# MahdiGhafoorian/NLML_HPE

Measured on AMD Instinct MI355X. Metric: faces_per_sec, higher is better.
Workload: dtype f16x2s

## Files before the change

include/nlml_hpe.h:

```cpp
#ifndef NLML_HPE_H
#define NLML_HPE_H

#include <stddef.h>
#include <stdint.h>

#ifdef __cplusplus
extern "C" {
#endif

#define NLML_ABI_VERSION 2

#define NLML_E_BADARG   (-1)
#define NLML_E_BADBLOB  (-2)
#define NLML_E_SHAPE    (-3)

#define NLML_NUM_LANDMARKS 468
#define NLML_F_REFERENCE   1404
#define NLML_LATENT        9
#define NLML_TUCKER_Q      135

int         nlml_abi_version(void);
const char* nlml_last_error(void);

int nlml_normalize_ipd(const float* raw, int64_t B, int normalize,
                       float* out, uint8_t* valid, void* stream);

int nlml_normalize_centroid(const float* raw, int64_t B, float* out, uint8_t* valid, double* stats, void* stream);
int nlml_normalize_centroid_host(const float* h_raw, int64_t B, float* h_out, uint8_t* h_valid, double* h_stats);

#define NLML_ROT_INTRINSIC 0
#define NLML_ROT_EXTRINSIC 1
int nlml_compose_rotation_tensor(const float* base, int64_t I, const double* rot_yaw, int ny, const double* rot_pitch, int np,
                                 const double* rot_roll, int nr, int order, int zero_yaw, int zero_pitch, int zero_roll,
                                 float* out, double* out64, void* stream);
int nlml_rotate_landmarks(const float* lm, const double* rot, float* out, double* out64, int64_t B, void* stream);
int nlml_compose_rotation_tensor_host(const float* h_base, int64_t I, const double* h_rot_yaw, int ny, const double* h_rot_pitch, int np,
                                      const double* h_rot_roll, int nr, int order, int zero_yaw, int zero_pitch, int zero_roll,
                                      float* h_out, double* h_out64);
int nlml_rotate_landmarks_host(const float* h_lm, const double* h_rot, float* h_out, double* h_out64, int64_t B);

#define NLML_MODE_F32   0
#define NLML_MODE_BF16  1
#define NLML_MODE_F16X2 2
#define NLML_MODE_F16X2S 3

size_t nlml_encoder_heads_packed_bytes(int F, int mode);
int    nlml_encoder_heads_pack(int F, int mode,
                               const float* const h_enc_w[6], const float* const h_enc_b[6],
                               const float* const h_head_w[3][5], const float* const h_head_b[3][5],
                               void* h_blob, size_t blob_bytes);

int nlml_encoder_heads_fwd(const float* x, int64_t ldx, int64_t B, int F,
                           const void* blob, size_t blob_bytes,
                           float* out, float* latent, uint8_t* valid, void* stream);

int nlml_encoder_heads_fwd_debug(const float* x, int64_t ldx, int64_t B, int F,
                                 const void* blob, size_t blob_bytes,
                                 float* out, float* latent, float* pre_tanh,
                                 unsigned long long* stamps, void* stream);

int nlml_landmarks_to_pose(const float* raw, int64_t B, int normalize,
                           const void* blob, size_t blob_bytes,
                           float* out, float* latent, uint8_t* valid, void* stream);

size_t nlml_encoder_heads_small_workspace_bytes(int64_t B, int F);
int nlml_encoder_heads_fwd_small(const float* x, int64_t ldx, int64_t B, int F,
                                 const void* blob, size_t blob_bytes, float* out, float* latent, uint8_t* valid,
                                 void* workspace, size_t ws_bytes, void* stream);
int nlml_landmarks_to_pose_small(const float* raw, int64_t B, int normalize,
                                 const void* blob, size_t blob_bytes, float* out, float* latent, uint8_t* valid,
                                 void* workspace, size_t ws_bytes, void* stream);

int nlml_encoder_heads_fwd_streamed(const float* x, int64_t ldx, int64_t B, int F,
                                    const void* blob, size_t blob_bytes, float* out, float* latent, uint8_t* valid,
                                    void* workspace, size_t ws_bytes, void* stream);
int nlml_landmarks_to_pose_streamed(const float* raw, int64_t B, int normalize,
                                    const void* blob, size_t blob_bytes, float* out, float* latent, uint8_t* valid,
                                    void* workspace, size_t ws_bytes, void* stream);

size_t nlml_encoder_heads_workspace_bytes(int64_t B, int F);
int nlml_encoder_heads_fwd_ws(const float* x, int64_t ldx, int64_t B, int F,
                              const void* blob, size_t blob_bytes, float* out, float* latent, uint8_t* valid,
                              void* workspace, size_t ws_bytes, void* stream);
int nlml_landmarks_to_pose_ws(const float* raw, int64_t B, int normalize,
                              const void* blob, size_t blob_bytes, float* out, float* latent, uint8_t* valid,
                              void* workspace, size_t ws_bytes, void* stream);

#define NLML_TD_ORDER_FAST      0
#define NLML_TD_ORDER_REFERENCE 1
int nlml_tucker_objective(const float* Wm, const float* x, int64_t ldx, const int32_t* x_index,
                          const double* params, const double* cos_params, int64_t N,
                          double* err, double* x_hat, void* stream);
int nlml_tucker_objective_ex(const float* Wm, const float* x, int64_t ldx, const int32_t* x_index,
                             const double* params, const double* cos_params, int64_t N,
                             double* err, double* x_hat, int order, void* stream);

int nlml_tucker_powell(const float* Wm, const float* x, int64_t ldx, const double* cos_params, int64_t N,
                       const double* x0, double* result, double* fval, int32_t* nfev, int32_t* nit,
                       int32_t* status, void* stream);
int nlml_tucker_powell_ex(const float* Wm, const float* x, int64_t ldx, const double* cos_params, int64_t N,
                          const double* x0, double* result, double* fval, int32_t* nfev, int32_t* nit,
                          int32_t* status, int order, void* stream);

#define NLML_TUCKER_RANK_MIN 1
#define NLML_TUCKER_RANK_MAX 16
int nlml_tucker_objective_r(const float* Wm, const float* x, int64_t ldx, const int32_t* x_index,
                            const double* params, const double* cos_params, int64_t N,
                            double* err, double* x_hat, int r_id, int order, void* stream);
int nlml_tucker_powell_r(const float* Wm, const float* x, int64_t ldx, const double* cos_params, int64_t N,
                         const double* x0, double* result, double* fval, int32_t* nfev, int32_t* nit,
                         int32_t* status, int r_id, int order, void* stream);

size_t nlml_tucker_gradient_workspace_bytes(int64_t N, int r_id);
int nlml_tucker_gradient_r(const float* Wm, const float* x, int64_t ldx, const int32_t* x_index,
                           const double* params, const double* cos_params, int64_t N,
                           double* err, double* grad, int r_id, void* workspace, size_t workspace_bytes, void* stream);
int nlml_tucker_gradient_host(const float* h_Wm, const float* h_x, int64_t ldx, const int32_t* h_x_index,
                              const double* h_params, const double* h_cos_params, int64_t N,
                              double* h_err, double* h_grad, int r_id, float* h_v);

int nlml_video_post(const float* pose_rad, const float* raw, const uint8_t* valid, int64_t S,
                    double frame_w, double frame_h, double alpha, double max_jump, double size,
                    double* state, double* smoothed, double* centre, double* endpoints, void* stream);
int nlml_video_post_ex(const float* pose_rad, const float* raw, const uint8_t* valid, int64_t S,
                       double frame_w, double frame_h, double alpha, double max_jump, double size,
                       double* state, double* smoothed, double* centre, double* endpoints, uint8_t* updated, void* stream);

#define NLML_POSE_EVAL_MAX_INTERVALS    64
#define NLML_POSE_EVAL_FACES_PER_RECORD 2048
size_t nlml_pose_eval_record_len(int n_intervals);
size_t nlml_pose_eval_result_len(int n_intervals);
size_t nlml_pose_eval_workspace_bytes(int64_t B, int n_intervals);
int nlml_pose_eval(const float* pose_rad, const double* pred_deg, const uint8_t* valid, const double* gt_deg, int64_t B,
                   const double* h_lo, const double* h_hi, int decimals, const double* h_intervals, const int32_t* h_axes,
                   int n_intervals, void* workspace, size_t workspace_bytes, double* record_out, double* result_out,
                   double* pred_out, uint8_t* keep_out, void* stream);
int nlml_pose_eval_merge(const double* records, int64_t n, int n_intervals, double* record_out, double* result_out,
                         void* stream);

int nlml_cosine_table(const float* angles_rad, int64_t n, const double* cos_params, int R, double* out, void* stream);
int nlml_mode5_product(const float* core, const float* U_feat, int Q, int R5, int M, float* W, void* stream);

size_t nlml_powell_state_bytes(void);
int    nlml_powell_init(void* h_state, const double* h_x0, double xtol, double ftol);
int    nlml_powell_step(void* h_state, double fin, double* h_xeval);
int    nlml_powell_result(const void* h_state, double* h_x, double* h_fval, int* h_nfev, int* h_nit, int* h_status);
size_t nlml_powell_state_bytes_n(int n);
int    nlml_powell_init_n(void* h_state, int n, const double* h_x0, double xtol, double ftol);
int    nlml_powell_step_n(void* h_state, double fin, double* h_xeval);
int    nlml_powell_result_n(const void* h_state, double* h_x, double* h_fval, int* h_nfev, int* h_nit, int* h_status);

#ifdef __cplusplus
}
#endif
#endif
```

nlml_hpe_amd/_lib.py:

```python
from __future__ import annotations

import ctypes as C
import os

_HERE = os.path.dirname(os.path.abspath(__file__))
LIB_PATH = os.environ.get("NLML_HPE_LIB") or os.path.join(_HERE, "libnlml_hpe_hip.so")

_c_f32p = C.c_void_p
_FWD_X = [C.c_void_p, C.c_int64, C.c_int64, C.c_int]
_FWD_RAW = [C.c_void_p, C.c_int64, C.c_int]
_FWD_OUT = [C.c_void_p, C.c_size_t, C.c_void_p, C.c_void_p, C.c_void_p]
_FWD_WS = [C.c_void_p, C.c_size_t]


def _k2_forwards():
    for form, ws in (("", []), ("_small", _FWD_WS), ("_streamed", _FWD_WS), ("_ws", _FWD_WS)):
        yield "nlml_encoder_heads_fwd" + form, (C.c_int, _FWD_X + _FWD_OUT + ws + [C.c_void_p])
        yield "nlml_landmarks_to_pose" + form, (C.c_int, _FWD_RAW + _FWD_OUT + ws + [C.c_void_p])


_TD_EVAL = [C.c_void_p, C.c_void_p, C.c_int64, C.c_void_p, C.c_void_p, C.c_void_p, C.c_int64, C.c_void_p, C.c_void_p]
_TD_POWELL = [C.c_void_p, C.c_void_p, C.c_int64, C.c_void_p, C.c_int64] + [C.c_void_p] * 6


def _td_entries():
    for op, head in (("objective", _TD_EVAL), ("powell", _TD_POWELL)):
        for form, tail in (("", []), ("_ex", [C.c_int]), ("_r", [C.c_int, C.c_int])):
            yield f"nlml_tucker_{op}{form}", (C.c_int, head + tail + [C.c_void_p])
    yield "nlml_tucker_gradient_r", (C.c_int, _TD_EVAL + [C.c_int, C.c_void_p, C.c_size_t, C.c_void_p])
    yield "nlml_tucker_gradient_host", (C.c_int, _TD_EVAL + [C.c_int, C.c_void_p])


_ROT_GRID = ([C.c_void_p, C.c_int64] + [C.c_void_p, C.c_int] * 3 + [C.c_int] * 4 + [C.c_void_p, C.c_void_p])

SYMBOLS = {
    **dict(_k2_forwards()),
    **dict(_td_entries()),
    "nlml_abi_version": (C.c_int, []),
    "nlml_last_error": (C.c_char_p, []),
    "nlml_normalize_ipd": (C.c_int, [C.c_void_p, C.c_int64, C.c_int, C.c_void_p, C.c_void_p, C.c_void_p]),
    "nlml_normalize_centroid": (C.c_int, [C.c_void_p, C.c_int64, C.c_void_p, C.c_void_p, C.c_void_p, C.c_void_p]),
    "nlml_normalize_centroid_host": (C.c_int, [C.c_void_p, C.c_int64, C.c_void_p, C.c_void_p, C.c_void_p]),
    "nlml_compose_rotation_tensor": (C.c_int, _ROT_GRID + [C.c_void_p]),
    "nlml_compose_rotation_tensor_host": (C.c_int, _ROT_GRID),
    "nlml_rotate_landmarks": (C.c_int, [C.c_void_p, C.c_void_p, C.c_void_p, C.c_void_p, C.c_int64, C.c_void_p]),
    "nlml_rotate_landmarks_host": (C.c_int, [C.c_void_p, C.c_void_p, C.c_void_p, C.c_void_p, C.c_int64]),
    "nlml_encoder_heads_packed_bytes": (C.c_size_t, [C.c_int, C.c_int]),
    "nlml_encoder_heads_pack": (C.c_int, [C.c_int, C.c_int, C.c_void_p, C.c_void_p, C.c_void_p, C.c_void_p,
                                          C.c_void_p, C.c_size_t]),
    "nlml_encoder_heads_fwd_debug": (C.c_int, [C.c_void_p, C.c_int64, C.c_int64, C.c_int, C.c_void_p, C.c_size_t,
                                               C.c_void_p, C.c_void_p, C.c_void_p, C.c_void_p, C.c_void_p]),
    "nlml_encoder_heads_small_workspace_bytes": (C.c_size_t, [C.c_int64, C.c_int]),
    "nlml_encoder_heads_workspace_bytes": (C.c_size_t, [C.c_int64, C.c_int]),
    "nlml_tucker_gradient_workspace_bytes": (C.c_size_t, [C.c_int64, C.c_int]),
    "nlml_video_post": (C.c_int, [C.c_void_p, C.c_void_p, C.c_void_p, C.c_int64, C.c_double, C.c_double, C.c_double,
                                  C.c_double, C.c_double, C.c_void_p, C.c_void_p, C.c_void_p, C.c_void_p, C.c_void_p]),
    "nlml_video_post_ex": (C.c_int, [C.c_void_p, C.c_void_p, C.c_void_p, C.c_int64, C.c_double, C.c_double, C.c_double,
                                     C.c_double, C.c_double, C.c_void_p, C.c_void_p, C.c_void_p, C.c_void_p, C.c_void_p, C.c_void_p]),
    "nlml_pose_eval_record_len": (C.c_size_t, [C.c_int]),
    "nlml_pose_eval_result_len": (C.c_size_t, [C.c_int]),
    "nlml_pose_eval_workspace_bytes": (C.c_size_t, [C.c_int64, C.c_int]),
    "nlml_pose_eval": (C.c_int, [C.c_void_p, C.c_void_p, C.c_void_p, C.c_void_p, C.c_int64, C.c_void_p, C.c_void_p, C.c_int,
                                 C.c_void_p, C.c_void_p, C.c_int, C.c_void_p, C.c_size_t, C.c_void_p, C.c_void_p, C.c_void_p,
                                 C.c_void_p, C.c_void_p]),
    "nlml_pose_eval_merge": (C.c_int, [C.c_void_p, C.c_int64, C.c_int, C.c_void_p, C.c_void_p, C.c_void_p]),
    "nlml_cosine_table": (C.c_int, [C.c_void_p, C.c_int64, C.c_void_p, C.c_int, C.c_void_p, C.c_void_p]),
    "nlml_mode5_product": (C.c_int, [C.c_void_p, C.c_void_p, C.c_int, C.c_int, C.c_int, C.c_void_p, C.c_void_p]),
    "nlml_powell_state_bytes": (C.c_size_t, []),
    "nlml_powell_init": (C.c_int, [C.c_void_p, C.c_void_p, C.c_double, C.c_double]),
    "nlml_powell_step": (C.c_int, [C.c_void_p, C.c_double, C.c_void_p]),
    "nlml_powell_result": (C.c_int, [C.c_void_p, C.c_void_p, C.c_void_p, C.c_void_p, C.c_void_p, C.c_void_p]),
    "nlml_powell_state_bytes_n": (C.c_size_t, [C.c_int]),
    "nlml_powell_init_n": (C.c_int, [C.c_void_p, C.c_int, C.c_void_p, C.c_double, C.c_double]),
    "nlml_powell_step_n": (C.c_int, [C.c_void_p, C.c_double, C.c_void_p]),
    "nlml_powell_result_n": (C.c_int, [C.c_void_p, C.c_void_p, C.c_void_p, C.c_void_p, C.c_void_p, C.c_void_p]),
}

MODE_F32 = 0
MODE_BF16 = 1
MODE_F16X2 = 2
MODE_F16X2S = 3
MODE_NAMES = {"f32": MODE_F32, "bf16": MODE_BF16, "f16x2": MODE_F16X2, "f16x2s": MODE_F16X2S}
DEFAULT_MODE = MODE_F16X2S
DEFAULT_MODE_NAME = "f16x2s"
TD_ORDER_FAST = 0
TD_ORDER_REFERENCE = 1
TD_ORDER_NAMES = {"fast": TD_ORDER_FAST, "reference": TD_ORDER_REFERENCE}
ROT_INTRINSIC = 0
ROT_EXTRINSIC = 1
ROT_ORDER_NAMES = {"intrinsic": ROT_INTRINSIC, "extrinsic": ROT_EXTRINSIC}
TUCKER_RANK_MIN, TUCKER_RANK_MAX = 1, 16
POSE_EVAL_MAX_INTERVALS = 64
POSE_EVAL_FACES_PER_RECORD = 2048


def td_order_from_name(order) -> int:
    if isinstance(order, str):
        if order not in TD_ORDER_NAMES:
            raise ValueError(f"unknown TD order {order!r}; expected one of {sorted(TD_ORDER_NAMES)}")
        return TD_ORDER_NAMES[order]
    if int(order) not in TD_ORDER_NAMES.values():
        raise ValueError(f"unknown TD order {order!r}")
    return int(order)


def rot_order_from_name(order) -> int:
    if isinstance(order, str):
        if order not in ROT_ORDER_NAMES:
            raise ValueError("Rotation type must be 'intrinsic' or 'extrinsic'.")
        return ROT_ORDER_NAMES[order]
    if int(order) not in ROT_ORDER_NAMES.values():
        raise ValueError(f"unknown rotation order {order!r}")
    return int(order)


def tucker_rank_of_rows(rows: int, what: str = "Wm") -> int:
    r, rem = divmod(int(rows), 27)
    if rem or not TUCKER_RANK_MIN <= r <= TUCKER_RANK_MAX:
        raise ValueError(f"{what}: expected 27*R rows (R*3*3*3) for an identity rank R in [{TUCKER_RANK_MIN}, {TUCKER_RANK_MAX}], "
                         f"got {rows}")
    return r


def mode_from_name(mode) -> int:
    if isinstance(mode, str):
        if mode not in MODE_NAMES:
            raise ValueError(f"unknown mode {mode!r}; expected one of {sorted(MODE_NAMES)}")
        return MODE_NAMES[mode]
    if int(mode) not in MODE_NAMES.values():
        raise ValueError(f"unknown mode {mode!r}")
    return int(mode)

_lib = None


class NlmlError(RuntimeError):
    pass


def lib() -> C.CDLL:
    global _lib
    if _lib is None:
        if not os.path.exists(LIB_PATH):
            raise NlmlError(
                f"{LIB_PATH} is missing: build it with `python -c 'import __graft_entry__ as g; g.build()'` "
                "(make -C nlml_hpe_amd/csrc).  There is no CPU fallback.")
        handle = C.CDLL(LIB_PATH)
        for name, (res, args) in SYMBOLS.items():
            fn = getattr(handle, name)
            fn.restype = res
            fn.argtypes = args
        if handle.nlml_abi_version() != 2:
            raise NlmlError("libnlml_hpe_hip.so ABI version mismatch")
        _lib = handle
    return _lib


def check(rc: int, what: str) -> None:
    if rc != 0:
        msg = lib().nlml_last_error()
        raise NlmlError(f"{what} failed (code {rc}): {msg.decode() if msg else ''}")
```

nlml_hpe_amd/csrc/abi.cpp:

```cpp
#include <hip/hip_runtime_api.h>

#include <cstdio>
#include <cstdlib>
#include <cstring>

#include "../../include/nlml_hpe.h"
#include "abi_internal.h"
#include "centroid_ref.h"
#include "layout.h"
#include "powell.h"
#include "rotate_ref.h"
#include "tucker_grad_ref.h"

namespace nlml {
static thread_local char g_err[256] = "";
int fail(int code, const char* msg) {
  std::snprintf(g_err, sizeof g_err, "%s", msg ? msg : "unknown error");
  return code ? code : NLML_E_BADARG;
}
int hip_launch_status() {
  const hipError_t e = hipGetLastError();
  return e == hipSuccess ? 0 : fail((int)e, hipGetErrorString(e));
}
}

using namespace nlml;

static bool known_mode(int mode) { return mode == NLML_MODE_F32 || mode == NLML_MODE_BF16 || mode == NLML_MODE_F16X2 || mode == NLML_MODE_F16X2S; }
static bool split_f16(int mode) { return mode == NLML_MODE_F16X2 || mode == NLML_MODE_F16X2S; }

extern "C" {

int nlml_abi_version(void) { return NLML_ABI_VERSION; }
const char* nlml_last_error(void) { return g_err; }

int nlml_normalize_ipd(const float* raw, int64_t B, int normalize, float* out, uint8_t* valid, void* stream) {
  if (B < 0 || (B > 0 && (!raw || !out))) return fail(NLML_E_BADARG, "normalize_ipd: null buffer or negative B");
  if ((reinterpret_cast<uintptr_t>(raw) | reinterpret_cast<uintptr_t>(out)) & 15)
    return fail(NLML_E_BADARG, "normalize_ipd: raw/out must be 16-byte aligned");
  return launch_normalize_ipd(raw, B, normalize, out, valid, stream);
}

int nlml_normalize_centroid(const float* raw, int64_t B, float* out, uint8_t* valid, double* stats, void* stream) {
  if (B < 0 || (B > 0 && (!raw || !out))) return fail(NLML_E_BADARG, "normalize_centroid: null buffer or negative B");
  if ((reinterpret_cast<uintptr_t>(raw) | reinterpret_cast<uintptr_t>(out)) & 15)
    return fail(NLML_E_BADARG, "normalize_centroid: raw/out must be 16-byte aligned");
  if (reinterpret_cast<uintptr_t>(stats) & 7) return fail(NLML_E_BADARG, "normalize_centroid: stats must be 8-byte aligned");
  return launch_normalize_centroid(raw, B, out, valid, stats, stream);
}

int nlml_normalize_centroid_host(const float* h_raw, int64_t B, float* h_out, uint8_t* h_valid, double* h_stats) {
  if (B < 0 || (B > 0 && (!h_raw || !h_out))) return fail(NLML_E_BADARG, "normalize_centroid_host: null buffer or negative B");
  for (int64_t b = 0; b < B; ++b) {
    const int v = cn_face_host(h_raw + b * NLML_F_REFERENCE, h_out + b * NLML_F_REFERENCE, h_stats ? h_stats + 4 * b : nullptr);
    if (h_valid) h_valid[b] = (uint8_t)v;
  }
  return 0;
}

static int check_rotation_grid(const char* who, bool have_buffers, int64_t I, int ny, int np, int nr, int order, int zy, int zp, int zr,
                               int64_t* rows) {
  char msg[128];
  const bool empty = I == 0 || ny == 0 || np == 0 || nr == 0;
  auto refuse = [&](const char* what) {
    std::snprintf(msg, sizeof msg, "%s: %s", who, what);
    return fail(NLML_E_BADARG, msg);
  };
  if (!empty && !have_buffers) return refuse("null buffer");
  if (I < 0 || ny < 0 || np < 0 || nr < 0) return refuse("negative extent");
  if (order != NLML_ROT_INTRINSIC && order != NLML_ROT_EXTRINSIC) return refuse("unknown order");
  if (zy < -1 || zy >= ny || zp < -1 || zp >= np || zr < -1 || zr >= nr) return refuse("zero index outside -1..n-1");
  *rows = 0;
  if (empty) return 0;
  int64_t n = 0;
  if (__builtin_mul_overflow(I, (int64_t)ny, &n) || __builtin_mul_overflow(n, (int64_t)np, &n) || __builtin_mul_overflow(n, (int64_t)nr, &n) ||
      n > INT64_MAX / (NLML_F_REFERENCE * 8))
    return refuse("tensor too large for 64-bit byte offsets");
  *rows = n;
  return 0;
}

int nlml_compose_rotation_tensor(const float* base, int64_t I, const double* rot_yaw, int ny, const double* rot_pitch, int np,
                                 const double* rot_roll, int nr, int order, int zero_yaw, int zero_pitch, int zero_roll, float* out,
                                 double* out64, void* stream) {
  int64_t rows;
  if (const int rc = check_rotation_grid("compose_rotation_tensor", base && rot_yaw && rot_pitch && rot_roll && out, I, ny, np, nr, order,
                                         zero_yaw, zero_pitch, zero_roll, &rows))
    return rc;
  if (rows == 0) return 0;
  if ((reinterpret_cast<uintptr_t>(base) | reinterpret_cast<uintptr_t>(out)) & 15)
    return fail(NLML_E_BADARG, "compose_rotation_tensor: base/out must be 16-byte aligned");
  if ((reinterpret_cast<uintptr_t>(rot_yaw) | reinterpret_cast<uintptr_t>(rot_pitch) | reinterpret_cast<uintptr_t>(rot_roll) |
       reinterpret_cast<uintptr_t>(out64)) & 7)
    return fail(NLML_E_BADARG, "compose_rotation_tensor: the matrices and out64 must be 8-byte aligned");
  return launch_compose_rotation_tensor(base, rows, rot_yaw, ny, rot_pitch, np, rot_roll, nr, order, zero_yaw, zero_pitch, zero_roll, out,
                                        out64, stream);
}

int nlml_compose_rotation_tensor_host(const float* h_base, int64_t I, const double* h_rot_yaw, int ny, const double* h_rot_pitch, int np,
                                      const double* h_rot_roll, int nr, int order, int zero_yaw, int zero_pitch, int zero_roll,
                                      float* h_out, double* h_out64) {
  int64_t rows;
  if (const int rc = check_rotation_grid("compose_rotation_tensor_host", h_base && h_rot_yaw && h_rot_pitch && h_rot_roll && (h_out || h_out64),
                                         I, ny, np, nr, order, zero_yaw, zero_pitch, zero_roll, &rows))
    return rc;
  if (rows) rt_grid_host(h_base, I, h_rot_yaw, ny, h_rot_pitch, np, h_rot_roll, nr, order, zero_yaw, zero_pitch, zero_roll, h_out, h_out64);
  return 0;
}

int nlml_rotate_landmarks(const float* lm, const double* rot, float* out, double* out64, int64_t B, void* stream) {
  if (B != 0 && (!lm || !rot || (!out && !out64))) return fail(NLML_E_BADARG, "rotate_landmarks: null buffer (lm, rot, and out or out64)");
  if (B < 0) return fail(NLML_E_BADARG, "rotate_landmarks: negative extent");
  if (B == 0) return 0;
  if (B > INT64_MAX / (NLML_F_REFERENCE * 8)) return fail(NLML_E_BADARG, "rotate_landmarks: too many faces for 64-bit byte offsets");
  if ((reinterpret_cast<uintptr_t>(lm) | reinterpret_cast<uintptr_t>(out)) & 15)
    return fail(NLML_E_BADARG, "rotate_landmarks: lm/out must be 16-byte aligned");
  if ((reinterpret_cast<uintptr_t>(rot) | reinterpret_cast<uintptr_t>(out64)) & 7)
    return fail(NLML_E_BADARG, "rotate_landmarks: rot/out64 must be 8-byte aligned");
  return launch_rotate_landmarks(lm, rot, out, out64, B, stream);
}

int nlml_rotate_landmarks_host(const float* h_lm, const double* h_rot, float* h_out, double* h_out64, int64_t B) {
  if (B != 0 && (!h_lm || !h_rot || (!h_out && !h_out64))) return fail(NLML_E_BADARG, "rotate_landmarks_host: null buffer (lm, rot, and out or out64)");
  if (B < 0) return fail(NLML_E_BADARG, "rotate_landmarks_host: negative extent");
  for (int64_t b = 0; b < B; ++b)
    rt_face_host(h_lm + b * NLML_F_REFERENCE, h_rot + b * 27, h_rot + b * 27 + 9, h_rot + b * 27 + 18,
                 h_out ? h_out + b * NLML_F_REFERENCE : nullptr, h_out64 ? h_out64 + b * NLML_F_REFERENCE : nullptr);
  return 0;
}

size_t nlml_encoder_heads_packed_bytes(int F, int mode) {
  if (F <= 0 || !known_mode(mode)) return 0;
  return blob_bytes_for(F, mode);
}

int nlml_encoder_heads_pack(int F, int mode, const float* const h_enc_w[6], const float* const h_enc_b[6],
                            const float* const h_head_w[3][5], const float* const h_head_b[3][5], void* h_blob,
                            size_t blob_bytes) {
  if (!known_mode(mode)) return fail(NLML_E_BADARG, "pack: unsupported mode");
  if (!h_enc_w || !h_enc_b || !h_head_w || !h_head_b) return fail(NLML_E_BADARG, "pack: null table");
  return pack_blob(F, mode, h_enc_w, h_enc_b, h_head_w, h_head_b, h_blob, blob_bytes);
}

static int check_blob_args(int64_t B, int F, const void* blob, size_t blob_bytes, const float* out, int* mode) {
  if (B < 0 || F <= 0) return fail(NLML_E_BADARG, "encoder_heads: negative B or bad F");
  if (B > 0 && (!blob || !out)) return fail(NLML_E_BADARG, "encoder_heads: null buffer");
  if (reinterpret_cast<uintptr_t>(blob) & 15) return fail(NLML_E_BADARG, "encoder_heads: blob must be 16-byte aligned");
  if (blob_bytes == blob_bytes_for(F, NLML_MODE_F32)) *mode = NLML_MODE_F32;
  else if (blob_bytes == blob_bytes_for(F, NLML_MODE_BF16)) *mode = NLML_MODE_BF16;
  else if (blob_bytes == blob_bytes_for(F, NLML_MODE_F16X2)) *mode = NLML_MODE_F16X2;
  else if (blob_bytes == blob_bytes_for(F, NLML_MODE_F16X2S)) *mode = NLML_MODE_F16X2S;
  else return fail(NLML_E_BADBLOB, "encoder_heads: blob size does not match F in any mode");
  return 0;
}

static const int64_t kSmallMax = 4096;
static int64_t streamed_min() {
  static const int64_t v = [] { const char* e = getenv("NLML_K2_STREAMED_MIN"); return e && e[0] ? (int64_t)atoll(e) : (int64_t)-1; }();
  return v;
}

enum K2Form { K2_FUSED, K2_SMALL, K2_STREAMED, K2_AUTO };

static int k2_forward(K2Form form, bool landmarks, const float* x, int64_t ldx, const float* raw, int normalize, int64_t B, int F,
                      const void* blob, size_t blob_bytes, float* out, float* latent, uint8_t* valid, void* workspace, size_t ws_bytes,
                      void* stream) {
  const char* no_input = nullptr;
  if (B > 0 && landmarks && !raw) no_input = "landmarks_to_pose: null raw";
  if (B > 0 && !landmarks && (!x || ldx < F)) no_input = "encoder_heads: null x or ldx < F";
  if (no_input && form == K2_AUTO && landmarks) return fail(NLML_E_BADARG, no_input);
  int mode = 0;
  if (int rc = check_blob_args(B, F, blob, blob_bytes, out, &mode)) return rc;
  if (form == K2_SMALL && !split_f16(mode)) return fail(NLML_E_BADARG, "small-batch path: NLML_MODE_F16X2 / NLML_MODE_F16X2S blob only");
  if (form == K2_STREAMED && mode != NLML_MODE_F16X2S) return fail(NLML_E_BADARG, "streamed-tail path: NLML_MODE_F16X2S blob only");
  if (no_input) return fail(NLML_E_BADARG, no_input);
  const int split = mode == NLML_MODE_F16X2S;
  if (form == K2_AUTO) {
    if (split_f16(mode) && B <= kSmallMax) form = K2_SMALL;
    else if (split && streamed_min() >= 0 && B >= streamed_min() && k2_input(x, ldx, raw, normalize, F).vec4) form = K2_STREAMED;
    else form = K2_FUSED;
  }
  if (form == K2_SMALL)
    return launch_encoder_heads_f16x2_small(x, ldx, raw, normalize, B, F, blob, out, latent, valid, workspace, ws_bytes, split, stream);
  if (form == K2_STREAMED)
    return launch_encoder_heads_f16x2_tailws(x, ldx, raw, normalize, B, F, blob, out, latent, valid, workspace, ws_bytes, stream);
  if (mode == NLML_MODE_BF16) return launch_encoder_heads_bf16(x, ldx, raw, normalize, B, F, blob, out, latent, valid, stream);
  if (split_f16(mode)) return launch_encoder_heads_f16x2(x, ldx, raw, normalize, B, F, blob, out, latent, valid, split, stream);
  return launch_encoder_heads_f32(x, ldx, raw, normalize, B, F, blob, out, latent, valid, nullptr, nullptr, stream);
}

int nlml_encoder_heads_fwd(const float* x, int64_t ldx, int64_t B, int F, const void* blob, size_t blob_bytes,
                           float* out, float* latent, uint8_t* valid, void* stream) {
  return k2_forward(K2_FUSED, false, x, ldx, nullptr, 0, B, F, blob, blob_bytes, out, latent, valid, nullptr, 0, stream);
}

int nlml_encoder_heads_fwd_debug(const float* x, int64_t ldx, int64_t B, int F, const void* blob, size_t blob_bytes,
                                 float* out, float* latent, float* pre_tanh, unsigned long long* stamps, void* stream) {
  int mode = 0;
  if (int rc = check_blob_args(B, F, blob, blob_bytes, out, &mode)) return rc;
  if (mode != NLML_MODE_F32) return fail(NLML_E_BADARG, "debug build: f32 blob only");
  if (B > 0 && (!x || ldx < F)) return fail(NLML_E_BADARG, "encoder_heads: null x or ldx < F");
  return launch_encoder_heads_f32(x, ldx, nullptr, 0, B, F, blob, out, latent, nullptr, pre_tanh, stamps, stream);
}

int nlml_landmarks_to_pose(const float* raw, int64_t B, int normalize, const void* blob, size_t blob_bytes,
                           float* out, float* latent, uint8_t* valid, void* stream) {
  return k2_forward(K2_FUSED, true, nullptr, 0, raw, normalize, B, NLML_F_REFERENCE, blob, blob_bytes, out, latent, valid, nullptr, 0, stream);
}

size_t nlml_encoder_heads_small_workspace_bytes(int64_t B, int F) { return small_workspace_bytes(B, F); }

int nlml_encoder_heads_fwd_small(const float* x, int64_t ldx, int64_t B, int F, const void* blob, size_t blob_bytes,
                                 float* out, float* latent, uint8_t* valid, void* workspace, size_t ws_bytes, void* stream) {
  return k2_forward(K2_SMALL, false, x, ldx, nullptr, 0, B, F, blob, blob_bytes, out, latent, valid, workspace, ws_bytes, stream);
}

int nlml_landmarks_to_pose_small(const float* raw, int64_t B, int normalize, const void* blob, size_t blob_bytes,
                                 float* out, float* latent, uint8_t* valid, void* workspace, size_t ws_bytes, void* stream) {
  return k2_forward(K2_SMALL, true, nullptr, 0, raw, normalize, B, NLML_F_REFERENCE, blob, blob_bytes, out, latent, valid, workspace, ws_bytes, stream);
}

int nlml_encoder_heads_fwd_streamed(const float* x, int64_t ldx, int64_t B, int F, const void* blob, size_t blob_bytes,
                                    float* out, float* latent, uint8_t* valid, void* workspace, size_t ws_bytes, void* stream) {
  return k2_forward(K2_STREAMED, false, x, ldx, nullptr, 0, B, F, blob, blob_bytes, out, latent, valid, workspace, ws_bytes, stream);
}

int nlml_landmarks_to_pose_streamed(const float* raw, int64_t B, int normalize, const void* blob, size_t blob_bytes,
                                    float* out, float* latent, uint8_t* valid, void* workspace, size_t ws_bytes, void* stream) {
  return k2_forward(K2_STREAMED, true, nullptr, 0, raw, normalize, B, NLML_F_REFERENCE, blob, blob_bytes, out, latent, valid, workspace, ws_bytes, stream);
}

size_t nlml_encoder_heads_workspace_bytes(int64_t B, int F) {
  const size_t a = small_workspace_bytes(B, F), b = tailws_workspace_bytes(B, F);
  return a > b ? a : b;
}

int nlml_encoder_heads_fwd_ws(const float* x, int64_t ldx, int64_t B, int F, const void* blob, size_t blob_bytes,
                              float* out, float* latent, uint8_t* valid, void* workspace, size_t ws_bytes, void* stream) {
  return k2_forward(K2_AUTO, false, x, ldx, nullptr, 0, B, F, blob, blob_bytes, out, latent, valid, workspace, ws_bytes, stream);
}

int nlml_landmarks_to_pose_ws(const float* raw, int64_t B, int normalize, const void* blob, size_t blob_bytes,
                              float* out, float* latent, uint8_t* valid, void* workspace, size_t ws_bytes, void* stream) {
  return k2_forward(K2_AUTO, true, nullptr, 0, raw, normalize, B, NLML_F_REFERENCE, blob, blob_bytes, out, latent, valid, workspace, ws_bytes, stream);
}

int nlml_video_post_ex(const float* pose_rad, const float* raw, const uint8_t* valid, int64_t S, double frame_w,
                       double frame_h, double alpha, double max_jump, double size, double* state, double* smoothed,
                       double* centre, double* endpoints, uint8_t* updated, void* stream) {
  if (S < 0) return fail(NLML_E_BADARG, "video_post: negative S");
  if (S > 0 && (!pose_rad || !raw || !state || !smoothed || !centre || !endpoints))
    return fail(NLML_E_BADARG, "video_post: null buffer");
  return launch_video_post(pose_rad, raw, valid, S, frame_w, frame_h, alpha, max_jump, size, state, smoothed, centre,
                           endpoints, updated, stream);
}

int nlml_video_post(const float* pose_rad, const float* raw, const uint8_t* valid, int64_t S, double frame_w,
                    double frame_h, double alpha, double max_jump, double size, double* state, double* smoothed,
                    double* centre, double* endpoints, void* stream) {
  return nlml_video_post_ex(pose_rad, raw, valid, S, frame_w, frame_h, alpha, max_jump, size, state, smoothed, centre, endpoints,
                            nullptr, stream);
}

int nlml_cosine_table(const float* angles_rad, int64_t n, const double* cos_params, int R, double* out, void* stream) {
  if (n < 0 || R < 0) return fail(NLML_E_BADARG, "cosine_table: negative size");
  if (n > 0 && R > 0 && (!angles_rad || !cos_params || !out)) return fail(NLML_E_BADARG, "cosine_table: null buffer");
  return launch_cosine_table(angles_rad, n, cos_params, R, out, stream);
}

int nlml_mode5_product(const float* core, const float* U_feat, int Q, int R5, int M, float* W, void* stream) {
  if (Q < 0 || R5 < 0 || M < 0) return fail(NLML_E_BADARG, "mode5_product: negative size");
  if (Q > 0 && M > 0 && (!W || (R5 > 0 && (!core || !U_feat)))) return fail(NLML_E_BADARG, "mode5_product: null buffer");
  return launch_mode5_product(core, U_feat, Q, R5, M, W, stream);
}

static bool eval_k_ok(int K) { return K >= 0 && K <= NLML_POSE_EVAL_MAX_INTERVALS; }
static int64_t eval_records(int64_t B) { return (B + NLML_POSE_EVAL_FACES_PER_RECORD - 1) / NLML_POSE_EVAL_FACES_PER_RECORD; }

size_t nlml_pose_eval_record_len(int n_intervals) { return eval_k_ok(n_intervals) ? (size_t)(12 + 2 * n_intervals) : 0; }
size_t nlml_pose_eval_result_len(int n_intervals) { return eval_k_ok(n_intervals) ? (size_t)(14 + 2 * n_intervals) : 0; }
size_t nlml_pose_eval_workspace_bytes(int64_t B, int n_intervals) {
  if (B < 0 || !eval_k_ok(n_intervals)) return 0;
  return (size_t)eval_records(B) * nlml_pose_eval_record_len(n_intervals) * sizeof(double);
}

static bool misaligned8(const void* p) { return (reinterpret_cast<uintptr_t>(p) & 7) != 0; }

int nlml_pose_eval(const float* pose_rad, const double* pred_deg, const uint8_t* valid, const double* gt_deg, int64_t B,
                   const double* h_lo, const double* h_hi, int decimals, const double* h_intervals, const int32_t* h_axes,
                   int n_intervals, void* workspace, size_t workspace_bytes, double* record_out, double* result_out,
                   double* pred_out, uint8_t* keep_out, void* stream) {
  if (B < 0) return fail(NLML_E_BADARG, "pose_eval: negative B");
  if ((pose_rad && pred_deg) || (B > 0 && !pose_rad && !pred_deg))
    return fail(NLML_E_BADARG, "pose_eval: give exactly one of pose_rad and pred_deg");
  if (B > 0 && !gt_deg) return fail(NLML_E_BADARG, "pose_eval: null gt_deg");
  if (!h_lo || !h_hi || !result_out) return fail(NLML_E_BADARG, "pose_eval: null lo / hi / result_out");
  if (!eval_k_ok(n_intervals)) return fail(NLML_E_BADARG, "pose_eval: number of intervals outside [0, NLML_POSE_EVAL_MAX_INTERVALS]");
  if (n_intervals > 0 && (!h_intervals || !h_axes)) return fail(NLML_E_BADARG, "pose_eval: null intervals / axes");
  if (decimals > 15) return fail(NLML_E_BADARG, "pose_eval: decimals > 15");
  const size_t need = nlml_pose_eval_workspace_bytes(B, n_intervals);
  if (workspace_bytes < need || (need > 0 && !workspace)) return fail(NLML_E_BADARG, "pose_eval: workspace too small");
  if (misaligned8(pred_deg) || misaligned8(gt_deg) || misaligned8(workspace) || misaligned8(record_out) || misaligned8(result_out) ||
      misaligned8(pred_out) || (reinterpret_cast<uintptr_t>(pose_rad) & 3))
    return fail(NLML_E_BADARG, "pose_eval: f64 buffers must be 8-byte aligned, pose_rad 4-byte aligned");
  PoseEvalArgs a{};
  for (int i = 0; i < 3; ++i) { a.lo[i] = h_lo[i]; a.hi[i] = h_hi[i]; }
  for (int k = 0; k < n_intervals; ++k) {
    if (h_axes[k] < 0 || h_axes[k] > 2) return fail(NLML_E_BADARG, "pose_eval: interval axis outside {0, 1, 2}");
    a.axes[k] = h_axes[k];
    a.ivl[k][0] = h_intervals[2 * k];
    a.ivl[k][1] = h_intervals[2 * k + 1];
  }
  a.scale = 1.0;
  for (int i = 0; i < decimals; ++i) a.scale *= 10.0;
  a.K = n_intervals;
  a.decimals = decimals;
  return launch_pose_eval(pose_rad, pred_deg, valid, gt_deg, B, a, static_cast<double*>(workspace), record_out, result_out, pred_out,
                          keep_out, stream);
}

int nlml_pose_eval_merge(const double* records, int64_t n, int n_intervals, double* record_out, double* result_out, void* stream) {
  if (n < 0) return fail(NLML_E_BADARG, "pose_eval_merge: negative record count");
  if (!eval_k_ok(n_intervals)) return fail(NLML_E_BADARG, "pose_eval_merge: number of intervals outside [0, NLML_POSE_EVAL_MAX_INTERVALS]");
  if ((n > 0 && !records) || !result_out) return fail(NLML_E_BADARG, "pose_eval_merge: null records / result_out");
  if (misaligned8(records) || misaligned8(record_out) || misaligned8(result_out))
    return fail(NLML_E_BADARG, "pose_eval_merge: buffers must be 8-byte aligned");
  return launch_pose_eval_merge(records, n, n_intervals, record_out, result_out, stream);
}

static_assert(PW_NMAX == 3 + NLML_TUCKER_RANK_MAX && PW_N == 3 + 5, "powell.h's state sizes follow the ranks");
static bool rank_ok(int r_id) { return r_id >= NLML_TUCKER_RANK_MIN && r_id <= NLML_TUCKER_RANK_MAX; }
static int bad_rank(const char* who, int r_id) {
  char msg[160];
  snprintf(msg, sizeof msg, "%s: identity rank %d outside [%d, %d]", who, r_id, NLML_TUCKER_RANK_MIN, NLML_TUCKER_RANK_MAX);
  return fail(NLML_E_SHAPE, msg);
}

static int check_td_args(const char* who, int r_id, int order, int64_t N, int64_t ldx, bool null_buffer, const float* Wm, const float* x) {
  if (!rank_ok(r_id)) return bad_rank(who, r_id);
  const char* what = nullptr;
  if (order != NLML_TD_ORDER_FAST && order != NLML_TD_ORDER_REFERENCE) what = "unknown order";
  else if (N < 0) what = "negative N";
  else if (N == 0) return 0;
  else if (null_buffer) what = "null buffer";
  else if (ldx < NLML_F_REFERENCE) what = "ldx < 1404";
  else if (order == NLML_TD_ORDER_FAST && (((reinterpret_cast<uintptr_t>(Wm) | reinterpret_cast<uintptr_t>(x)) & 15) || (ldx & 3)))
    what = "NLML_TD_ORDER_FAST needs Wm and x 16-byte aligned and ldx % 4 == 0";
  if (!what) return 0;
  char msg[160];
  snprintf(msg, sizeof msg, "%s: %s", who, what);
  return fail(NLML_E_BADARG, msg);
}

static int td_objective(const char* who, const float* Wm, const float* x, int64_t ldx, const int32_t* x_index, const double* params,
                        const double* cos_params, int64_t N, double* err, double* x_hat, int r_id, int order, void* stream) {
  if (int rc = check_td_args(who, r_id, order, N, ldx, !Wm || !x || !params || !cos_params || !err, Wm, x)) return rc;
  return launch_tucker_objective(Wm, x, ldx, x_index, params, cos_params, N, err, x_hat, r_id, order, stream);
}

int nlml_tucker_objective(const float* Wm, const float* x, int64_t ldx, const int32_t* x_index, const double* params,
                          const double* cos_params, int64_t N, double* err, double* x_hat, void* stream) {
  return td_objective("tucker_objective", Wm, x, ldx, x_index, params, cos_params, N, err, x_hat, 5, NLML_TD_ORDER_REFERENCE, stream);
}

int nlml_tucker_objective_ex(const float* Wm, const float* x, int64_t ldx, const int32_t* x_index, const double* params,
                             const double* cos_params, int64_t N, double* err, double* x_hat, int order, void* stream) {
  return td_objective("tucker_objective", Wm, x, ldx, x_index, params, cos_params, N, err, x_hat, 5, order, stream);
}

int nlml_tucker_objective_r(const float* Wm, const float* x, int64_t ldx, const int32_t* x_index, const double* params,
                            const double* cos_params, int64_t N, double* err, double* x_hat, int r_id, int order, void* stream) {
  return td_objective("tucker_objective_r", Wm, x, ldx, x_index, params, cos_params, N, err, x_hat, r_id, order, stream);
}

static int td_powell(const char* who, const float* Wm, const float* x, int64_t ldx, const double* cos_params, int64_t N, const double* x0,
                     double* result, double* fval, int32_t* nfev, int32_t* nit, int32_t* status, int r_id, int order, void* stream) {
  if (int rc = check_td_args(who, r_id, order, N, ldx, !Wm || !x || !cos_params || !result, Wm, x)) return rc;
  return launch_tucker_powell(Wm, x, ldx, cos_params, N, x0, result, fval, nfev, nit, status, r_id, order, stream);
}

int nlml_tucker_powell(const float* Wm, const float* x, int64_t ldx, const double* cos_params, int64_t N, const double* x0,
                       double* result, double* fval, int32_t* nfev, int32_t* nit, int32_t* status, void* stream) {
  return td_powell("tucker_powell", Wm, x, ldx, cos_params, N, x0, result, fval, nfev, nit, status, 5, NLML_TD_ORDER_REFERENCE, stream);
}

int nlml_tucker_powell_ex(const float* Wm, const float* x, int64_t ldx, const double* cos_params, int64_t N, const double* x0,
                          double* result, double* fval, int32_t* nfev, int32_t* nit, int32_t* status, int order, void* stream) {
  return td_powell("tucker_powell", Wm, x, ldx, cos_params, N, x0, result, fval, nfev, nit, status, 5, order, stream);
}

int nlml_tucker_powell_r(const float* Wm, const float* x, int64_t ldx, const double* cos_params, int64_t N, const double* x0,
                         double* result, double* fval, int32_t* nfev, int32_t* nit, int32_t* status, int r_id, int order,
                         void* stream) {
  return td_powell("tucker_powell_r", Wm, x, ldx, cos_params, N, x0, result, fval, nfev, nit, status, r_id, order, stream);
}

size_t nlml_tucker_gradient_workspace_bytes(int64_t N, int r_id) { return rank_ok(r_id) ? tucker_gradient_workspace_bytes(N) : 0; }

int nlml_tucker_gradient_r(const float* Wm, const float* x, int64_t ldx, const int32_t* x_index, const double* params,
                           const double* cos_params, int64_t N, double* err, double* grad, int r_id, void* workspace,
                           size_t workspace_bytes, void* stream) {
  if (int rc = check_td_args("tucker_gradient_r", r_id, NLML_TD_ORDER_REFERENCE, N, ldx, !Wm || !x || !params || !cos_params || !grad, Wm, x))
    return rc;
  const size_t need = tucker_gradient_workspace_bytes(N);
  if (workspace_bytes < need || (need > 0 && !workspace)) return fail(NLML_E_BADARG, "tucker_gradient_r: workspace too small");
  if (misaligned8(workspace) || misaligned8(err) || misaligned8(grad) || misaligned8(params))
    return fail(NLML_E_BADARG, "tucker_gradient_r: f64 buffers and the workspace must be 8-byte aligned");
  return launch_tucker_gradient(Wm, x, ldx, x_index, params, cos_params, N, err, grad, r_id, workspace, stream);
}

int nlml_tucker_gradient_host(const float* h_Wm, const float* h_x, int64_t ldx, const int32_t* h_x_index, const double* h_params,
                              const double* h_cos_params, int64_t N, double* h_err, double* h_grad, int r_id, float* h_v) {
  if (int rc = check_td_args("tucker_gradient_host", r_id, NLML_TD_ORDER_REFERENCE, N, ldx,
                             !h_Wm || !h_x || !h_params || !h_cos_params || !h_grad, h_Wm, h_x))
    return rc;
  for (int64_t n = 0; n < N; ++n)
    tg_gradient_host(h_Wm, h_x + (h_x_index ? (int64_t)h_x_index[n] : n) * ldx, h_params + n * (3 + r_id), h_cos_params, r_id,
                     h_err ? h_err + n : nullptr, h_grad + n * (3 + r_id), h_v ? h_v + n * NLML_F_REFERENCE : nullptr);
  return 0;
}

static bool dim_ok(int n) { return n >= 3 + NLML_TUCKER_RANK_MIN && n <= 3 + NLML_TUCKER_RANK_MAX; }
static int null_pointer(const char* who) {
  char msg[64];
  snprintf(msg, sizeof msg, "%s: null pointer", who);
  return fail(NLML_E_BADARG, msg);
}

extern "C++" {
template <class S> static int powell_host_init(const char* who, void* h_state, int n, const double* h_x0, double xtol, double ftol) {
  if (!dim_ok(n)) return bad_rank(who, n - 3);
  if (!h_state || !h_x0) return null_pointer(who);
  S& s = *static_cast<S*>(h_state);
  if (S::kDyn) std::memset(h_state, 0, sizeof(S));
  s.set_dim(n);
  powell_init(s, h_x0, xtol, ftol);
  return 0;
}

template <class S> static int powell_host_step(const char* who, void* h_state, double fin, double* h_xeval) {
  if (!h_state || !h_xeval) return null_pointer(who);
  S& s = *static_cast<S*>(h_state);
  if (!dim_ok(s.dim())) return bad_rank(who, s.dim() - 3);
  const bool need = powell_step(s, fin);
  if (need) std::memcpy(h_xeval, s.xeval, sizeof(double) * s.dim());
  return need ? 1 : 0;
}

template <class S>
static int powell_host_result(const char* who, const void* h_state, double* h_x, double* h_fval, int* h_nfev, int* h_nit, int* h_status) {
  if (!h_state || !h_x) return null_pointer(who);
  const S& s = *static_cast<const S*>(h_state);
  if (!dim_ok(s.dim())) return bad_rank(who, s.dim() - 3);
  std::memcpy(h_x, s.x, sizeof(double) * s.dim());
  if (h_fval) *h_fval = s.fval;
  if (h_nfev) *h_nfev = s.nfev;
  if (h_nit) *h_nit = s.iter;
  if (h_status) *h_status = s.status;
  return 0;
}
}

size_t nlml_powell_state_bytes(void) { return sizeof(PowellState); }
int nlml_powell_init(void* h_state, const double* h_x0, double xtol, double ftol) {
  return powell_host_init<PowellState>("powell_init", h_state, PW_N, h_x0, xtol, ftol);
}
int nlml_powell_step(void* h_state, double fin, double* h_xeval) { return powell_host_step<PowellState>("powell_step", h_state, fin, h_xeval); }
int nlml_powell_result(const void* h_state, double* h_x, double* h_fval, int* h_nfev, int* h_nit, int* h_status) {
  return powell_host_result<PowellState>("powell_result", h_state, h_x, h_fval, h_nfev, h_nit, h_status);
}

size_t nlml_powell_state_bytes_n(int n) { return dim_ok(n) ? sizeof(PowellStateN) : 0; }
int nlml_powell_init_n(void* h_state, int n, const double* h_x0, double xtol, double ftol) {
  return powell_host_init<PowellStateN>("powell_init_n", h_state, n, h_x0, xtol, ftol);
}
int nlml_powell_step_n(void* h_state, double fin, double* h_xeval) { return powell_host_step<PowellStateN>("powell_step_n", h_state, fin, h_xeval); }
int nlml_powell_result_n(const void* h_state, double* h_x, double* h_fval, int* h_nfev, int* h_nit, int* h_status) {
  return powell_host_result<PowellStateN>("powell_result_n", h_state, h_x, h_fval, h_nfev, h_nit, h_status);
}

}
```

nlml_hpe_amd/csrc/abi_internal.h:

```cpp
#pragma once
#include <stddef.h>
#include <stdint.h>

#include <type_traits>

#include "../../include/nlml_hpe.h"

namespace nlml {

int fail(int code, const char* msg);
int hip_launch_status();

struct K2Input { const float* src; int64_t ld; int norm; bool vec4; };
inline K2Input k2_input(const float* x, int64_t ldx, const float* raw, int normalize, int F) {
  K2Input a;
  if (raw) {
    a.src = raw; a.ld = NLML_F_REFERENCE; a.norm = normalize ? 1 : 0;
  } else {
    a.src = x; a.ld = ldx; a.norm = 0;
  }
  a.vec4 = (F % 4 == 0) && (a.ld % 4 == 0) && ((reinterpret_cast<uintptr_t>(a.src) & 15) == 0);
  return a;
}
template <class Args>
Args k2_args(const K2Input& in, int64_t B, int F, const void* blob, float* out, float* latent, uint8_t* valid) {
  Args a{};
  a.B = B; a.F = F; a.blob = blob; a.out = out; a.latent = latent; a.valid = valid;
  a.x = in.src; a.ldx = in.ld; a.norm = in.norm;
  return a;
}
template <class Fn> void k2_with_variant(const K2Input& in, Fn&& fn) {
  if (in.norm) {
    if (in.vec4) fn(std::true_type{}, std::true_type{}); else fn(std::false_type{}, std::true_type{});
  } else {
    if (in.vec4) fn(std::true_type{}, std::false_type{}); else fn(std::false_type{}, std::false_type{});
  }
}

size_t blob_bytes_for(int F, int mode);
int pack_blob(int F, int mode, const float* const enc_w[6], const float* const enc_b[6],
              const float* const head_w[3][5], const float* const head_b[3][5],
              void* blob, size_t blob_bytes);

int launch_encoder_heads_f32(const float* x, int64_t ldx, const float* raw, int normalize,
                             int64_t B, int F, const void* blob, float* out, float* latent,
                             uint8_t* valid, float* pre_tanh, unsigned long long* stamps, void* stream,
                             int reeval_over = -1);
size_t strict_f32_image_offset(int F);
int launch_strict_reeval(const float* x, int64_t ldx, const float* raw, int normalize, int64_t B, int F, const void* blob,
                         float* out, float* latent, void* stream);
constexpr int STRICT_INKERNEL_RESCUE_MAX = 0;
int launch_encoder_heads_bf16(const float* x, int64_t ldx, const float* raw, int normalize,
                              int64_t B, int F, const void* blob, float* out, float* latent,
                              uint8_t* valid, void* stream);
int launch_encoder_heads_f16x2(const float* x, int64_t ldx, const float* raw, int normalize,
                               int64_t B, int F, const void* blob, float* out, float* latent,
                               uint8_t* valid, int split, void* stream);
int launch_encoder_heads_f16x2_w8(const float* x, int64_t ldx, const float* raw, int normalize, int64_t B, int F,
                                  const void* blob, float* out, float* latent, uint8_t* valid, void* stream);
size_t tailws_workspace_bytes(int64_t B, int F);
int launch_encoder_heads_f16x2_tailws(const float* x, int64_t ldx, const float* raw, int normalize, int64_t B, int F,
                                      const void* blob, float* out, float* latent, uint8_t* valid, void* workspace,
                                      size_t ws_bytes, void* stream);
int launch_tail_ws(const void* blob, const void* h3, int64_t nfb, int64_t B, float* out, float* latent, void* stream);
size_t small_workspace_bytes(int64_t B, int F);
int launch_encoder_heads_f16x2_small(const float* x, int64_t ldx, const float* raw, int normalize, int64_t B, int F,
                                     const void* blob, float* out, float* latent, uint8_t* valid, void* workspace,
                                     size_t ws_bytes, int split, void* stream);
int launch_cosine_table(const float* angles, int64_t n, const double* cos_params, int R, double* out, void* stream);
int launch_mode5_product(const float* core, const float* U, int Q, int R5, int M, float* W, void* stream);
int launch_normalize_ipd(const float* raw, int64_t B, int normalize, float* out, uint8_t* valid,
                         void* stream);
int launch_normalize_centroid(const float* raw, int64_t B, float* out, uint8_t* valid, double* stats, void* stream);
int launch_compose_rotation_tensor(const float* base, int64_t rows, const double* rot_yaw, int ny, const double* rot_pitch, int np,
                                   const double* rot_roll, int nr, int order, int zero_yaw, int zero_pitch, int zero_roll, float* out,
                                   double* out64, void* stream);
int launch_rotate_landmarks(const float* lm, const double* rot, float* out, double* out64, int64_t B, void* stream);
int launch_tucker_objective(const float* Wm, const float* x, int64_t ldx, const int32_t* x_index, const double* params,
                            const double* cos_params, int64_t N, double* err, double* x_hat, int r_id, int order, void* stream);
int launch_tucker_powell(const float* Wm, const float* x, int64_t ldx, const double* cos_params, int64_t N, const double* x0,
                         double* result, double* fval, int32_t* nfev, int32_t* nit, int32_t* status, int r_id, int order,
                         void* stream);

size_t tucker_gradient_workspace_bytes(int64_t N);
int launch_tucker_gradient(const float* Wm, const float* x, int64_t ldx, const int32_t* x_index, const double* params,
                           const double* cos_params, int64_t N, double* err, double* grad, int r_id, void* workspace, void* stream);

int launch_video_post(const float* pose_rad, const float* raw, const uint8_t* valid, int64_t S, double frame_w,
                      double frame_h, double alpha, double max_jump, double size, double* state, double* smoothed,
                      double* centre, double* endpoints, uint8_t* updated, void* stream);

struct PoseEvalArgs {
  double lo[3], hi[3];
  double scale;
  double ivl[NLML_POSE_EVAL_MAX_INTERVALS][2];
  int32_t axes[NLML_POSE_EVAL_MAX_INTERVALS];
  int K, decimals;
};
int launch_pose_eval(const float* pose_rad, const double* pred_deg, const uint8_t* valid, const double* gt_deg, int64_t B,
                     const PoseEvalArgs& args, double* workspace, double* record_out, double* result_out, double* pred_out,
                     uint8_t* keep_out, void* stream);
int launch_pose_eval_merge(const double* records, int64_t n, int K, double* record_out, double* result_out, void* stream);

}
```

nlml_hpe_amd/csrc/encoder_heads_f16x2_tailws.hip:

```cpp
#include <hip/hip_runtime.h>

#include "../../include/nlml_hpe.h"
#include "abi_internal.h"
#include "encoder_heads_f16x2_dev.h"
#include "layout.h"

#if defined(__HIP_DEVICE_COMPILE__) && !defined(__gfx950__)
#error "global_load_lds_dwordx4: gfx950"
#endif

namespace nlml {
namespace hx {

typedef unsigned u4 __attribute__((ext_vector_type(4)));
#define TW_PRIO(p) __builtin_amdgcn_s_setprio(p)
typedef __attribute__((address_space(3))) const char LdsC;
typedef __attribute__((address_space(3))) char LdsW;

struct TwArgs {
  const void* blob;
  const u4* h3;
  float* out;
  float* latent;
  int64_t B, nfb;
};

constexpr int TW_SLOT = 65536;
constexpr int tw_bias_n16(int s) { return kStages[s].jobs * kStages[s].nb * 8; }
constexpr int tw_bias_off(int s) {
  int o = 0;
  for (int t = ST_E3; t < s; ++t) o += tw_bias_n16(t) * 16;
  return o;
}
constexpr uint32_t tw_b_off(int s, uint32_t k16_e0) {
  int c = (int)(sizeof(Header) / 16), m = 0;
  for (int t = 0; t < s; ++t) {
    c += kStages[t].jobs * ((t == ST_E0 ? 0 : kStages[t].k8 * kStages[t].nb * 64 * PIECES) + kStages[t].nb * 8);
    m += kStages[t].jobs * (t == ST_E0 ? kStages[t].nb * 64 * PIECES : 0);
  }
  return c + m * k16_e0 + kStages[s].jobs * ((s == ST_E0 ? 0 : kStages[s].k8 * kStages[s].nb * 64 * PIECES) + (s == ST_E0 ? kStages[s].nb * 64 * PIECES : 0) * k16_e0);
}
constexpr bool tw_b_off_is_layouts() {
  for (int s = 0; s < NUM_STAGES; ++s)
    if (tw_b_off(s, 0u) != layout_b_off(kLayoutHX, s, 0u) || tw_b_off(s, 88u) != layout_b_off(kLayoutHX, s, 88u)) return false;
  return true;
}
static_assert(tw_b_off_is_layouts(), "the written-out bias offsets are layout.h's");
constexpr int TW_O_BIAS = 2 * TW_SLOT;
constexpr int TW_O_LAT = TW_O_BIAS + ((tw_bias_off(NUM_STAGES) + 511) / 512) * 512;
constexpr int TW_LAT_WAVE = 3 * 2 * 256;
constexpr int TW_LDS = TW_O_LAT + 8 * TW_LAT_WAVE;
static_assert(TW_LDS <= 163840, "LDS map");

constexpr int TW_HEAD_UNITS = 9, TW_UNITS = 4 + 3 * TW_HEAD_UNITS;
constexpr uint32_t tw_job_w16(int s) { return layout_job_w16(kLayoutHX, s, 0u); }
__device__ __forceinline__ void tw_unit(const HdrRegs& H, int idx, uint32_t& off, uint32_t& n16) {
  constexpr uint32_t J3 = tw_job_w16(ST_E3), J4 = tw_job_w16(ST_E4), J5 = tw_job_w16(ST_E5);
  constexpr uint32_t K0 = tw_job_w16(ST_H0), K1 = tw_job_w16(ST_H1), K2 = tw_job_w16(ST_H2), K3 = tw_job_w16(ST_H3), K4 = tw_job_w16(ST_H4);
  static_assert(2 * J3 * 16 == TW_SLOT && 2 * J4 * 16 <= TW_SLOT && J5 * 16 <= TW_SLOT && 4 * K0 * 16 <= TW_SLOT && K1 * 16 <= TW_SLOT &&
                    2 * K2 * 16 == TW_SLOT && 2 * K3 * 16 <= TW_SLOT && K4 * 16 <= TW_SLOT,
                "a unit fits a buffer");
  if (idx < 2) { n16 = 2 * J3; off = H.w_off(ST_E3) + idx * 2 * J3; }
  else if (idx == 2) { n16 = 2 * J4; off = H.w_off(ST_E4); }
  else if (idx == 3) { n16 = J5; off = H.w_off(ST_E5); }
  else {
    const int k = idx - 4, g = k / TW_HEAD_UNITS, r = k - TW_HEAD_UNITS * g;
    if (r == 0) { n16 = 4 * K0; off = H.w_off(ST_H0) + 4 * g * K0; }
    else if (r <= 4) { n16 = K1; off = H.w_off(ST_H1) + (4 * g + (r - 1)) * K1; }
    else if (r <= 6) { n16 = 2 * K2; off = H.w_off(ST_H2) + (4 * g + 2 * (r - 5)) * K2; }
    else if (r == 7) { n16 = 2 * K3; off = H.w_off(ST_H3) + 2 * g * K3; }
    else { n16 = K4; off = H.w_off(ST_H4) + g * K4; }
  }
}

template <int K16, int NCH = 2>
__device__ __forceinline__ void tw_job2(f32x16 (&acc)[2], LdsC* w0, LdsC* w1, int wstep, LdsC* b0, LdsC* b1, const h8 (&in)[K16][2]) {
  typedef const __attribute__((address_space(3))) h8 LdsH8;
#pragma unroll
  for (int c = 0; c < NCH; ++c)
#pragma unroll
    for (int q = 0; q < 4; ++q) {
      const f32x4 v = *reinterpret_cast<const __attribute__((address_space(3))) f32x4*>((c ? b1 : b0) + q * 16);
      acc[c][4 * q + 0] = v[0];
      acc[c][4 * q + 1] = v[1];
      acc[c][4 * q + 2] = v[2];
      acc[c][4 * q + 3] = v[3];
    }
  TW_PRIO(2);
#pragma unroll
  for (int ks = 0; ks < K16; ++ks) {
    h8 wf[NCH][2];
#pragma unroll
    for (int c = 0; c < NCH; ++c)
#pragma unroll
      for (int p = 0; p < 2; ++p) wf[c][p] = *reinterpret_cast<LdsH8*>((c ? w1 : w0) + ks * wstep + p * 1024);
#pragma unroll
    for (int t = 0; t < 3; ++t)
#pragma unroll
      for (int c = 0; c < NCH; ++c)
        acc[c] = __builtin_amdgcn_mfma_f32_32x32x16_f16(wf[c][t == 0 ? 1 : 0], in[ks][t == 1 ? 1 : 0], acc[c], 0, 0, 0);
  }
  TW_PRIO(0);
}

template <int K16>
__device__ __forceinline__ void tw_job2p(f32x16 (&acc)[2], LdsC* w0, LdsC* w1, int wstep, LdsC* b0, LdsC* b1, const h8 (&in)[K16][2]) {
  typedef const __attribute__((address_space(3))) h8 LdsH8;
#pragma unroll
  for (int c = 0; c < 2; ++c)
#pragma unroll
    for (int q = 0; q < 4; ++q) {
      const f32x4 v = *reinterpret_cast<const __attribute__((address_space(3))) f32x4*>((c ? b1 : b0) + q * 16);
      acc[c][4 * q + 0] = v[0];
      acc[c][4 * q + 1] = v[1];
      acc[c][4 * q + 2] = v[2];
      acc[c][4 * q + 3] = v[3];
    }
  h8 wf[2][2][2];
#pragma unroll
  for (int c = 0; c < 2; ++c)
#pragma unroll
    for (int p = 0; p < 2; ++p) wf[0][c][p] = *reinterpret_cast<LdsH8*>((c ? w1 : w0) + p * 1024);
  TW_PRIO(2);
  __builtin_amdgcn_sched_barrier(0);
#pragma unroll
  for (int ks = 0; ks < K16; ++ks) {
#pragma unroll
    for (int m = 0; m < 6; ++m) {
      const int t = m >> 1, c = m & 1;
      acc[c] = __builtin_amdgcn_mfma_f32_32x32x16_f16(wf[ks & 1][c][t == 0 ? 1 : 0], in[ks][t == 1 ? 1 : 0], acc[c], 0, 0, 0);
      __builtin_amdgcn_sched_barrier(0);
      if (m < 4 && ks + 1 < K16)
        wf[(ks + 1) & 1][m & 1][m < 2 ? 1 : 0] = *reinterpret_cast<LdsH8*>(((m & 1) ? w1 : w0) + (ks + 1) * wstep + (m < 2 ? 1024 : 0));
      __builtin_amdgcn_sched_barrier(0);
    }
  }
  TW_PRIO(0);
}

__global__ __launch_bounds__(512) void tail_ws_kernel(TwArgs a) {
  __shared__ __attribute__((aligned(1024))) char lds[TW_LDS];
  const int tid = threadIdx.x, lane = tid & 63, f = lane & 31, h = lane >> 5;
  const int wv = __builtin_amdgcn_readfirstlane(tid >> 6);
  const HdrRegs H = load_hdr(reinterpret_cast<const Header*>(a.blob));
  const h8* const blob8 = reinterpret_cast<const h8*>(a.blob);
  const f32x4* const blob4 = reinterpret_cast<const f32x4*>(a.blob);

  int64_t fbg = (int64_t)blockIdx.x * 8 + wv;
  const bool wave_live = fbg < a.nfb;
  fbg = wave_live ? fbg : a.nfb - 1;
  const int64_t row = fbg * 32 + f;
  const bool row_live = wave_live && row < a.B;

  LdsW* const ring = (LdsW*)(lds);
  auto issue = [&](int idx, int slot_off) {
    if (idx >= TW_UNITS) return;
    uint32_t off, n16;
    tw_unit(H, idx, off, n16);
    const int npieces = (int)(n16 >> 6);
#pragma unroll
    for (int i = 0; i < TW_SLOT / 8192; ++i) {
      const int pc = wv + 8 * i;
      if (pc < npieces)
        __builtin_amdgcn_global_load_lds((const __attribute__((address_space(1))) void*)(blob8 + off + pc * 64 + lane),
                                         (__attribute__((address_space(3))) void*)(ring + slot_off + pc * 1024), 16, 0, 0);
    }
  };
#ifdef TW_STAMPS
  int tw_u = 0;
#define TWS(i)                                                                                                                \
  do {                                                                                                                        \
    if (a.latent && lane == 0)                                                                                                \
      reinterpret_cast<unsigned long long*>(a.latent)[((size_t)blockIdx.x * 8 + wv) * 96 + (i)] = __builtin_amdgcn_s_memtime(); \
  } while (0)
#define TW_STAMP_MID() TWS(2 + 2 * tw_u)
#define TW_STAMP_END() do { TWS(3 + 2 * tw_u); ++tw_u; } while (0)
#else
#define TWS(i) do { } while (0)
#define TW_STAMP_MID() do { } while (0)
#define TW_STAMP_END() do { } while (0)
#endif
  TWS(0);
  issue(0, 0);

  {
    f32x4* const bl = reinterpret_cast<f32x4*>(lds + TW_O_BIAS);
#pragma unroll
    for (int s = ST_E3; s < NUM_STAGES; ++s) {
      const f32x4* src = blob4 + tw_b_off(s, H.k8_e0);
      for (int i = tid; i < tw_bias_n16(s); i += 512) bl[tw_bias_off(s) / 16 + i] = src[i];
    }
  }
  h8 x3[TrunkFrags::STEPS][2];
  {
    const u4* src = a.h3 + TrunkFrags::unit(fbg, 0, 0, 0) + lane;
#pragma unroll
    for (int ks = 0; ks < TrunkFrags::STEPS; ++ks)
#pragma unroll
      for (int p = 0; p < 2; ++p) x3[ks][p] = __builtin_bit_cast(h8, src[TrunkFrags::frag(0, ks, p)]);
  }
  asm volatile("s_waitcnt vmcnt(0)" ::: "memory");
  __syncthreads();
  TWS(1);

  int cur = 0;
  LdsC* const bias0 = (LdsC*)(lds + TW_O_BIAS) + 64 * h;
  LdsC* const wl0 = (LdsC*)(lds) + lane * 16;
  LdsW* const latw = (LdsW*)(lds + TW_O_LAT) + wv * TW_LAT_WAVE + f * 8;
#ifdef TW_NO_SKEW
  const bool late = false;
#else
  const bool late = wv >= 4;
#endif
#define TW_BEGIN(idx) issue((idx) + 1, cur ^ TW_SLOT); LdsC* const wl = wl0 + cur
#define TW_MID()                                      \
  TW_STAMP_MID();                                     \
  asm volatile("s_waitcnt vmcnt(0)" ::: "memory");    \
  if (late) __syncthreads()
#define TW_END()                                      \
  asm volatile("s_waitcnt vmcnt(0)" ::: "memory");    \
  if (!late) __syncthreads();                         \
  TW_STAMP_END();                                     \
  cur ^= TW_SLOT

  f32x16 acc[2];
  auto emit = [&](auto act, const f32x16& ac, float inv, h8 (&d0)[2], h8 (&d1)[2]) {
    h8 fr[2][2];
    frags_from_acc<decltype(act)::value>(ac, inv, fr);
    d0[0] = fr[0][0]; d0[1] = fr[0][1]; d1[0] = fr[1][0]; d1[1] = fr[1][1];
  };
  constexpr std::integral_constant<int, ACT_RELU> RELU{};
  constexpr std::integral_constant<int, ACT_TANH> TANH{};
  const float inv3 = H.inv_scale[ST_E3], inv4 = H.inv_scale[ST_E4], inv5 = H.inv_scale[ST_E5];
  constexpr int JB3 = (int)(tw_job_w16(ST_E3) * 16), JB4 = (int)(tw_job_w16(ST_E4) * 16);

  h8 x4[8][2];
#pragma unroll
  for (int u = 0; u < 2; ++u) {
    TW_BEGIN(u);
    LdsC* const b = bias0 + tw_bias_off(ST_E3) + (2 * u) * 128;
    tw_job2p<16>(acc, wl, wl + JB3, 2048, b, b + 128, x3);
    TW_MID();
    emit(RELU, acc[0], inv3, x4[4 * u], x4[4 * u + 1]);
    emit(RELU, acc[1], inv3, x4[4 * u + 2], x4[4 * u + 3]);
    TW_END();
  }
  h8 x5[4][2];
  {
    TW_BEGIN(2);
    LdsC* const b = bias0 + tw_bias_off(ST_E4);
    tw_job2<8>(acc, wl, wl + JB4, 2048, b, b + 128, x4);
    TW_MID();
    emit(TANH, acc[0], inv4, x5[0], x5[1]);
    emit(TANH, acc[1], inv4, x5[2], x5[3]);
    TW_END();
  }
  {
    TW_BEGIN(3);
    LdsC* const b = bias0 + tw_bias_off(ST_E5);
    tw_job2<4>(acc, wl, wl + 2048, 4096, b, b + 128, x5);
    TW_MID();
#ifndef TW_STAMPS
    if (a.latent && row_live) {
#pragma unroll
      for (int nb = 0; nb < 2; ++nb)
#pragma unroll
        for (int q = 0; q < 16; ++q) {
          const int rowi = 32 * nb + (q & 3) + 8 * (q >> 2) + 4 * h, g = rowi >> 4, cc = rowi & 15;
          if (g < 3 && cc < 3) a.latent[row * NLML_LATENT + 3 * g + cc] = acc[nb][q] * inv5;
        }
    }
#endif
#pragma unroll
    for (int nb = 0; nb < 2; ++nb) {
      h8 fr[2][2];
      frags_from_acc<ACT_NONE>(acc[nb], inv5, fr);
#pragma unroll
      for (int p = 0; p < 2; ++p)
#pragma unroll
        for (int pc = 0; pc < 2; ++pc)
          if (2 * nb + p < 3 && h == 0) {
            const u4 t = __builtin_bit_cast(u4, fr[p][pc]);
            typedef unsigned u2 __attribute__((ext_vector_type(2)));
            *reinterpret_cast<__attribute__((address_space(3))) u2*>(latw + ((2 * nb + p) * 2 + pc) * 256) = u2{t[0], t[1]};
          }
    }
    TW_END();
  }
#pragma unroll 1
  for (int g = 0; g < 3; ++g) {
    const int u0 = 4 + TW_HEAD_UNITS * g;
    const float i0 = H.inv_scale[ST_H0], i1 = H.inv_scale[ST_H1], i2 = H.inv_scale[ST_H2], i3 = H.inv_scale[ST_H3];
    h8 xa[8][2];
    {
      TW_BEGIN(u0);
      h8 xin[1][2];
#pragma unroll
      for (int pc = 0; pc < 2; ++pc) {
        typedef unsigned u2 __attribute__((ext_vector_type(2)));
        const u2 t = *reinterpret_cast<const __attribute__((address_space(3))) u2*>((LdsC*)latw + (g * 2 + pc) * 256);
        xin[0][pc] = __builtin_bit_cast(h8, u4{h == 0 ? t[0] : 0u, h == 0 ? t[1] : 0u, 0u, 0u});
      }
      LdsC* const b = bias0 + tw_bias_off(ST_H0) + (4 * g) * 128;
      constexpr int JB = (int)(tw_job_w16(ST_H0) * 16);
#pragma unroll
      for (int jj = 0; jj < 2; ++jj) {
        tw_job2<1>(acc, wl + (2 * jj) * JB, wl + (2 * jj + 1) * JB, 2048, b + (2 * jj) * 128, b + (2 * jj + 1) * 128, xin);
        if (jj == 1) { TW_MID(); }
        emit(RELU, acc[0], i0, xa[4 * jj], xa[4 * jj + 1]);
        emit(RELU, acc[1], i0, xa[4 * jj + 2], xa[4 * jj + 3]);
      }
      TW_END();
    }
    h8 xb[16][2];
#pragma unroll
    for (int j = 0; j < 4; ++j) {
      TW_BEGIN(u0 + 1 + j);
      LdsC* const b = bias0 + tw_bias_off(ST_H1) + (4 * g + j) * 256;
      tw_job2p<8>(acc, wl, wl + 2048, 4096, b, b + 128, xa);
      TW_MID();
      emit(RELU, acc[0], i1, xb[4 * j], xb[4 * j + 1]);
      emit(RELU, acc[1], i1, xb[4 * j + 2], xb[4 * j + 3]);
      TW_END();
    }
    h8 xc[8][2];
#pragma unroll
    for (int u = 0; u < 2; ++u) {
      TW_BEGIN(u0 + 5 + u);
      constexpr int JB = (int)(tw_job_w16(ST_H2) * 16);
      LdsC* const b = bias0 + tw_bias_off(ST_H2) + (4 * g + 2 * u) * 128;
      tw_job2p<16>(acc, wl, wl + JB, 2048, b, b + 128, xb);
      TW_MID();
      emit(RELU, acc[0], i2, xc[4 * u], xc[4 * u + 1]);
      emit(RELU, acc[1], i2, xc[4 * u + 2], xc[4 * u + 3]);
      TW_END();
    }
    h8 xd[4][2];
    {
      TW_BEGIN(u0 + 7);
      LdsC* const b = bias0 + tw_bias_off(ST_H3) + (2 * g) * 128;
      tw_job2p<8>(acc, wl, wl + (int)(tw_job_w16(ST_H3) * 16), 2048, b, b + 128, xc);
      TW_MID();
      emit(RELU, acc[0], i3, xd[0], xd[1]);
      emit(RELU, acc[1], i3, xd[2], xd[3]);
      TW_END();
    }
    {
      TW_BEGIN(u0 + 8);
      LdsC* const b = bias0 + tw_bias_off(ST_H4) + g * 128;
      tw_job2<4, 1>(acc, wl, wl, 2048, b, b, xd);
      TW_MID();
      if (h == 0 && row_live) a.out[row * 3 + g] = acc[0][0] * H.inv_scale[ST_H4];
      TW_END();
    }
  }
#undef TW_BEGIN
#undef TW_MID
#undef TW_END
}

}

int launch_tail_ws(const void* blob, const void* h3, int64_t nfb, int64_t B, float* out, float* latent, void* stream) {
  if (B == 0) return 0;
  hx::TwArgs a;
  a.blob = blob; a.h3 = reinterpret_cast<const hx::u4*>(h3); a.out = out; a.latent = latent; a.B = B; a.nfb = nfb;
  hipLaunchKernelGGL(hx::tail_ws_kernel, dim3((unsigned)((nfb + 7) / 8)), dim3(512), 0, reinterpret_cast<hipStream_t>(stream), a);
  return hip_launch_status();
}

}
```

nlml_hpe_amd/csrc/encoder_heads_f16x2_w8.hip:

```cpp
#include <hip/hip_runtime.h>

#include "../../include/nlml_hpe.h"
#include "abi_internal.h"
#include "ipd_norm.h"
#include "encoder_heads_f16x2_dev.h"
#include "layout.h"

#ifndef W8_D0_HI
#define W8_D0_HI 2
#endif
#ifndef W8_D0_LO
#define W8_D0_LO 2
#endif

namespace nlml {
namespace hx {

template <typename XHi, typename XLo, typename Extra>
__device__ __forceinline__ void step_w8(f32x16 (&acc)[2][2], f32x16 (&accS)[2][2], const h8 (&wcur)[2][2], const h8 (&xh)[2], h8 (&xl)[2],
                                        h8 (&wnext_hi)[2][2], const h8* __restrict__ wp_hi, h8 (&wnext_lo)[2][2], const h8* __restrict__ wp_lo,
                                        XHi xload_hi, XLo xload_lo, Extra extra) {
#pragma unroll
  for (int m = 0; m < 12; ++m) {
    const int t = m / 4, nb = (m % 4) / 2, fb = m % 2;
    if (t == 0) accS[nb][fb] = __builtin_amdgcn_mfma_f32_32x32x16_f16(wcur[nb][1], xh[fb], accS[nb][fb], 0, 0, 0);
    else if (t == 1) accS[nb][fb] = __builtin_amdgcn_mfma_f32_32x32x16_f16(wcur[nb][0], xl[fb], accS[nb][fb], 0, 0, 0);
    else acc[nb][fb] = __builtin_amdgcn_mfma_f32_32x32x16_f16(wcur[nb][0], xh[fb], acc[nb][fb], 0, 0, 0);
    __builtin_amdgcn_sched_barrier(0);
    if (m == 0) xload_hi(0);
    if (m == 1) xload_hi(1);
    if (m == 2) wnext_hi[0][0] = wp_hi[0];
    if (m == 4) wnext_lo[0][1] = wp_lo[64];
    if (m == 6) wnext_hi[1][0] = wp_hi[128];
    if (m == 8) xload_lo(0);
    if (m == 9) xload_lo(1);
    if (m == 10) wnext_lo[1][1] = wp_lo[192];
    extra(m);
    __builtin_amdgcn_sched_barrier(0);
  }
}

template <bool VEC4, bool NORM>
__device__ __forceinline__ void stage_e0_pass_w8(const Ctx& c, const Args& a, int64_t row0, int tid, int pass, int jw, int nbh,
                                                 f32x16 (&acc)[2][2], f32x16 (&accS)[2][2]) {
  constexpr int NB = 2, NFB = 2;
  constexpr int WSTEP = 4 * 2 * 64;
  const int F = a.F;
  const int nslab = (int)c.hdr.k8_e0 / XS_STEPS;

  const int srow = tid >> 3, scol = (tid & 7) * 4;
  int64_t r = row0 + srow;
  const bool live = r < a.B;
  r = live ? r : a.B - 1;
  const float* p = a.x + r * a.ldx;
  double ipd = 1.0, rcp = 1.0, ra = 0.0, rb = 0.0, rc = 0.0;
  if (NORM) {
    double x0, y0, z0;
    ipd_setup(p, ipd, rcp, x0, y0, z0);
    ipd_phase(scol % 3, x0, y0, z0, ra, rb, rc);
  }
  unsigned nzbits = 0u;

  struct Set { float v[4]; };
  auto gload = [&](int s, Set& st) {
    s = s < nslab ? s : nslab - 1;
    const int k = s * XS_COLS + scol;
    if (VEC4) {
      const int kc = k < F ? k : (NORM ? k - 12 * ((k - F + 15) / 12) : F - 4);
      const f32x4 t = *reinterpret_cast<const f32x4*>(p + kc);
#pragma unroll
      for (int e = 0; e < 4; ++e) st.v[e] = t[e];
    } else {
#pragma unroll
      for (int e = 0; e < 4; ++e) st.v[e] = p[k + e < F ? k + e : F - 1];
    }
  };
  auto lw_begin = [&](Set& st) {
#pragma unroll
    for (int e = 0; e < 4; ++e) asm volatile("" : "+v"(st.v[e]));
  };
  auto lw_norm = [&](Set& st, int q) {
    const int t = q % 3;
    const double rr = t == 0 ? ra : (t == 1 ? rb : rc);
    st.v[q] = (float)div_ipd((double)st.v[q] - rr, ipd, rcp);
  };
  auto lw_rotate = [&]() {
    const double t0 = rc; rc = rb; rb = ra; ra = t0;
  };
  typedef unsigned u2 __attribute__((ext_vector_type(2)));
  unsigned pend_hi[2], pend_lo[2];
  auto lw_split = [&](Set& st, int j, bool real_slab) {
    const unsigned m = real_slab ? 0x7fffffffu : 0u;
    nzbits |= (__float_as_uint(st.v[2 * j]) | __float_as_uint(st.v[2 * j + 1])) & m;
    split2(st.v[2 * j], st.v[2 * j + 1], pend_hi[j], pend_lo[j]);
  };
  constexpr int XW_PLANE = 64 * 64, XW_SLAB = 2 * XW_PLANE, XW_BUF = 2 * XW_SLAB, O_XW = LDS_BYTES - 2 * XW_BUF;
  static_assert(O_XW >= 16 * 512 * 16, "slabs behind the parked accumulators");
  const int wr_off = srow * 64 + ((((tid & 7) >> 1) ^ ((srow >> 2) & 3)) << 4) + 8 * (tid & 1);
  auto lw_store = [&](int slab_off, int piece) {
    char* d = c.lds + O_XW + slab_off + wr_off;
    if (piece == 0) *reinterpret_cast<u2*>(d) = u2{pend_hi[0], pend_hi[1]};
    else *reinterpret_cast<u2*>(d + XW_PLANE) = u2{pend_lo[0], pend_lo[1]};
  };
  auto lwrite = [&](int slab_off, Set& st, bool real_slab) {
    lw_begin(st);
    if (NORM) {
#pragma unroll
      for (int q = 0; q < 4; ++q) lw_norm(st, q);
      lw_rotate();
    }
#pragma unroll
    for (int j = 0; j < 2; ++j) lw_split(st, j, real_slab);
    lw_store(slab_off, 0);
    lw_store(slab_off, 1);
  };

  const int job = 4 * pass + jw;
  load_bias<NB, NFB>(acc, c.blob4 + c.hdr.b_off(ST_E0) + job * (4 * 8) + (2 * nbh) * 8, c.h);
  zero_acc<NB, NFB>(accS);
  const h8* w = c.blob8 + c.hdr.w_off(ST_E0) + (size_t)job * c.hdr.job_w16(ST_E0) + (2 * nbh * 2) * 64 + c.lane;
  auto wfrag = [&](int ks) { return w + (size_t)ks * WSTEP; };

  Set set[2];
  constexpr int R0 = 4, DH = W8_D0_HI, DL = W8_D0_LO;
  h8 wr[R0][NB][2];
  gload(0, set[0]);
  gload(1, set[1]);
  lwrite(0, set[0], true);
  lwrite(XW_SLAB, set[1], true);
  gload(2, set[0]);
  gload(3, set[1]);
#pragma unroll
  for (int d = 0; d < (DH > DL ? DH : DL); ++d)
#pragma unroll
    for (int nb = 0; nb < NB; ++nb)
#pragma unroll
      for (int pp = 0; pp < 2; ++pp)
        if (d < (pp ? DL : DH)) wr[d][nb][pp] = wfrag(d)[(nb * 2 + pp) * 64];
  __syncthreads();

  const int rd0 = c.f * 64 + ((c.h ^ ((c.f >> 2) & 3)) << 4);
  typedef __attribute__((address_space(3))) const char LdsC;
  LdsC* const xb0 = (LdsC*)(c.lds + O_XW + rd0);
  LdsC* const xb1 = (LdsC*)(c.lds + O_XW + (rd0 ^ 32));
  h8 xh[2][NFB], xl[NFB];
  auto xread = [&](LdsC* base, int t, int fb, int pp) {
    return *reinterpret_cast<const __attribute__((address_space(3))) h8*>(base + (t >> 1) * XW_SLAB + pp * XW_PLANE + fb * (32 * 64));
  };
  const int niter = nslab / 2;
#pragma unroll
  for (int fb = 0; fb < NFB; ++fb) {
    xh[0][fb] = xread(xb0, 0, fb, 0);
    xl[fb] = xread(xb0, 0, fb, 1);
  }
  int cur = 0, nxt = XW_BUF;
  for (int it = 0; it < niter; ++it) {
    const int s = 2 * it;
    LdsC* xc[2] = {xb0 + cur, xb1 + cur};
    LdsC* xn = xb0 + nxt;
    asm volatile("" : "+v"(xc[0]), "+v"(xc[1]), "+v"(xn));
#pragma unroll
    for (int t = 0; t < 4; ++t) {
      const int ks = 4 * it + t;
      if (t == 3) __syncthreads();
      step_w8(acc, accS, wr[t], xh[t & 1], xl, wr[(t + DH) % R0], wfrag(ks + DH), wr[(t + DL) % R0], wfrag(ks + DL),
              [&](int fb) { xh[(t + 1) & 1][fb] = t < 3 ? xread(xc[(t + 1) & 1], t + 1, fb, 0) : xread(xn, 0, fb, 0); },
              [&](int fb) { xl[fb] = t < 3 ? xread(xc[(t + 1) & 1], t + 1, fb, 1) : xread(xn, 0, fb, 1); },
              [&](int m) {
                if (t >= 2) return;
                Set& st = set[t & 1];
                const int j = m;
                const bool real = s + t + 2 < nslab;
                if (j == 0) lw_begin(st);
                if (NORM && j >= 1 && j < 5) lw_norm(st, j - 1);
                if (NORM && j == 5) lw_rotate();
                if (j == 6 || j == 7) lw_split(st, j - 6, real);
                if (j == 8) lw_store(nxt + t * XW_SLAB, 0);
                if (j == 9) lw_store(nxt + t * XW_SLAB, 1);
                if (j == 11) gload(s + t + 4, st);
              });
    }
    const int t0 = cur; cur = nxt; nxt = t0;
  }
  if (pass == 0 && a.valid) write_valid<8>(a.valid, nzbits, tid & 7, c.lane, live, row0 + srow);
}

#ifdef HX_STAMPS
#define W8S(i)                                                                                                          \
  do {                                                                                                                  \
    if (a.latent && c.lane == 0)                                                                                        \
      reinterpret_cast<unsigned long long*>(a.latent)[((size_t)blockIdx.x * 8 + c.wv) * 16 + (i)] = __builtin_amdgcn_s_memtime(); \
  } while (0)
#define W8S_WALL(i)                                                                                                     \
  do {                                                                                                                  \
    if (a.latent && c.lane == 0)                                                                                        \
      reinterpret_cast<unsigned long long*>(a.latent)[((size_t)blockIdx.x * 8 + c.wv) * 16 + (i)] = wall_clock64();     \
  } while (0)
#else
#define W8S(i) do { } while (0)
#define W8S_WALL(i) do { } while (0)
#endif

template <bool VEC4, bool NORM, bool TRUNK = false>
__global__ __launch_bounds__(512) void encoder_heads_f16x2_w8_kernel(Args a) {
  __shared__ __attribute__((aligned(16))) char lds[LDS_BYTES];

  const int tid = threadIdx.x;
  Ctx c;
  c.blob8 = reinterpret_cast<const h8*>(a.blob);
  c.blob4 = reinterpret_cast<const f32x4*>(a.blob);
  c.hdr = load_hdr(reinterpret_cast<const Header*>(a.blob));
  c.lds = lds;
  c.lane = tid & 63;
  c.f = c.lane & 31;
  c.h = c.lane >> 5;
  c.wv = __builtin_amdgcn_readfirstlane(tid >> 6);
  const int jw = c.wv >> 1, nbh = c.wv & 1;
  const int64_t row0 = (int64_t)blockIdx.x * TILE_FACES;

  {
    constexpr int WSTEP1 = 4 * 2 * 64;
    const h8* w1 = c.blob8 + c.hdr.w_off(ST_E1) + (size_t)jw * c.hdr.job_w16(ST_E1) + (2 * nbh * 2) * 64 + c.lane;
    const float inv0 = c.hdr.inv_scale[ST_E0];
    f32x16 acc1[2][2];
    f32x4* const park = reinterpret_cast<f32x4*>(c.lds + O_H1H) + tid;
    static_assert(16 * 512 * 16 <= 2 * P_H1H, "the parked layer-1 accumulators fit the h1 half image");
    load_bias<2, 2>(acc1, c.blob4 + c.hdr.b_off(ST_E1) + jw * (4 * 8) + (2 * nbh) * 8, c.h);
    auto park_acc1 = [&]() {
#pragma unroll
      for (int nb = 0; nb < 2; ++nb)
#pragma unroll
        for (int fb = 0; fb < 2; ++fb)
#pragma unroll
          for (int q = 0; q < 4; ++q)
            park[512 * ((nb * 2 + fb) * 4 + q)] = f32x4{acc1[nb][fb][4 * q], acc1[nb][fb][4 * q + 1], acc1[nb][fb][4 * q + 2], acc1[nb][fb][4 * q + 3]};
    };
    park_acc1();
    W8S(0);
    W8S_WALL(14);
#pragma unroll 1
    for (int pass = 0; pass < 2; ++pass) {
      {
        f32x16 acc0[2][2], acc0s[2][2];
        stage_e0_pass_w8<VEC4, NORM>(c, a, row0, tid, pass, jw, nbh, acc0, acc0s);
        add_acc<2, 2>(acc0, acc0s);
        W8S(1 + 4 * pass);
#pragma unroll
        for (int nb = 0; nb < 2; ++nb)
#pragma unroll
          for (int fb = 0; fb < 2; ++fb)
#pragma unroll
            for (int q = 0; q < 4; ++q) {
              const f32x4 t = park[512 * ((nb * 2 + fb) * 4 + q)];
              acc1[nb][fb][4 * q] = t[0]; acc1[nb][fb][4 * q + 1] = t[1]; acc1[nb][fb][4 * q + 2] = t[2]; acc1[nb][fb][4 * q + 3] = t[3];
            }
        __syncthreads();
        job_store<2, 2, ACT_RELU>(c, acc0, O_H1H, P_H1H, S_H1H, 128 * jw + 64 * nbh, 0, inv0);
      }
      __syncthreads();
      W8S(2 + 4 * pass);
      {
        f32x16 acc1s[2][2];
        zero_acc<2, 2>(acc1s);
        kloop<2, 2, 32, WSTEP1>(acc1, acc1s, w1 + (size_t)pass * 32 * WSTEP1, c.lds + O_H1H + (c.f * S_H1H + 8 * c.h) * 2, P_H1H,
                                32 * S_H1H * 2);
        add_acc<2, 2>(acc1, acc1s);
      }
      W8S(3 + 4 * pass);
      __syncthreads();
      if (pass == 0) park_acc1();
      W8S(4 + 4 * pass);
    }
    job_store<2, 2, ACT_RELU>(c, acc1, O_H2, P_H2, S_H2, 128 * jw + 64 * nbh, 0, c.hdr.inv_scale[ST_E1]);
  }
  __syncthreads();
  W8S(9);
  Ctx ct = c;
  ct.wv = c.wv & 3;
  f32x16 acc3[1][2];
  h8 wr3[ring_slots(1, 2)][1][2];
  {
    constexpr int WSTEP2 = 2 * 2 * 64;
    f32x16 acc2[1][2], acc2s[1][2];
    load_bias<1, 2>(acc2, c.blob4 + c.hdr.b_off(ST_E2) + jw * (2 * 8) + nbh * 8, c.h);
    zero_acc<1, 2>(acc2s);
    const h8* w2 = c.blob8 + c.hdr.w_off(ST_E2) + (size_t)jw * c.hdr.job_w16(ST_E2) + (nbh * 2) * 64 + c.lane;
    kloop<1, 2, 32, WSTEP2>(acc2, acc2s, w2, c.lds + O_H2 + (c.f * S_H2 + 8 * c.h) * 2, P_H2, 32 * S_H2 * 2);
    add_acc<1, 2>(acc2, acc2s);
    W8S(10);
    if constexpr (TRUNK) {
      typedef unsigned u4_ __attribute__((ext_vector_type(4)));
      u4_* const dst = reinterpret_cast<u4_*>(a.h3ws) + (size_t)blockIdx.x * TrunkFrags::TILE_UNITS + c.lane;
#pragma unroll
      for (int fb = 0; fb < 2; ++fb) {
        h8 fr[2][2];
        frags_from_acc<ACT_RELU>(acc2[0][fb], c.hdr.inv_scale[ST_E2], fr);
#pragma unroll
        for (int p = 0; p < 2; ++p)
#pragma unroll
          for (int pc = 0; pc < 2; ++pc)
            dst[((fb * TrunkFrags::STEPS + 4 * jw + 2 * nbh + p) * PIECES + pc) * 64] = __builtin_bit_cast(u4_, fr[p][pc]);
      }
      return;
    }
    tail_pre_e3<false>(ct, acc3, wr3);
    __syncthreads();
    job_store<1, 2, ACT_RELU>(c, acc2, O_H3, P_H3, S_H3, 64 * jw + 32 * nbh, 0, c.hdr.inv_scale[ST_E2]);
  }
  __syncthreads();
  W8S(11);
  W8S_WALL(15);
  ct.helper = c.wv >= 4 ? 1 : 0;
  constexpr bool H1W8 = true;
#ifdef HX_STAMPS
  Args at = a;
  if (a.latent) at.latent = a.latent + (size_t)gridDim.x * 8 * 16 * 2;
  tail_stages<false, STRICT_INKERNEL_RESCUE_MAX, H1W8>(ct, at, row0, acc3, wr3);
#else
  tail_stages<false, STRICT_INKERNEL_RESCUE_MAX, H1W8>(ct, a, row0, acc3, wr3);
#endif
}

}

size_t tailws_workspace_bytes(int64_t B, int F) {
  if (B <= 0 || F <= 0) return 0;
  return hx::TrunkFrags::bytes(B);
}

int launch_encoder_heads_f16x2_tailws(const float* x, int64_t ldx, const float* raw, int normalize, int64_t B, int F,
                                      const void* blob, float* out, float* latent, uint8_t* valid, void* workspace,
                                      size_t ws_bytes, void* stream) {
  if (B == 0) return 0;
  if (!workspace || ws_bytes < tailws_workspace_bytes(B, F)) return fail(NLML_E_BADARG, "streamed-tail path: workspace too small");
  if (reinterpret_cast<uintptr_t>(workspace) & 15) return fail(NLML_E_BADARG, "streamed-tail path: workspace must be 16-byte aligned");
  const K2Input in = k2_input(x, ldx, raw, normalize, F);
  hx::Args a = k2_args<hx::Args>(in, B, F, blob, out, latent, valid);
  a.h3ws = workspace;
  if (!in.vec4) return fail(NLML_E_BADARG, "streamed-tail path: x must be 16-byte aligned with F and ldx multiples of 4");
  const int64_t ntiles = (B + TILE_FACES - 1) / TILE_FACES;
  const dim3 grid((unsigned)ntiles), block(512);
  hipStream_t st = reinterpret_cast<hipStream_t>(stream);
  if (a.norm) hipLaunchKernelGGL((hx::encoder_heads_f16x2_w8_kernel<true, true, true>), grid, block, 0, st, a);
  else hipLaunchKernelGGL((hx::encoder_heads_f16x2_w8_kernel<true, false, true>), grid, block, 0, st, a);
  if (int rc = hip_launch_status()) return rc;
  if (int rc = launch_tail_ws(blob, workspace, 2 * ntiles, B, out, latent, stream)) return rc;
  return launch_strict_reeval(x, ldx, raw, normalize, B, F, blob, out, latent, stream);
}

int launch_encoder_heads_f16x2_w8(const float* x, int64_t ldx, const float* raw, int normalize, int64_t B, int F,
                                  const void* blob, float* out, float* latent, uint8_t* valid, void* stream) {
  if (B == 0) return 0;
  const K2Input in = k2_input(x, ldx, raw, normalize, F);
  const hx::Args a = k2_args<hx::Args>(in, B, F, blob, out, latent, valid);
  const dim3 grid((unsigned)((B + TILE_FACES - 1) / TILE_FACES)), block(512);
  hipStream_t st = reinterpret_cast<hipStream_t>(stream);
  k2_with_variant(in, [&](auto V, auto N) {
    hipLaunchKernelGGL((hx::encoder_heads_f16x2_w8_kernel<decltype(V)::value, decltype(N)::value>), grid, block, 0, st, a);
  });
  if (int rc = hip_launch_status()) return rc;
  return launch_strict_reeval(x, ldx, raw, normalize, B, F, blob, out, latent, stream);
}

}
```

nlml_hpe_amd/csrc/torch_ops.cpp:

```cpp
#include <ATen/ATen.h>
#include <ATen/hip/impl/HIPGuardImplMasqueradingAsCUDA.h>
#include <ATen/hip/impl/HIPStreamMasqueradingAsCUDA.h>
#include <torch/library.h>

#include <string>
#include <tuple>
#include <vector>

#include "../../include/nlml_hpe.h"

namespace {

constexpr int64_t F_REF = NLML_F_REFERENCE;

void need(const at::Tensor& t, const char* name, at::ScalarType dt) {
  TORCH_CHECK(t.is_cuda(), name, ": expected a GPU tensor (there is no CPU fallback), got ", t.device());
  TORCH_CHECK(t.scalar_type() == dt, name, ": expected ", dt, ", got ", t.scalar_type());
}

void need_dense(const at::Tensor& t, const char* name) {
  TORCH_CHECK(t.is_contiguous(), name, ": expected a contiguous tensor (its data_ptr() and numel() go to the kernel as pointer and size)");
}

void same_device(const at::Tensor& a, const at::Tensor& b, const char* nb) {
  TORCH_CHECK(a.device() == b.device(), nb, " is on ", b.device(), " but the first operand is on ", a.device(),
              ": all operands must share one GPU");
}

void check(int rc, const char* what) {
  if (rc != 0) {
    const char* msg = nlml_last_error();
    TORCH_CHECK(false, what, " failed (code ", rc, "): ", msg ? msg : "");
  }
}

struct OnDevice {
  c10::hip::HIPGuardMasqueradingAsCUDA guard;
  void* stream;
  explicit OnDevice(const at::Tensor& t)
      : guard(t.device()), stream(c10::hip::getCurrentHIPStreamMasqueradingAsCUDA(t.device().index()).stream()) {}
};

int td_order(const std::string& order) {
  if (order == "reference") return NLML_TD_ORDER_REFERENCE;
  if (order == "fast") return NLML_TD_ORDER_FAST;
  TORCH_CHECK(false, "unknown TD order '", order, "'; expected 'fast' or 'reference'");
}

at::Tensor normalize_ipd(const at::Tensor& raw_, bool normalize) {
  need(raw_, "raw", at::kFloat);
  TORCH_CHECK(raw_.dim() == 3 && raw_.size(1) == 468 && raw_.size(2) == 3, "raw: expected [B,468,3], got ", raw_.sizes());
  const at::Tensor raw = raw_.contiguous();
  const int64_t B = raw.size(0);
  at::Tensor out = at::empty({B, F_REF}, raw.options());
  OnDevice dev(raw);
  check(nlml_normalize_ipd(raw.data_ptr<float>(), B, normalize ? 1 : 0, out.data_ptr<float>(), nullptr, dev.stream), "nlml_normalize_ipd");
  return out;
}

at::Tensor normalize_centroid(const at::Tensor& raw_) {
  need(raw_, "raw", at::kFloat);
  TORCH_CHECK(raw_.dim() == 3 && raw_.size(1) == 468 && raw_.size(2) == 3, "raw: expected [B,468,3], got ", raw_.sizes());
  const at::Tensor raw = raw_.contiguous();
  const int64_t B = raw.size(0);
  at::Tensor out = at::empty({B, F_REF}, raw.options());
  OnDevice dev(raw);
  check(nlml_normalize_centroid(raw.data_ptr<float>(), B, out.data_ptr<float>(), nullptr, nullptr, dev.stream), "nlml_normalize_centroid");
  return out;
}

std::tuple<at::Tensor, at::Tensor> compose_rotation_tensor(const at::Tensor& base_, const at::Tensor& ry_, const at::Tensor& rp_,
                                                           const at::Tensor& rr_, int64_t order, at::IntArrayRef zero_index, bool return_f64) {
  need(base_, "base", at::kFloat);
  TORCH_CHECK(base_.dim() == 3 && base_.size(1) == 468 && base_.size(2) == 3, "base: expected [I,468,3], got ", base_.sizes());
  const at::Tensor* const tabs[] = {&ry_, &rp_, &rr_};
  const char* const names[] = {"rot_yaw", "rot_pitch", "rot_roll"};
  for (int k = 0; k < 3; ++k) {
    need(*tabs[k], names[k], at::kDouble);
    same_device(base_, *tabs[k], names[k]);
    TORCH_CHECK(tabs[k]->dim() == 3 && tabs[k]->size(1) == 3 && tabs[k]->size(2) == 3, names[k], ": expected [n,3,3], got ", tabs[k]->sizes());
  }
  TORCH_CHECK(zero_index.size() == 3, "zero_index: expected 3 values (yaw, pitch, roll)");
  const at::Tensor base = base_.contiguous(), ry = ry_.contiguous(), rp = rp_.contiguous(), rr = rr_.contiguous();
  const int64_t I = base.size(0), ny = ry.size(0), np = rp.size(0), nr = rr.size(0);
  TORCH_CHECK(ny <= INT32_MAX && np <= INT32_MAX && nr <= INT32_MAX, "more than 2^31 - 1 bins on an axis");
  for (int k = 0; k < 3; ++k)
    TORCH_CHECK(zero_index[k] >= -1 && zero_index[k] < tabs[k]->size(0), "zero_index[", k, "] = ", zero_index[k], " is outside -1..n-1");
  at::Tensor out = at::empty({I, ny, np, nr, F_REF}, base.options());
  at::Tensor out64 = return_f64 ? at::empty({I, ny, np, nr, F_REF}, ry.options()) : at::empty({0}, ry.options());
  OnDevice dev(base);
  check(nlml_compose_rotation_tensor(base.data_ptr<float>(), I, ry.data_ptr<double>(), (int)ny, rp.data_ptr<double>(), (int)np,
                                     rr.data_ptr<double>(), (int)nr, (int)order, (int)zero_index[0], (int)zero_index[1], (int)zero_index[2],
                                     out.data_ptr<float>(), return_f64 ? out64.data_ptr<double>() : nullptr, dev.stream),
        "nlml_compose_rotation_tensor");
  return {out, out64};
}

std::tuple<at::Tensor, at::Tensor> rotate_landmarks(const at::Tensor& lm_, const at::Tensor& rot_, bool return_f32, bool return_f64) {
  need(lm_, "lm", at::kFloat);
  need(rot_, "rot", at::kDouble);
  same_device(lm_, rot_, "rot");
  TORCH_CHECK(lm_.dim() == 3 && lm_.size(1) == 468 && lm_.size(2) == 3, "lm: expected [B,468,3], got ", lm_.sizes());
  const int64_t B = lm_.size(0);
  TORCH_CHECK(rot_.dim() == 4 && rot_.size(0) == B && rot_.size(1) == 3 && rot_.size(2) == 3 && rot_.size(3) == 3, "rot: expected [", B,
              ",3,3,3], got ", rot_.sizes());
  TORCH_CHECK(return_f32 || return_f64, "rotate_landmarks: at least one of return_f32, return_f64");
  const at::Tensor lm = lm_.contiguous(), rot = rot_.contiguous();
  at::Tensor out = return_f32 ? at::empty({B, 468, 3}, lm.options()) : at::empty({0}, lm.options());
  at::Tensor out64 = return_f64 ? at::empty({B, 468, 3}, rot.options()) : at::empty({0}, rot.options());
  OnDevice dev(lm);
  check(nlml_rotate_landmarks(lm.data_ptr<float>(), rot.data_ptr<double>(), return_f32 ? out.data_ptr<float>() : nullptr,
                              return_f64 ? out64.data_ptr<double>() : nullptr, B, dev.stream), "nlml_rotate_landmarks");
  return {out, out64};
}

struct K2Out { at::Tensor pose, valid; };
K2Out k2_forward(const at::Tensor& in_, bool landmarks, const at::Tensor& blob, int64_t F, bool normalize, const at::Tensor* ws,
                 bool want_valid) {
  need(in_, landmarks ? "raw" : "x", at::kFloat);
  need(blob, "packed_w", at::kByte);
  need_dense(blob, "packed_w");
  if (ws) {
    need(*ws, "workspace", at::kByte);
    need_dense(*ws, "workspace");
  }
  same_device(in_, blob, "packed_w");
  if (ws) same_device(in_, *ws, "workspace");
  if (landmarks) {
    TORCH_CHECK(in_.dim() == 3 && in_.size(1) == 468 && in_.size(2) == 3, "raw: expected [B,468,3], got ", in_.sizes());
  } else {
    TORCH_CHECK(in_.dim() == 2 && in_.size(1) == F, "x: expected [B,", F, "], got ", in_.sizes());
  }
  const at::Tensor in = !landmarks && in_.stride(1) == 1 ? in_ : in_.contiguous();
  const int64_t B = in.size(0);
  K2Out r{at::empty({B, 3}, in.options()), want_valid ? at::empty({B}, in.options().dtype(at::kByte)) : at::Tensor()};
  uint8_t* const valid = want_valid ? r.valid.data_ptr<uint8_t>() : nullptr;
  float* const out = r.pose.data_ptr<float>();
  const size_t blob_bytes = (size_t)blob.numel();
  OnDevice dev(in);
  if (landmarks) {
    const int norm = normalize ? 1 : 0;
    if (ws)
      check(nlml_landmarks_to_pose_small(in.data_ptr<float>(), B, norm, blob.data_ptr(), blob_bytes, out, nullptr, valid, ws->data_ptr(),
                                         (size_t)ws->numel(), dev.stream), "nlml_landmarks_to_pose_small");
    else
      check(nlml_landmarks_to_pose(in.data_ptr<float>(), B, norm, blob.data_ptr(), blob_bytes, out, nullptr, valid, dev.stream),
            "nlml_landmarks_to_pose");
  } else {
    const int64_t ldx = B > 1 ? in.stride(0) : F;
    if (ws)
      check(nlml_encoder_heads_fwd_small(in.data_ptr<float>(), ldx, B, (int)F, blob.data_ptr(), blob_bytes, out, nullptr, valid,
                                         ws->data_ptr(), (size_t)ws->numel(), dev.stream), "nlml_encoder_heads_fwd_small");
    else
      check(nlml_encoder_heads_fwd(in.data_ptr<float>(), ldx, B, (int)F, blob.data_ptr(), blob_bytes, out, nullptr, valid, dev.stream),
            "nlml_encoder_heads_fwd");
  }
  return r;
}

at::Tensor encoder_heads_fwd(const at::Tensor& x, const at::Tensor& blob, int64_t F) {
  return k2_forward(x, false, blob, F, false, nullptr, false).pose;
}
at::Tensor landmarks_to_pose(const at::Tensor& raw, const at::Tensor& blob, bool normalize) {
  return k2_forward(raw, true, blob, F_REF, normalize, nullptr, false).pose;
}
at::Tensor encoder_heads_fwd_small(const at::Tensor& x, const at::Tensor& blob, int64_t F, const at::Tensor& ws) {
  return k2_forward(x, false, blob, F, false, &ws, false).pose;
}
at::Tensor landmarks_to_pose_small(const at::Tensor& raw, const at::Tensor& blob, bool normalize, const at::Tensor& ws) {
  return k2_forward(raw, true, blob, F_REF, normalize, &ws, false).pose;
}
std::tuple<at::Tensor, at::Tensor> landmarks_to_pose_valid(const at::Tensor& raw, const at::Tensor& blob, bool normalize,
                                                           const std::optional<at::Tensor>& ws) {
  K2Out r = k2_forward(raw, true, blob, F_REF, normalize, ws.has_value() ? &*ws : nullptr, true);
  return {r.pose, r.valid};
}

int check_td(const at::Tensor& Wm, const at::Tensor& x, const at::Tensor& cosp, const at::Tensor* params = nullptr) {
  need(Wm, "Wm", at::kFloat);
  need(x, "x", at::kFloat);
  need(cosp, "cos_params", at::kDouble);
  same_device(x, Wm, "Wm");
  same_device(x, cosp, "cos_params");
  TORCH_CHECK(Wm.dim() == 2 && Wm.size(1) == F_REF && Wm.size(0) % 27 == 0 && Wm.size(0) >= 27 * NLML_TUCKER_RANK_MIN &&
                  Wm.size(0) <= 27 * NLML_TUCKER_RANK_MAX,
              "Wm: expected [27*R,1404] for an identity rank R in [", NLML_TUCKER_RANK_MIN, ", ", NLML_TUCKER_RANK_MAX, "], got ", Wm.sizes());
  TORCH_CHECK(x.dim() == 2 && x.size(1) == F_REF, "x: expected [N,1404], got ", x.sizes());
  TORCH_CHECK(cosp.dim() == 3 && cosp.size(0) == 3 && cosp.size(1) == 3 && cosp.size(2) == 4, "cos_params: expected [3,3,4], got ", cosp.sizes());
  const int r_id = (int)(Wm.size(0) / 27);
  if (params) {
    need(*params, "params", at::kDouble);
    same_device(x, *params, "params");
    TORCH_CHECK(params->dim() == 2 && params->size(1) == 3 + r_id, "params: expected [N,", 3 + r_id, "], got ", params->sizes());
    TORCH_CHECK(x.size(0) == params->size(0), "x has ", x.size(0), " rows but params has ", params->size(0));
  }
  return r_id;
}

at::Tensor tucker_objective(const at::Tensor& Wm_, const at::Tensor& x_, const at::Tensor& params_, const at::Tensor& cosp_,
                            std::string order) {
  const int r_id = check_td(Wm_, x_, cosp_, &params_);
  const at::Tensor Wm = Wm_.contiguous(), x = x_.contiguous(), params = params_.contiguous(), cosp = cosp_.contiguous();
  const int64_t N = params.size(0);
  at::Tensor err = at::empty({N}, params.options());
  OnDevice dev(x);
  check(nlml_tucker_objective_r(Wm.data_ptr<float>(), x.data_ptr<float>(), F_REF, nullptr, params.data_ptr<double>(),
                                cosp.data_ptr<double>(), N, err.data_ptr<double>(), nullptr, r_id, td_order(order), dev.stream),
        "nlml_tucker_objective_r");
  return err;
}

std::tuple<at::Tensor, at::Tensor> tucker_gradient(const at::Tensor& Wm_, const at::Tensor& x_, const at::Tensor& params_,
                                                   const at::Tensor& cosp_) {
  const int r_id = check_td(Wm_, x_, cosp_, &params_);
  const at::Tensor Wm = Wm_.contiguous(), x = x_.contiguous(), params = params_.contiguous(), cosp = cosp_.contiguous();
  const int64_t N = params.size(0);
  at::Tensor err = at::empty({N}, params.options()), grad = at::empty({N, 3 + r_id}, params.options());
  const size_t ws_bytes = nlml_tucker_gradient_workspace_bytes(N, r_id);
  at::Tensor ws = at::empty({(int64_t)(ws_bytes / sizeof(double))}, params.options());
  OnDevice dev(x);
  check(nlml_tucker_gradient_r(Wm.data_ptr<float>(), x.data_ptr<float>(), F_REF, nullptr, params.data_ptr<double>(),
                               cosp.data_ptr<double>(), N, err.data_ptr<double>(), grad.data_ptr<double>(), r_id, ws.data_ptr(), ws_bytes,
                               dev.stream),
        "nlml_tucker_gradient_r");
  return {err, grad};
}

std::tuple<at::Tensor, at::Tensor, at::Tensor, at::Tensor, at::Tensor> tucker_powell(const at::Tensor& Wm_, const at::Tensor& x_,
                                                                                      const at::Tensor& cosp_, std::string order) {
  const int r_id = check_td(Wm_, x_, cosp_);
  const at::Tensor Wm = Wm_.contiguous(), x = x_.contiguous(), cosp = cosp_.contiguous();
  const int64_t N = x.size(0);
  const auto f64 = x.options().dtype(at::kDouble), i32 = x.options().dtype(at::kInt);
  at::Tensor res = at::empty({N, 3 + r_id}, f64), fun = at::empty({N}, f64), nfev = at::empty({N}, i32), nit = at::empty({N}, i32),
             status = at::empty({N}, i32);
  OnDevice dev(x);
  check(nlml_tucker_powell_r(Wm.data_ptr<float>(), x.data_ptr<float>(), F_REF, cosp.data_ptr<double>(), N, nullptr,
                             res.data_ptr<double>(), fun.data_ptr<double>(), nfev.data_ptr<int32_t>(), nit.data_ptr<int32_t>(),
                             status.data_ptr<int32_t>(), r_id, td_order(order), dev.stream), "nlml_tucker_powell_r");
  return {res, fun, nfev, nit, status};
}

void video_post(const at::Tensor& pose_, const at::Tensor& raw_, const std::optional<at::Tensor>& valid_, double frame_w, double frame_h,
                double alpha, double max_jump, double size, at::Tensor state, at::Tensor sm, at::Tensor centre, at::Tensor ep,
                at::Tensor upd) {
  need(pose_, "pose_rad", at::kFloat);
  need(raw_, "raw", at::kFloat);
  need(state, "state", at::kDouble);
  need(sm, "smoothed", at::kDouble);
  need(centre, "centre", at::kDouble);
  need(ep, "endpoints", at::kDouble);
  need(upd, "updated", at::kByte);
  const at::Tensor* const others[] = {&raw_, &state, &sm, &centre, &ep, &upd};
  for (const at::Tensor* t : others) same_device(pose_, *t, "video_post operand");
  const int64_t S = pose_.size(0);
  TORCH_CHECK(pose_.dim() == 2 && pose_.size(1) == 3, "pose_rad: expected [S,3], got ", pose_.sizes());
  TORCH_CHECK(raw_.dim() == 3 && raw_.size(0) == S && raw_.size(1) == 468 && raw_.size(2) == 3, "raw: expected [S,468,3], got ", raw_.sizes());
  TORCH_CHECK(state.is_contiguous() && state.numel() == S * 6 && sm.is_contiguous() && sm.numel() == S * 3 && centre.is_contiguous() &&
                  centre.numel() == S * 2 && ep.is_contiguous() && ep.numel() == S * 6 && upd.is_contiguous() && upd.numel() == S,
              "video_post: state [S,6], smoothed [S,3], centre [S,2], endpoints [S,3,2], updated [S], all contiguous");
  const at::Tensor pose = pose_.contiguous(), raw = raw_.contiguous();
  at::Tensor valid;
  if (valid_.has_value()) {
    need(*valid_, "valid", at::kByte);
    same_device(pose_, *valid_, "valid");
    TORCH_CHECK(valid_->dim() == 1 && valid_->size(0) == S, "valid: expected [S]");
    valid = valid_->contiguous();
  }
  OnDevice dev(pose);
  check(nlml_video_post_ex(pose.data_ptr<float>(), raw.data_ptr<float>(), valid.defined() ? valid.data_ptr<uint8_t>() : nullptr, S,
                           frame_w, frame_h, alpha, max_jump, size, state.data_ptr<double>(), sm.data_ptr<double>(),
                           centre.data_ptr<double>(), ep.data_ptr<double>(), upd.data_ptr<uint8_t>(), dev.stream), "nlml_video_post_ex");
}

at::Tensor cosine_table(const at::Tensor& angles_, const at::Tensor& cosp_) {
  need(angles_, "angles_rad", at::kFloat);
  need(cosp_, "cos_params", at::kDouble);
  same_device(angles_, cosp_, "cos_params");
  TORCH_CHECK(angles_.dim() == 1 && cosp_.dim() == 2 && cosp_.size(1) == 4, "expected angles [n] and cos_params [R,4]");
  const at::Tensor angles = angles_.contiguous(), cosp = cosp_.contiguous();
  at::Tensor out = at::empty({angles.size(0), cosp.size(0)}, cosp.options());
  OnDevice dev(angles);
  check(nlml_cosine_table(angles.data_ptr<float>(), angles.size(0), cosp.data_ptr<double>(), (int)cosp.size(0), out.data_ptr<double>(),
                          dev.stream), "nlml_cosine_table");
  return out;
}

std::tuple<at::Tensor, at::Tensor> pose_eval(const at::Tensor& pose_, const std::optional<at::Tensor>& valid_, const at::Tensor& gt_,
                                             at::ArrayRef<double> lo, at::ArrayRef<double> hi, int64_t decimals,
                                             at::ArrayRef<double> intervals, at::ArrayRef<int64_t> axes) {
  TORCH_CHECK(pose_.is_cuda(), "pose: expected a GPU tensor (there is no CPU fallback), got ", pose_.device());
  TORCH_CHECK(pose_.scalar_type() == at::kFloat || pose_.scalar_type() == at::kDouble, "pose: expected float32 radians or float64 degrees");
  need(gt_, "gt", at::kDouble);
  same_device(pose_, gt_, "gt");
  const int64_t B = pose_.size(0);
  TORCH_CHECK(pose_.dim() == 2 && pose_.size(1) == 3 && gt_.dim() == 2 && gt_.size(0) == B && gt_.size(1) == 3,
              "pose and gt: expected [B,3] each, got ", pose_.sizes(), " and ", gt_.sizes());
  TORCH_CHECK(lo.size() == 3 && hi.size() == 3, "lo / hi: expected 3 values each");
  const int64_t K = (int64_t)axes.size();
  TORCH_CHECK((int64_t)intervals.size() == 2 * K, "intervals: expected 2 values per axis entry");
  TORCH_CHECK(K <= NLML_POSE_EVAL_MAX_INTERVALS, "at most ", NLML_POSE_EVAL_MAX_INTERVALS, " intervals");
  std::vector<int32_t> ax(axes.begin(), axes.end());
  const at::Tensor pose = pose_.contiguous(), gt = gt_.contiguous();
  at::Tensor valid;
  if (valid_.has_value()) {
    TORCH_CHECK(valid_->scalar_type() == at::kBool || valid_->scalar_type() == at::kByte, "valid: expected bool or uint8");
    same_device(pose_, *valid_, "valid");
    TORCH_CHECK(valid_->dim() == 1 && valid_->size(0) == B, "valid: expected [B]");
    valid = valid_->contiguous();
  }
  const auto f64 = gt.options();
  at::Tensor ws = at::empty({std::max<int64_t>(1, (int64_t)nlml_pose_eval_workspace_bytes(B, (int)K) / 8)}, f64);
  at::Tensor record = at::empty({12 + 2 * K}, f64), result = at::empty({14 + 2 * K}, f64);
  const bool f32 = pose.scalar_type() == at::kFloat;
  OnDevice dev(pose);
  check(nlml_pose_eval(f32 ? pose.data_ptr<float>() : nullptr, f32 ? nullptr : pose.data_ptr<double>(),
                       valid.defined() ? static_cast<const uint8_t*>(valid.data_ptr()) : nullptr, gt.data_ptr<double>(), B, lo.data(),
                       hi.data(), (int)decimals, intervals.data(), ax.data(), (int)K, ws.data_ptr(), (size_t)ws.numel() * 8,
                       record.data_ptr<double>(), result.data_ptr<double>(), nullptr, nullptr, dev.stream), "nlml_pose_eval");
  return {record, result};
}

std::tuple<at::Tensor, at::Tensor> pose_eval_merge(const at::Tensor& records_, int64_t K) {
  need(records_, "records", at::kDouble);
  TORCH_CHECK(K >= 0 && K <= NLML_POSE_EVAL_MAX_INTERVALS, "K: at most ", NLML_POSE_EVAL_MAX_INTERVALS, " intervals");
  TORCH_CHECK(records_.dim() == 2 && records_.size(1) == 12 + 2 * K, "records: expected [n,", 12 + 2 * K, "], got ", records_.sizes());
  const at::Tensor records = records_.contiguous();
  at::Tensor record = at::empty({12 + 2 * K}, records.options()), result = at::empty({14 + 2 * K}, records.options());
  OnDevice dev(records);
  check(nlml_pose_eval_merge(records.data_ptr<double>(), records.size(0), (int)K, record.data_ptr<double>(), result.data_ptr<double>(),
                             dev.stream), "nlml_pose_eval_merge");
  return {record, result};
}

at::Tensor normalize_ipd_meta(const at::Tensor& raw, bool) { return at::empty({raw.size(0), F_REF}, raw.options()); }
at::Tensor normalize_centroid_meta(const at::Tensor& raw) { return at::empty({raw.size(0), F_REF}, raw.options()); }
std::tuple<at::Tensor, at::Tensor> compose_rotation_tensor_meta(const at::Tensor& base, const at::Tensor& ry, const at::Tensor& rp,
                                                                const at::Tensor& rr, int64_t, at::IntArrayRef, bool return_f64) {
  const std::vector<int64_t> shape = {base.size(0), ry.size(0), rp.size(0), rr.size(0), F_REF};
  return {at::empty(shape, base.options()), return_f64 ? at::empty(shape, ry.options()) : at::empty({0}, ry.options())};
}
std::tuple<at::Tensor, at::Tensor> rotate_landmarks_meta(const at::Tensor& lm, const at::Tensor& rot, bool return_f32, bool return_f64) {
  return {return_f32 ? at::empty({lm.size(0), 468, 3}, lm.options()) : at::empty({0}, lm.options()),
          return_f64 ? at::empty({lm.size(0), 468, 3}, rot.options()) : at::empty({0}, rot.options())};
}
template <class... Rest> at::Tensor pose_meta(const at::Tensor& x, const at::Tensor&, Rest...) { return at::empty({x.size(0), 3}, x.options()); }
at::Tensor tucker_objective_meta(const at::Tensor&, const at::Tensor&, const at::Tensor& params, const at::Tensor&, std::string) {
  return at::empty({params.size(0)}, params.options());
}
std::tuple<at::Tensor, at::Tensor> tucker_gradient_meta(const at::Tensor&, const at::Tensor&, const at::Tensor& params, const at::Tensor&) {
  return {at::empty({params.size(0)}, params.options()), at::empty({params.size(0), params.size(1)}, params.options())};
}
std::tuple<at::Tensor, at::Tensor> pose_valid_meta(const at::Tensor& raw, const at::Tensor&, bool, const std::optional<at::Tensor>&) {
  return {at::empty({raw.size(0), 3}, raw.options()), at::empty({raw.size(0)}, raw.options().dtype(at::kByte))};
}
std::tuple<at::Tensor, at::Tensor, at::Tensor, at::Tensor, at::Tensor> tucker_powell_meta(const at::Tensor& Wm, const at::Tensor& x, const at::Tensor&,
                                                                                           std::string) {
  const int64_t N = x.size(0), n_par = 3 + Wm.size(0) / 27;
  const auto f64 = x.options().dtype(at::kDouble), i32 = x.options().dtype(at::kInt);
  return {at::empty({N, n_par}, f64), at::empty({N}, f64), at::empty({N}, i32), at::empty({N}, i32), at::empty({N}, i32)};
}
void video_post_meta(const at::Tensor&, const at::Tensor&, const std::optional<at::Tensor>&, double, double, double, double, double, at::Tensor,
                     at::Tensor, at::Tensor, at::Tensor, at::Tensor) {}
at::Tensor cosine_table_meta(const at::Tensor& angles, const at::Tensor& cosp) { return at::empty({angles.size(0), cosp.size(0)}, cosp.options()); }

std::tuple<at::Tensor, at::Tensor> pose_eval_meta(const at::Tensor& pose, const std::optional<at::Tensor>&, const at::Tensor& gt,
                                                  at::ArrayRef<double>, at::ArrayRef<double>, int64_t, at::ArrayRef<double>,
                                                  at::ArrayRef<int64_t> axes) {
  const int64_t K = (int64_t)axes.size();
  return {at::empty({12 + 2 * K}, gt.options()), at::empty({14 + 2 * K}, gt.options())};
}
std::tuple<at::Tensor, at::Tensor> pose_eval_merge_meta(const at::Tensor& records, int64_t K) {
  return {at::empty({12 + 2 * K}, records.options()), at::empty({14 + 2 * K}, records.options())};
}

}

TORCH_LIBRARY(nlml_hpe, m) {
  m.def("normalize_ipd(Tensor raw, bool normalize) -> Tensor");
  m.def("normalize_centroid(Tensor raw) -> Tensor");
  m.def("compose_rotation_tensor(Tensor base, Tensor rot_yaw, Tensor rot_pitch, Tensor rot_roll, int order, int[] zero_index, "
        "bool return_f64=False) -> (Tensor, Tensor)");
  m.def("rotate_landmarks(Tensor lm, Tensor rot, bool return_f32=True, bool return_f64=False) -> (Tensor, Tensor)");
  m.def("encoder_heads_fwd(Tensor x, Tensor packed_w, int F) -> Tensor");
  m.def("landmarks_to_pose(Tensor raw, Tensor packed_w, bool normalize) -> Tensor");
  m.def("encoder_heads_fwd_small(Tensor x, Tensor packed_w, int F, Tensor workspace) -> Tensor");
  m.def("landmarks_to_pose_small(Tensor raw, Tensor packed_w, bool normalize, Tensor workspace) -> Tensor");
  m.def("landmarks_to_pose_valid(Tensor raw, Tensor packed_w, bool normalize, Tensor? workspace) -> (Tensor, Tensor)");
  m.def("tucker_objective(Tensor Wm, Tensor x, Tensor params, Tensor cos_params, str order=\"reference\") -> Tensor");
  m.def("tucker_gradient(Tensor Wm, Tensor x, Tensor params, Tensor cos_params) -> (Tensor, Tensor)");
  m.def("tucker_powell(Tensor Wm, Tensor x, Tensor cos_params, str order=\"reference\") -> (Tensor, Tensor, Tensor, Tensor, Tensor)");
  m.def("video_post(Tensor pose_rad, Tensor raw, Tensor? valid, float frame_w, float frame_h, float alpha, float max_jump, float size, "
        "Tensor(a!) state, Tensor(b!) smoothed, Tensor(c!) centre, Tensor(d!) endpoints, Tensor(e!) updated) -> ()");
  m.def("cosine_table(Tensor angles_rad, Tensor cos_params) -> Tensor");
  m.def("pose_eval(Tensor pose, Tensor? valid, Tensor gt, float[] lo, float[] hi, int decimals, float[] intervals, int[] axes) "
        "-> (Tensor, Tensor)");
  m.def("pose_eval_merge(Tensor records, int K) -> (Tensor, Tensor)");
}

TORCH_LIBRARY_IMPL(nlml_hpe, CUDA, m) {
  m.impl("normalize_ipd", &normalize_ipd);
  m.impl("normalize_centroid", &normalize_centroid);
  m.impl("compose_rotation_tensor", &compose_rotation_tensor);
  m.impl("rotate_landmarks", &rotate_landmarks);
  m.impl("encoder_heads_fwd", &encoder_heads_fwd);
  m.impl("landmarks_to_pose", &landmarks_to_pose);
  m.impl("encoder_heads_fwd_small", &encoder_heads_fwd_small);
  m.impl("landmarks_to_pose_small", &landmarks_to_pose_small);
  m.impl("landmarks_to_pose_valid", &landmarks_to_pose_valid);
  m.impl("tucker_objective", &tucker_objective);
  m.impl("tucker_gradient", &tucker_gradient);
  m.impl("tucker_powell", &tucker_powell);
  m.impl("video_post", &video_post);
  m.impl("cosine_table", &cosine_table);
  m.impl("pose_eval", &pose_eval);
  m.impl("pose_eval_merge", &pose_eval_merge);
}

TORCH_LIBRARY_IMPL(nlml_hpe, Meta, m) {
  m.impl("normalize_ipd", &normalize_ipd_meta);
  m.impl("normalize_centroid", &normalize_centroid_meta);
  m.impl("compose_rotation_tensor", &compose_rotation_tensor_meta);
  m.impl("rotate_landmarks", &rotate_landmarks_meta);
  m.impl("encoder_heads_fwd", &pose_meta<int64_t>);
  m.impl("landmarks_to_pose", &pose_meta<bool>);
  m.impl("encoder_heads_fwd_small", &pose_meta<int64_t, const at::Tensor&>);
  m.impl("landmarks_to_pose_small", &pose_meta<bool, const at::Tensor&>);
  m.impl("tucker_objective", &tucker_objective_meta);
  m.impl("landmarks_to_pose_valid", &pose_valid_meta);
  m.impl("tucker_gradient", &tucker_gradient_meta);
  m.impl("tucker_powell", &tucker_powell_meta);
  m.impl("video_post", &video_post_meta);
  m.impl("cosine_table", &cosine_table_meta);
  m.impl("pose_eval", &pose_eval_meta);
  m.impl("pose_eval_merge", &pose_eval_merge_meta);
}
```

nlml_hpe_amd/ops.py:

```python
from __future__ import annotations

import torch

from . import _lib

F_REF = 1404
LATENT = 9


def _stream_ptr(device=None) -> int:
    return torch.cuda.current_stream(device).cuda_stream


def _need_cuda(t: torch.Tensor, name: str, dtype) -> None:
    if not t.is_cuda:
        raise _lib.NlmlError(f"{name}: expected a GPU tensor (there is no CPU fallback), got device {t.device}")
    if t.dtype != dtype:
        raise TypeError(f"{name}: expected {dtype}, got {t.dtype}")


class _on_device_of:

    def __init__(self, *named):
        ts = [(n, t) for n, t in named if t is not None]
        self.device = ts[0][1].device
        for n, t in ts[1:]:
            if t.device != self.device:
                raise _lib.NlmlError(f"{n} is on {t.device} but {ts[0][0]} is on {self.device}: all operands must share one GPU")
        self.guard = torch.cuda.device(self.device)

    def __enter__(self) -> int:
        self.guard.__enter__()
        return _stream_ptr(self.device)

    def __exit__(self, *exc):
        return self.guard.__exit__(*exc)


def _raw_rows(raw: torch.Tensor) -> torch.Tensor:
    if raw.dim() != 3 or raw.shape[1:] != (468, 3):
        raise ValueError(f"raw: expected [B,468,3], got {tuple(raw.shape)}")
    return raw.contiguous()


def normalize_ipd(raw: torch.Tensor, normalize: bool = True, return_valid: bool = False):
    _need_cuda(raw, "raw", torch.float32)
    raw = _raw_rows(raw)
    B = raw.shape[0]
    out = torch.empty((B, F_REF), dtype=torch.float32, device=raw.device)
    valid = torch.empty((B,), dtype=torch.uint8, device=raw.device) if return_valid else None
    with _on_device_of(("raw", raw)) as stream:
        _lib.check(_lib.lib().nlml_normalize_ipd(raw.data_ptr(), B, int(bool(normalize)), out.data_ptr(),
                                                 valid.data_ptr() if valid is not None else None, stream),
                   "nlml_normalize_ipd")
    return (out, valid.bool()) if return_valid else out


def normalize_centroid(raw: torch.Tensor, return_valid: bool = False, return_stats: bool = False):
    _need_cuda(raw, "raw", torch.float32)
    raw = _raw_rows(raw)
    B = raw.shape[0]
    out = torch.empty((B, F_REF), dtype=torch.float32, device=raw.device)
    valid = torch.empty((B,), dtype=torch.uint8, device=raw.device) if return_valid else None
    stats = torch.empty((B, 4), dtype=torch.float64, device=raw.device) if return_stats else None
    with _on_device_of(("raw", raw)) as stream:
        _lib.check(_lib.lib().nlml_normalize_centroid(raw.data_ptr(), B, out.data_ptr(),
                                                      valid.data_ptr() if valid is not None else None,
                                                      stats.data_ptr() if stats is not None else None, stream),
                   "nlml_normalize_centroid")
    res = [out]
    if return_valid:
        res.append(valid.bool())
    if return_stats:
        res.append(stats)
    return res[0] if len(res) == 1 else tuple(res)


def _rot_table(t: torch.Tensor, name: str) -> torch.Tensor:
    _need_cuda(t, name, torch.float64)
    if t.dim() != 3 or t.shape[1:] != (3, 3):
        raise ValueError(f"{name}: expected [n,3,3], got {tuple(t.shape)}")
    return t.contiguous()


def compose_rotation_tensor(base: torch.Tensor, rot_yaw: torch.Tensor, rot_pitch: torch.Tensor, rot_roll: torch.Tensor,
                            order="intrinsic", zero_index=None, return_f64: bool = False):
    _need_cuda(base, "base", torch.float32)
    if base.dim() != 3 or base.shape[1:] != (468, 3):
        raise ValueError(f"base: expected [I,468,3], got {tuple(base.shape)}")
    base = base.contiguous()
    rot_yaw, rot_pitch, rot_roll = _rot_table(rot_yaw, "rot_yaw"), _rot_table(rot_pitch, "rot_pitch"), _rot_table(rot_roll, "rot_roll")
    order = _lib.rot_order_from_name(order)
    zero = [-1, -1, -1] if zero_index is None else [int(z) for z in zero_index]
    I, ny, np_, nr = base.shape[0], rot_yaw.shape[0], rot_pitch.shape[0], rot_roll.shape[0]
    if len(zero) != 3 or any(not -1 <= z < n for z, n in zip(zero, (ny, np_, nr))):
        raise ValueError(f"zero_index: expected (yaw, pitch, roll) indices in -1..n-1 for {ny} x {np_} x {nr} bins, got {zero_index!r}")
    out = torch.empty((I, ny, np_, nr, F_REF), dtype=torch.float32, device=base.device)
    out64 = torch.empty((I, ny, np_, nr, F_REF), dtype=torch.float64, device=base.device) if return_f64 else None
    with _on_device_of(("base", base), ("rot_yaw", rot_yaw), ("rot_pitch", rot_pitch), ("rot_roll", rot_roll)) as stream:
        _lib.check(_lib.lib().nlml_compose_rotation_tensor(
            base.data_ptr(), I, rot_yaw.data_ptr(), ny, rot_pitch.data_ptr(), np_, rot_roll.data_ptr(), nr, order, *zero, out.data_ptr(),
            out64.data_ptr() if return_f64 else None, stream), "nlml_compose_rotation_tensor")
    return (out, out64) if return_f64 else out


def rotate_landmarks(lm: torch.Tensor, rot: torch.Tensor, return_f64: bool = False, return_f32: bool = True):
    _need_cuda(lm, "lm", torch.float32)
    _need_cuda(rot, "rot", torch.float64)
    lm = _raw_rows(lm)
    B = lm.shape[0]
    if tuple(rot.shape) != (B, 3, 3, 3):
        raise ValueError(f"rot: expected [{B},3,3,3], got {tuple(rot.shape)}")
    if not (return_f32 or return_f64):
        raise ValueError("rotate_landmarks: at least one of return_f32, return_f64")
    rot = rot.contiguous()
    out = torch.empty((B, 468, 3), dtype=torch.float32, device=lm.device) if return_f32 else None
    out64 = torch.empty((B, 468, 3), dtype=torch.float64, device=lm.device) if return_f64 else None
    with _on_device_of(("lm", lm), ("rot", rot)) as stream:
        _lib.check(_lib.lib().nlml_rotate_landmarks(lm.data_ptr(), rot.data_ptr(), out.data_ptr() if return_f32 else None,
                                                    out64.data_ptr() if return_f64 else None, B, stream), "nlml_rotate_landmarks")
    if return_f32 and return_f64:
        return out, out64
    return out if return_f32 else out64


_k2_ws: dict = {}


def _k2_workspace(form: str, B: int, F: int, device, floor_faces: int = 0) -> torch.Tensor:
    size_of = _lib.lib().nlml_encoder_heads_small_workspace_bytes if form == "small" else _lib.lib().nlml_encoder_heads_workspace_bytes
    need = max(16, size_of(B, F))
    pool = _k2_ws.setdefault((form, str(device), _stream_ptr(device)), [])
    for ws in pool:
        if ws.numel() >= need:
            return ws
    ws = torch.empty((max(need, size_of(floor_faces, F_REF)),), dtype=torch.uint8, device=device)
    pool.append(ws)
    return ws


def _small_workspace(B: int, F: int, device) -> torch.Tensor:
    return _k2_workspace("small", B, F, device, floor_faces=4096)


def _k2_forward(form: str, x, raw, blob: torch.Tensor, F: int, normalize, return_latent: bool, return_valid: bool, workspace=None):
    if raw is None:
        _need_cuda(x, "x", torch.float32)
        _need_cuda(blob, "blob", torch.uint8)
        if x.dim() != 2 or x.shape[1] != F:
            raise ValueError(f"x: expected [B,{F}], got {tuple(x.shape)}")
        if x.stride(1) != 1:
            x = x.contiguous()
        src, name, symbol = x, "x", "nlml_encoder_heads_fwd"
        B = x.shape[0]
        head = (x.data_ptr(), x.stride(0) if B > 1 else F, B, F)
    else:
        _need_cuda(raw, "raw", torch.float32)
        _need_cuda(blob, "blob", torch.uint8)
        src, name, symbol = _raw_rows(raw), "raw", "nlml_landmarks_to_pose"
        B = src.shape[0]
        head = (src.data_ptr(), B, int(bool(normalize)))
    dev = src.device
    tail = ()
    if form:
        symbol += "_" + form
        if workspace is None:
            workspace = _small_workspace(B, F, dev) if form == "small" else _k2_workspace(form, B, F, dev)
        tail = (workspace.data_ptr(), workspace.numel())
    out = torch.empty((B, 3), dtype=torch.float32, device=dev)
    latent = torch.empty((B, LATENT), dtype=torch.float32, device=dev) if return_latent else None
    valid = torch.empty((B,), dtype=torch.uint8, device=dev) if return_valid else None
    with _on_device_of((name, src), ("blob", blob), ("workspace", workspace)) as stream:
        _lib.check(getattr(_lib.lib(), symbol)(
            *head, blob.data_ptr(), blob.numel(), out.data_ptr(),
            latent.data_ptr() if latent is not None else None,
            valid.data_ptr() if valid is not None else None, *tail, stream), symbol)
    res = [out]
    if return_latent:
        res.append(latent)
    if return_valid:
        res.append(valid.bool())
    return res[0] if len(res) == 1 else tuple(res)


def encoder_heads_fwd(x: torch.Tensor, blob: torch.Tensor, F: int, return_latent: bool = False,
                      return_valid: bool = False):
    return _k2_forward("", x, None, blob, F, None, return_latent, return_valid)


def encoder_heads_fwd_debug(x: torch.Tensor, blob: torch.Tensor, F: int, want_stamps: bool = False):
    _need_cuda(x, "x", torch.float32)
    _need_cuda(blob, "blob", torch.uint8)
    if x.dim() != 2 or x.shape[1] != F:
        raise ValueError(f"x: expected [B,{F}], got {tuple(x.shape)}")
    x = x.contiguous()
    B = x.shape[0]
    out = torch.empty((B, 3), dtype=torch.float32, device=x.device)
    latent = torch.empty((B, LATENT), dtype=torch.float32, device=x.device)
    pre = torch.empty((B, 64), dtype=torch.float32, device=x.device)
    stamps = torch.zeros(((B + 63) // 64, 4, 16), dtype=torch.int64, device=x.device) if want_stamps else None
    with _on_device_of(("x", x), ("blob", blob)) as stream:
        _lib.check(_lib.lib().nlml_encoder_heads_fwd_debug(x.data_ptr(), F, B, F, blob.data_ptr(), blob.numel(),
                                                           out.data_ptr(), latent.data_ptr(), pre.data_ptr(),
                                                           stamps.data_ptr() if want_stamps else None, stream),
                   "nlml_encoder_heads_fwd_debug")
    return (out, latent, pre, stamps) if want_stamps else (out, latent, pre)


def landmarks_to_pose(raw: torch.Tensor, blob: torch.Tensor, normalize: bool = True, return_latent: bool = False,
                      return_valid: bool = False):
    return _k2_forward("", None, raw, blob, F_REF, normalize, return_latent, return_valid)


def _td_operands(Wm, x, cos_params, params=None, x_index=None, x0=None):
    _need_cuda(Wm, "Wm", torch.float32)
    _need_cuda(x, "x", torch.float32)
    if params is not None:
        _need_cuda(params, "params", torch.float64)
    _need_cuda(cos_params, "cos_params", torch.float64)
    if Wm.dim() != 2 or Wm.shape[1] != F_REF:
        raise ValueError(f"Wm: expected [27*R,1404], got {tuple(Wm.shape)}")
    r_id = _lib.tucker_rank_of_rows(Wm.shape[0])
    if x.dim() != 2 or x.shape[1] != F_REF:
        raise ValueError(f"x: expected [{'N' if params is None else 'M'},1404], got {tuple(x.shape)}")
    if params is not None and (params.dim() != 2 or params.shape[1] != 3 + r_id):
        raise ValueError(f"params: expected [N,{3 + r_id}] for Wm of identity rank {r_id}, got {tuple(params.shape)}")
    if tuple(cos_params.shape) != (3, 3, 4):
        raise ValueError(f"cos_params: expected [3,3,4], got {tuple(cos_params.shape)}")
    Wm, x, cos_params = Wm.contiguous(), x.contiguous(), cos_params.contiguous()
    if params is None:
        N = x.shape[0]
        if x0 is not None:
            _need_cuda(x0, "x0", torch.float64)
            if tuple(x0.shape) != (N, 3 + r_id):
                raise ValueError(f"x0: expected [{N},{3 + r_id}], got {tuple(x0.shape)}")
            x0 = x0.contiguous()
        return Wm, x, cos_params, None, None, x0, r_id, N
    params = params.contiguous()
    N = params.shape[0]
    if x_index is not None:
        _need_cuda(x_index, "x_index", torch.int32)
        if x_index.shape != (N,):
            raise ValueError("x_index: expected [N]")
        x_index = x_index.contiguous()
        if N and (int(x_index.min()) < 0 or int(x_index.max()) >= x.shape[0]):
            raise IndexError("x_index out of range")
    elif x.shape[0] != N:
        raise ValueError(f"x has {x.shape[0]} rows but params has {N} (pass x_index to share rows)")
    return Wm, x, cos_params, params, x_index, None, r_id, N


def tucker_objective(Wm: torch.Tensor, x: torch.Tensor, params: torch.Tensor, cos_params: torch.Tensor,
                     x_index: torch.Tensor | None = None, return_xhat: bool = False, order="reference"):
    order = _lib.td_order_from_name(order)
    Wm, x, cos_params, params, x_index, _, r_id, N = _td_operands(Wm, x, cos_params, params, x_index)
    err = torch.empty((N,), dtype=torch.float64, device=x.device)
    xh = torch.empty((N, F_REF), dtype=torch.float64, device=x.device) if return_xhat else None
    with _on_device_of(("x", x), ("Wm", Wm), ("params", params), ("cos_params", cos_params), ("x_index", x_index)) as stream:
        _lib.check(_lib.lib().nlml_tucker_objective_r(
            Wm.data_ptr(), x.data_ptr(), F_REF, x_index.data_ptr() if x_index is not None else None,
            params.data_ptr(), cos_params.data_ptr(), N, err.data_ptr(),
            xh.data_ptr() if xh is not None else None, r_id, order, stream), "nlml_tucker_objective_r")
    return (err, xh) if return_xhat else err


def tucker_gradient(Wm: torch.Tensor, x: torch.Tensor, params: torch.Tensor, cos_params: torch.Tensor,
                    x_index: torch.Tensor | None = None, return_err: bool = True):
    Wm, x, cos_params, params, x_index, _, r_id, N = _td_operands(Wm, x, cos_params, params, x_index)
    err = torch.empty((N,), dtype=torch.float64, device=x.device) if return_err else None
    grad = torch.empty((N, 3 + r_id), dtype=torch.float64, device=x.device)
    ws_bytes = _lib.lib().nlml_tucker_gradient_workspace_bytes(N, r_id)
    ws = torch.empty((ws_bytes // 8,), dtype=torch.float64, device=x.device)
    with _on_device_of(("x", x), ("Wm", Wm), ("params", params), ("cos_params", cos_params), ("x_index", x_index)) as stream:
        _lib.check(_lib.lib().nlml_tucker_gradient_r(
            Wm.data_ptr(), x.data_ptr(), F_REF, x_index.data_ptr() if x_index is not None else None,
            params.data_ptr(), cos_params.data_ptr(), N, err.data_ptr() if err is not None else None, grad.data_ptr(), r_id,
            ws.data_ptr(), ws_bytes, stream), "nlml_tucker_gradient_r")
    return (err, grad) if return_err else grad


import os as _os

TORCH_OPS_PATH = _os.path.join(_os.path.dirname(_os.path.abspath(__file__)), "libnlml_torch_ops.so")


def _load_torch_ops():
    if not _os.path.exists(TORCH_OPS_PATH):
        raise _lib.NlmlError(f"{TORCH_OPS_PATH} is missing: build it with `python -c 'import __graft_entry__ as g; g.build()'` "
                             "(make -C nlml_hpe_amd/csrc); torch.ops.nlml_hpe.* are registered from it")
    _lib.lib()
    torch.ops.load_library(TORCH_OPS_PATH)
    for name in ("normalize_ipd", "normalize_centroid", "encoder_heads_fwd", "landmarks_to_pose", "encoder_heads_fwd_small", "landmarks_to_pose_small",
                 "landmarks_to_pose_valid", "tucker_objective", "tucker_gradient", "tucker_powell", "video_post", "cosine_table", "pose_eval",
                 "pose_eval_merge", "compose_rotation_tensor", "rotate_landmarks"):
        getattr(torch.ops.nlml_hpe, name)


_load_torch_ops()


def tucker_powell(Wm: torch.Tensor, x: torch.Tensor, cos_params: torch.Tensor, x0: torch.Tensor | None = None, order="reference"):
    Wm, x, cos_params, _, _, x0, r_id, N = _td_operands(Wm, x, cos_params, x0=x0)
    n_par = 3 + r_id
    order = _lib.td_order_from_name(order)
    dev = x.device
    res = torch.empty((N, n_par), dtype=torch.float64, device=dev)
    fun = torch.empty((N,), dtype=torch.float64, device=dev)
    nfev = torch.empty((N,), dtype=torch.int32, device=dev)
    nit = torch.empty((N,), dtype=torch.int32, device=dev)
    status = torch.empty((N,), dtype=torch.int32, device=dev)
    with _on_device_of(("x", x), ("Wm", Wm), ("cos_params", cos_params), ("x0", x0)) as stream:
        _lib.check(_lib.lib().nlml_tucker_powell_r(Wm.data_ptr(), x.data_ptr(), F_REF, cos_params.data_ptr(), N,
                                                   x0.data_ptr() if x0 is not None else None, res.data_ptr(), fun.data_ptr(),
                                                   nfev.data_ptr(), nit.data_ptr(), status.data_ptr(), r_id, order, stream),
                   "nlml_tucker_powell_r")
    return {"x": res, "fun": fun, "nfev": nfev, "nit": nit, "status": status}


def cosine_table(angles_rad: torch.Tensor, cos_params: torch.Tensor) -> torch.Tensor:
    _need_cuda(angles_rad, "angles_rad", torch.float32)
    _need_cuda(cos_params, "cos_params", torch.float64)
    if angles_rad.dim() != 1 or cos_params.dim() != 2 or cos_params.shape[1] != 4:
        raise ValueError(f"expected angles [n] and cos_params [R,4], got {tuple(angles_rad.shape)}, {tuple(cos_params.shape)}")
    angles_rad, cos_params = angles_rad.contiguous(), cos_params.contiguous()
    n, R = angles_rad.shape[0], cos_params.shape[0]
    out = torch.empty((n, R), dtype=torch.float64, device=angles_rad.device)
    with _on_device_of(("angles_rad", angles_rad), ("cos_params", cos_params)) as stream:
        _lib.check(_lib.lib().nlml_cosine_table(angles_rad.data_ptr(), n, cos_params.data_ptr(), R, out.data_ptr(), stream),
                   "nlml_cosine_table")
    return out


def mode5_product(core: torch.Tensor, U_feat: torch.Tensor) -> torch.Tensor:
    _need_cuda(core, "core", torch.float32)
    _need_cuda(U_feat, "U_feat", torch.float32)
    if U_feat.dim() != 2 or core.dim() < 1 or core.shape[-1] != U_feat.shape[1]:
        raise ValueError(f"core [..., R5] and U_feat [M, R5] disagree: {tuple(core.shape)}, {tuple(U_feat.shape)}")
    lead = tuple(core.shape[:-1])
    c2 = core.contiguous().reshape(-1, core.shape[-1])
    U_feat = U_feat.contiguous()
    Q, R5, M = c2.shape[0], c2.shape[1], U_feat.shape[0]
    W = torch.empty((Q, M), dtype=torch.float32, device=core.device)
    with _on_device_of(("core", core), ("U_feat", U_feat)) as stream:
        _lib.check(_lib.lib().nlml_mode5_product(c2.data_ptr(), U_feat.data_ptr(), Q, R5, M, W.data_ptr(), stream),
                   "nlml_mode5_product")
    return W.reshape(lead + (M,))


def encoder_heads_fwd_small(x: torch.Tensor, blob: torch.Tensor, F: int, return_latent: bool = False,
                            return_valid: bool = False, workspace: torch.Tensor | None = None):
    return _k2_forward("small", x, None, blob, F, None, return_latent, return_valid, workspace)


def landmarks_to_pose_small(raw: torch.Tensor, blob: torch.Tensor, normalize: bool = True, return_latent: bool = False,
                            return_valid: bool = False, workspace: torch.Tensor | None = None):
    return _k2_forward("small", None, raw, blob, F_REF, normalize, return_latent, return_valid, workspace)


def landmarks_to_pose_streamed(raw: torch.Tensor, blob: torch.Tensor, normalize: bool = True, return_latent: bool = False,
                               return_valid: bool = False, workspace: torch.Tensor | None = None):
    return _k2_forward("streamed", None, raw, blob, F_REF, normalize, return_latent, return_valid, workspace)


_eval_ws: dict = {}


def _eval_workspace(B: int, K: int, device) -> torch.Tensor:
    need = max(8, _lib.lib().nlml_pose_eval_workspace_bytes(B, K))
    key = (str(device), _stream_ptr(device))
    ws = _eval_ws.get(key)
    if ws is None or ws.numel() * 8 < need:
        ws = torch.empty(((need + 7) // 8,), dtype=torch.float64, device=device)
        _eval_ws[key] = ws
    return ws


def _eval_intervals(intervals):
    import ctypes as C
    iv = [(int(a), float(lo), float(hi)) for a, lo, hi in intervals]
    K = len(iv)
    h_iv = (C.c_double * max(1, 2 * K))(*[v for _, lo, hi in iv for v in (lo, hi)])
    h_ax = (C.c_int32 * max(1, K))(*[a for a, _, _ in iv])
    return h_iv, h_ax, K


def pose_eval(pose: torch.Tensor, gt: torch.Tensor, valid: torch.Tensor | None = None, lo=None, hi=None, intervals=(), decimals: int = 3,
              return_per_face: bool = False, workspace: torch.Tensor | None = None):
    if not pose.is_cuda:
        raise _lib.NlmlError(f"pose: expected a GPU tensor (there is no CPU fallback), got device {pose.device}")
    if pose.dtype not in (torch.float32, torch.float64):
        raise TypeError(f"pose: expected float32 radians or float64 degrees, got {pose.dtype}")
    _need_cuda(gt, "gt", torch.float64)
    B = pose.shape[0]
    if pose.dim() != 2 or pose.shape[1] != 3 or tuple(gt.shape) != (B, 3):
        raise ValueError(f"pose and gt: expected [B,3] each, got {tuple(pose.shape)}, {tuple(gt.shape)}")
    if valid is not None:
        if not valid.is_cuda or valid.dtype not in (torch.bool, torch.uint8) or tuple(valid.shape) != (B,):
            raise ValueError(f"valid: expected a GPU bool/uint8 tensor [{B}], got {valid.dtype} {tuple(valid.shape)} on {valid.device}")
        valid = valid.contiguous()
        valid = valid.view(torch.uint8) if valid.dtype == torch.bool else valid
    pose, gt = pose.contiguous(), gt.contiguous()
    import ctypes as C
    h_lo = (C.c_double * 3)(*([-float("inf")] * 3 if lo is None else [float(v) for v in lo]))
    h_hi = (C.c_double * 3)(*([float("inf")] * 3 if hi is None else [float(v) for v in hi]))
    h_iv, h_ax, K = _eval_intervals(intervals)
    L = _lib.lib()
    dev = pose.device
    ws = workspace if workspace is not None else _eval_workspace(B, K, dev)
    record = torch.empty((L.nlml_pose_eval_record_len(K) or 1,), dtype=torch.float64, device=dev)
    result = torch.empty((L.nlml_pose_eval_result_len(K) or 1,), dtype=torch.float64, device=dev)
    pred = torch.empty((B, 3), dtype=torch.float64, device=dev) if return_per_face else None
    keep = torch.empty((B,), dtype=torch.uint8, device=dev) if return_per_face else None
    f32 = pose.dtype == torch.float32
    with _on_device_of(("pose", pose), ("gt", gt), ("valid", valid), ("workspace", ws)) as stream:
        _lib.check(L.nlml_pose_eval(pose.data_ptr() if f32 else None, None if f32 else pose.data_ptr(),
                                    valid.data_ptr() if valid is not None else None, gt.data_ptr(), B, h_lo, h_hi, int(decimals),
                                    h_iv, h_ax, K, ws.data_ptr(), ws.numel() * ws.element_size(), record.data_ptr(), result.data_ptr(),
                                    pred.data_ptr() if pred is not None else None, keep.data_ptr() if keep is not None else None, stream),
                   "nlml_pose_eval")
    if return_per_face:
        return record, result, pred, keep.bool()
    return record, result


def pose_eval_merge(records: torch.Tensor, K: int):
    _need_cuda(records, "records", torch.float64)
    Lr = _lib.lib().nlml_pose_eval_record_len(int(K))
    if Lr == 0:
        raise ValueError(f"K = {K}: at most {_lib.POSE_EVAL_MAX_INTERVALS} intervals")
    if records.dim() != 2 or records.shape[1] != Lr:
        raise ValueError(f"records: expected [n,{Lr}], got {tuple(records.shape)}")
    records = records.contiguous()
    dev = records.device
    record = torch.empty((Lr,), dtype=torch.float64, device=dev)
    result = torch.empty((_lib.lib().nlml_pose_eval_result_len(int(K)),), dtype=torch.float64, device=dev)
    with _on_device_of(("records", records)) as stream:
        _lib.check(_lib.lib().nlml_pose_eval_merge(records.data_ptr(), records.shape[0], int(K), record.data_ptr(), result.data_ptr(),
                                                   stream), "nlml_pose_eval_merge")
    return record, result
```

Measured before the change: 75.29 million.

## Add quad-tile fused kernel path splitting batch across CUs with trunk workspace

Adds a new "quad" forward path for F16X2S blobs. Each 512-thread workgroup processes four tiles (256 faces): the trunk writes intermediate fragments to a workspace, and the tail/head stages, now moved into a shared device header, reuse them. The batch is split so the quad part is a whole multiple of workgroups per CU, and the remainder runs through the existing fused w8 kernel. Auto dispatch, the torch ops and the Python wrapper now allocate the workspace and choose this path by default for large aligned batches. The cost is extra workspace memory traffic and a second kernel launch for the remainder.

```diff
diff --git a/include/nlml_hpe.h b/include/nlml_hpe.h
--- a/include/nlml_hpe.h
+++ b/include/nlml_hpe.h
@@ -78,6 +78,15 @@
                                     const void* blob, size_t blob_bytes, float* out, float* latent, uint8_t* valid,
                                     void* workspace, size_t ws_bytes, void* stream);
 
+int nlml_encoder_heads_fwd_quad(const float* x, int64_t ldx, int64_t B, int F,
+                                const void* blob, size_t blob_bytes, float* out, float* latent, uint8_t* valid,
+                                void* workspace, size_t ws_bytes, void* stream);
+int nlml_landmarks_to_pose_quad(const float* raw, int64_t B, int normalize,
+                                const void* blob, size_t blob_bytes, float* out, float* latent, uint8_t* valid,
+                                void* workspace, size_t ws_bytes, void* stream);
+int nlml_k2_quad_split(int64_t B, int cus, int64_t* quad_faces);
+int nlml_k2_quad_faces(int64_t B, int64_t* quad_faces, size_t* ws_bytes);
+
 size_t nlml_encoder_heads_workspace_bytes(int64_t B, int F);
 int nlml_encoder_heads_fwd_ws(const float* x, int64_t ldx, int64_t B, int F,
                               const void* blob, size_t blob_bytes, float* out, float* latent, uint8_t* valid,
diff --git a/nlml_hpe_amd/_lib.py b/nlml_hpe_amd/_lib.py
--- a/nlml_hpe_amd/_lib.py
+++ b/nlml_hpe_amd/_lib.py
@@ -14,7 +14,7 @@
 
 
 def _k2_forwards():
-    for form, ws in (("", []), ("_small", _FWD_WS), ("_streamed", _FWD_WS), ("_ws", _FWD_WS)):
+    for form, ws in (("", []), ("_small", _FWD_WS), ("_streamed", _FWD_WS), ("_quad", _FWD_WS), ("_ws", _FWD_WS)):
         yield "nlml_encoder_heads_fwd" + form, (C.c_int, _FWD_X + _FWD_OUT + ws + [C.c_void_p])
         yield "nlml_landmarks_to_pose" + form, (C.c_int, _FWD_RAW + _FWD_OUT + ws + [C.c_void_p])
 
@@ -52,6 +52,8 @@
                                                C.c_void_p, C.c_void_p, C.c_void_p, C.c_void_p, C.c_void_p]),
     "nlml_encoder_heads_small_workspace_bytes": (C.c_size_t, [C.c_int64, C.c_int]),
     "nlml_encoder_heads_workspace_bytes": (C.c_size_t, [C.c_int64, C.c_int]),
+    "nlml_k2_quad_split": (C.c_int, [C.c_int64, C.c_int, C.POINTER(C.c_int64)]),
+    "nlml_k2_quad_faces": (C.c_int, [C.c_int64, C.POINTER(C.c_int64), C.POINTER(C.c_size_t)]),
     "nlml_tucker_gradient_workspace_bytes": (C.c_size_t, [C.c_int64, C.c_int]),
     "nlml_video_post": (C.c_int, [C.c_void_p, C.c_void_p, C.c_void_p, C.c_int64, C.c_double, C.c_double, C.c_double,
                                   C.c_double, C.c_double, C.c_void_p, C.c_void_p, C.c_void_p, C.c_void_p, C.c_void_p]),
diff --git a/nlml_hpe_amd/csrc/abi.cpp b/nlml_hpe_amd/csrc/abi.cpp
--- a/nlml_hpe_amd/csrc/abi.cpp
+++ b/nlml_hpe_amd/csrc/abi.cpp
@@ -21,6 +21,10 @@
 int hip_launch_status() {
   const hipError_t e = hipGetLastError();
   return e == hipSuccess ? 0 : fail((int)e, hipGetErrorString(e));
+}
+int64_t k2_quad_faces(int64_t B, int cus) {
+  if (B <= 0 || cus <= 0) return 0;
+  return (B / TILE_FACES) / (4 * (int64_t)cus) * cus * (4 * TILE_FACES);
 }
 }
 
@@ -160,7 +164,39 @@
   return v;
 }
 
-enum K2Form { K2_FUSED, K2_SMALL, K2_STREAMED, K2_AUTO };
+static int64_t env_i64(const char* name, int64_t unset) {
+  const char* e = getenv(name);
+  return e && e[0] ? (int64_t)atoll(e) : unset;
+}
+static const int64_t kQuadMinUnset = INT64_MIN;
+static int64_t quad_min() {
+  static const int64_t v = env_i64("NLML_K2_QUAD_MIN", kQuadMinUnset);
+  return v;
+}
+static int device_cus() {
+  static const int64_t forced = env_i64("NLML_K2_QUAD_CUS", 0);
+  if (forced > 0) return (int)forced;
+  constexpr int kMaxDev = 64;
+  static int cus[kMaxDev];
+  int dev = 0;
+  if (hipGetDevice(&dev) != hipSuccess || dev < 0 || dev >= kMaxDev) return 0;
+  if (cus[dev] == 0) {
+    int n = 0;
+    if (hipDeviceGetAttribute(&n, hipDeviceAttributeMultiprocessorCount, dev) != hipSuccess || n <= 0) n = -1;
+    cus[dev] = n;
+  }
+  return cus[dev] > 0 ? cus[dev] : 0;
+}
+
+
+static int64_t auto_quad_faces(int64_t B) {
+  if (B <= 0) return 0;
+  if (B > kSmallMax && streamed_min() >= 0 && B >= streamed_min()) return 0;
+  if (quad_min() != kQuadMinUnset) return quad_min() >= 0 && B >= quad_min() ? B : 0;
+  return B > kSmallMax ? k2_quad_faces(B, device_cus()) : 0;
+}
+
+enum K2Form { K2_FUSED, K2_SMALL, K2_STREAMED, K2_QUAD, K2_AUTO };
 
 static int k2_forward(K2Form form, bool landmarks, const float* x, int64_t ldx, const float* raw, int normalize, int64_t B, int F,
                       const void* blob, size_t blob_bytes, float* out, float* latent, uint8_t* valid, void* workspace, size_t ws_bytes,
@@ -173,17 +209,25 @@
   if (int rc = check_blob_args(B, F, blob, blob_bytes, out, &mode)) return rc;
   if (form == K2_SMALL && !split_f16(mode)) return fail(NLML_E_BADARG, "small-batch path: NLML_MODE_F16X2 / NLML_MODE_F16X2S blob only");
   if (form == K2_STREAMED && mode != NLML_MODE_F16X2S) return fail(NLML_E_BADARG, "streamed-tail path: NLML_MODE_F16X2S blob only");
+  if (form == K2_QUAD && mode != NLML_MODE_F16X2S) return fail(NLML_E_BADARG, "quad path: NLML_MODE_F16X2S blob only");
   if (no_input) return fail(NLML_E_BADARG, no_input);
   const int split = mode == NLML_MODE_F16X2S;
+  int64_t quad_faces = B;
   if (form == K2_AUTO) {
-    if (split_f16(mode) && B <= kSmallMax) form = K2_SMALL;
-    else if (split && streamed_min() >= 0 && B >= streamed_min() && k2_input(x, ldx, raw, normalize, F).vec4) form = K2_STREAMED;
+    const bool wide = split && k2_input(x, ldx, raw, normalize, F).vec4;
+    quad_faces = wide ? auto_quad_faces(B) : 0;
+    const bool fits = workspace && ws_bytes >= quad_workspace_bytes(quad_faces) && !(reinterpret_cast<uintptr_t>(workspace) & 15);
+    if (quad_faces > 0 && (fits || quad_min() != kQuadMinUnset)) form = K2_QUAD;
+    else if (split_f16(mode) && B <= kSmallMax) form = K2_SMALL;
+    else if (wide && streamed_min() >= 0 && B >= streamed_min()) form = K2_STREAMED;
     else form = K2_FUSED;
   }
   if (form == K2_SMALL)
     return launch_encoder_heads_f16x2_small(x, ldx, raw, normalize, B, F, blob, out, latent, valid, workspace, ws_bytes, split, stream);
   if (form == K2_STREAMED)
     return launch_encoder_heads_f16x2_tailws(x, ldx, raw, normalize, B, F, blob, out, latent, valid, workspace, ws_bytes, stream);
+  if (form == K2_QUAD)
+    return launch_encoder_heads_f16x2_w8_mixed(x, ldx, raw, normalize, B, F, blob, out, latent, valid, quad_faces, workspace, ws_bytes, stream);
   if (mode == NLML_MODE_BF16) return launch_encoder_heads_bf16(x, ldx, raw, normalize, B, F, blob, out, latent, valid, stream);
   if (split_f16(mode)) return launch_encoder_heads_f16x2(x, ldx, raw, normalize, B, F, blob, out, latent, valid, split, stream);
   return launch_encoder_heads_f32(x, ldx, raw, normalize, B, F, blob, out, latent, valid, nullptr, nullptr, stream);
@@ -228,6 +272,34 @@
 int nlml_landmarks_to_pose_streamed(const float* raw, int64_t B, int normalize, const void* blob, size_t blob_bytes,
                                     float* out, float* latent, uint8_t* valid, void* workspace, size_t ws_bytes, void* stream) {
   return k2_forward(K2_STREAMED, true, nullptr, 0, raw, normalize, B, NLML_F_REFERENCE, blob, blob_bytes, out, latent, valid, workspace, ws_bytes, stream);
+}
+
+int nlml_encoder_heads_fwd_quad(const float* x, int64_t ldx, int64_t B, int F, const void* blob, size_t blob_bytes,
+                                float* out, float* latent, uint8_t* valid, void* workspace, size_t ws_bytes, void* stream) {
+  return k2_forward(K2_QUAD, false, x, ldx, nullptr, 0, B, F, blob, blob_bytes, out, latent, valid, workspace, ws_bytes, stream);
+}
+
+int nlml_landmarks_to_pose_quad(const float* raw, int64_t B, int normalize, const void* blob, size_t blob_bytes,
+                                float* out, float* latent, uint8_t* valid, void* workspace, size_t ws_bytes, void* stream) {
+  return k2_forward(K2_QUAD, true, nullptr, 0, raw, normalize, B, NLML_F_REFERENCE, blob, blob_bytes, out, latent, valid, workspace, ws_bytes, stream);
+}
+
+int nlml_k2_quad_split(int64_t B, int cus, int64_t* quad_faces) {
+  if (!quad_faces) return fail(NLML_E_BADARG, "k2_quad_split: null quad_faces");
+  *quad_faces = 0;
+  if (B < 0 || cus <= 0) return fail(NLML_E_BADARG, "k2_quad_split: negative B or cus <= 0");
+  *quad_faces = k2_quad_faces(B, cus);
+  return 0;
+}
+
+int nlml_k2_quad_faces(int64_t B, int64_t* quad_faces, size_t* ws_bytes) {
+  if (quad_faces) *quad_faces = 0;
+  if (ws_bytes) *ws_bytes = 0;
+  if (!quad_faces) return fail(NLML_E_BADARG, "k2_quad_faces: null quad_faces");
+  if (B < 0) return fail(NLML_E_BADARG, "k2_quad_faces: negative B");
+  *quad_faces = auto_quad_faces(B);
+  if (ws_bytes) *ws_bytes = quad_workspace_bytes(*quad_faces);
+  return 0;
 }
 
 size_t nlml_encoder_heads_workspace_bytes(int64_t B, int F) {
diff --git a/nlml_hpe_amd/csrc/abi_internal.h b/nlml_hpe_amd/csrc/abi_internal.h
--- a/nlml_hpe_amd/csrc/abi_internal.h
+++ b/nlml_hpe_amd/csrc/abi_internal.h
@@ -62,6 +62,11 @@
 int launch_encoder_heads_f16x2_tailws(const float* x, int64_t ldx, const float* raw, int normalize, int64_t B, int F,
                                       const void* blob, float* out, float* latent, uint8_t* valid, void* workspace,
                                       size_t ws_bytes, void* stream);
+size_t quad_workspace_bytes(int64_t quad_faces);
+int launch_encoder_heads_f16x2_w8_mixed(const float* x, int64_t ldx, const float* raw, int normalize, int64_t B, int F,
+                                        const void* blob, float* out, float* latent, uint8_t* valid, int64_t quad_faces,
+                                        void* workspace, size_t ws_bytes, void* stream);
+int64_t k2_quad_faces(int64_t B, int cus);
 int launch_tail_ws(const void* blob, const void* h3, int64_t nfb, int64_t B, float* out, float* latent, void* stream);
 size_t small_workspace_bytes(int64_t B, int F);
 int launch_encoder_heads_f16x2_small(const float* x, int64_t ldx, const float* raw, int normalize, int64_t B, int F,
diff --git a/nlml_hpe_amd/csrc/encoder_heads_f16x2_tailws.hip b/nlml_hpe_amd/csrc/encoder_heads_f16x2_tailws.hip
--- a/nlml_hpe_amd/csrc/encoder_heads_f16x2_tailws.hip
+++ b/nlml_hpe_amd/csrc/encoder_heads_f16x2_tailws.hip
@@ -2,361 +2,14 @@
 
 #include "../../include/nlml_hpe.h"
 #include "abi_internal.h"
-#include "encoder_heads_f16x2_dev.h"
-#include "layout.h"
-
-#if defined(__HIP_DEVICE_COMPILE__) && !defined(__gfx950__)
-#error "global_load_lds_dwordx4: gfx950"
-#endif
+#include "encoder_heads_f16x2_tailws_dev.h"
 
 namespace nlml {
 namespace hx {
 
-typedef unsigned u4 __attribute__((ext_vector_type(4)));
-#define TW_PRIO(p) __builtin_amdgcn_s_setprio(p)
-typedef __attribute__((address_space(3))) const char LdsC;
-typedef __attribute__((address_space(3))) char LdsW;
-
-struct TwArgs {
-  const void* blob;
-  const u4* h3;
-  float* out;
-  float* latent;
-  int64_t B, nfb;
-};
-
-constexpr int TW_SLOT = 65536;
-constexpr int tw_bias_n16(int s) { return kStages[s].jobs * kStages[s].nb * 8; }
-constexpr int tw_bias_off(int s) {
-  int o = 0;
-  for (int t = ST_E3; t < s; ++t) o += tw_bias_n16(t) * 16;
-  return o;
-}
-constexpr uint32_t tw_b_off(int s, uint32_t k16_e0) {
-  int c = (int)(sizeof(Header) / 16), m = 0;
-  for (int t = 0; t < s; ++t) {
-    c += kStages[t].jobs * ((t == ST_E0 ? 0 : kStages[t].k8 * kStages[t].nb * 64 * PIECES) + kStages[t].nb * 8);
-    m += kStages[t].jobs * (t == ST_E0 ? kStages[t].nb * 64 * PIECES : 0);
-  }
-  return c + m * k16_e0 + kStages[s].jobs * ((s == ST_E0 ? 0 : kStages[s].k8 * kStages[s].nb * 64 * PIECES) + (s == ST_E0 ? kStages[s].nb * 64 * PIECES : 0) * k16_e0);
-}
-constexpr bool tw_b_off_is_layouts() {
-  for (int s = 0; s < NUM_STAGES; ++s)
-    if (tw_b_off(s, 0u) != layout_b_off(kLayoutHX, s, 0u) || tw_b_off(s, 88u) != layout_b_off(kLayoutHX, s, 88u)) return false;
-  return true;
-}
-static_assert(tw_b_off_is_layouts(), "the written-out bias offsets are layout.h's");
-constexpr int TW_O_BIAS = 2 * TW_SLOT;
-constexpr int TW_O_LAT = TW_O_BIAS + ((tw_bias_off(NUM_STAGES) + 511) / 512) * 512;
-constexpr int TW_LAT_WAVE = 3 * 2 * 256;
-constexpr int TW_LDS = TW_O_LAT + 8 * TW_LAT_WAVE;
-static_assert(TW_LDS <= 163840, "LDS map");
-
-constexpr int TW_HEAD_UNITS = 9, TW_UNITS = 4 + 3 * TW_HEAD_UNITS;
-constexpr uint32_t tw_job_w16(int s) { return layout_job_w16(kLayoutHX, s, 0u); }
-__device__ __forceinline__ void tw_unit(const HdrRegs& H, int idx, uint32_t& off, uint32_t& n16) {
-  constexpr uint32_t J3 = tw_job_w16(ST_E3), J4 = tw_job_w16(ST_E4), J5 = tw_job_w16(ST_E5);
-  constexpr uint32_t K0 = tw_job_w16(ST_H0), K1 = tw_job_w16(ST_H1), K2 = tw_job_w16(ST_H2), K3 = tw_job_w16(ST_H3), K4 = tw_job_w16(ST_H4);
-  static_assert(2 * J3 * 16 == TW_SLOT && 2 * J4 * 16 <= TW_SLOT && J5 * 16 <= TW_SLOT && 4 * K0 * 16 <= TW_SLOT && K1 * 16 <= TW_SLOT &&
-                    2 * K2 * 16 == TW_SLOT && 2 * K3 * 16 <= TW_SLOT && K4 * 16 <= TW_SLOT,
-                "a unit fits a buffer");
-  if (idx < 2) { n16 = 2 * J3; off = H.w_off(ST_E3) + idx * 2 * J3; }
-  else if (idx == 2) { n16 = 2 * J4; off = H.w_off(ST_E4); }
-  else if (idx == 3) { n16 = J5; off = H.w_off(ST_E5); }
-  else {
-    const int k = idx - 4, g = k / TW_HEAD_UNITS, r = k - TW_HEAD_UNITS * g;
-    if (r == 0) { n16 = 4 * K0; off = H.w_off(ST_H0) + 4 * g * K0; }
-    else if (r <= 4) { n16 = K1; off = H.w_off(ST_H1) + (4 * g + (r - 1)) * K1; }
-    else if (r <= 6) { n16 = 2 * K2; off = H.w_off(ST_H2) + (4 * g + 2 * (r - 5)) * K2; }
-    else if (r == 7) { n16 = 2 * K3; off = H.w_off(ST_H3) + 2 * g * K3; }
-    else { n16 = K4; off = H.w_off(ST_H4) + g * K4; }
-  }
-}
-
-template <int K16, int NCH = 2>
-__device__ __forceinline__ void tw_job2(f32x16 (&acc)[2], LdsC* w0, LdsC* w1, int wstep, LdsC* b0, LdsC* b1, const h8 (&in)[K16][2]) {
-  typedef const __attribute__((address_space(3))) h8 LdsH8;
-#pragma unroll
-  for (int c = 0; c < NCH; ++c)
-#pragma unroll
-    for (int q = 0; q < 4; ++q) {
-      const f32x4 v = *reinterpret_cast<const __attribute__((address_space(3))) f32x4*>((c ? b1 : b0) + q * 16);
-      acc[c][4 * q + 0] = v[0];
-      acc[c][4 * q + 1] = v[1];
-      acc[c][4 * q + 2] = v[2];
-      acc[c][4 * q + 3] = v[3];
-    }
-  TW_PRIO(2);
-#pragma unroll
-  for (int ks = 0; ks < K16; ++ks) {
-    h8 wf[NCH][2];
-#pragma unroll
-    for (int c = 0; c < NCH; ++c)
-#pragma unroll
-      for (int p = 0; p < 2; ++p) wf[c][p] = *reinterpret_cast<LdsH8*>((c ? w1 : w0) + ks * wstep + p * 1024);
-#pragma unroll
-    for (int t = 0; t < 3; ++t)
-#pragma unroll
-      for (int c = 0; c < NCH; ++c)
-        acc[c] = __builtin_amdgcn_mfma_f32_32x32x16_f16(wf[c][t == 0 ? 1 : 0], in[ks][t == 1 ? 1 : 0], acc[c], 0, 0, 0);
-  }
-  TW_PRIO(0);
-}
-
-template <int K16>
-__device__ __forceinline__ void tw_job2p(f32x16 (&acc)[2], LdsC* w0, LdsC* w1, int wstep, LdsC* b0, LdsC* b1, const h8 (&in)[K16][2]) {
-  typedef const __attribute__((address_space(3))) h8 LdsH8;
-#pragma unroll
-  for (int c = 0; c < 2; ++c)
-#pragma unroll
-    for (int q = 0; q < 4; ++q) {
-      const f32x4 v = *reinterpret_cast<const __attribute__((address_space(3))) f32x4*>((c ? b1 : b0) + q * 16);
-      acc[c][4 * q + 0] = v[0];
-      acc[c][4 * q + 1] = v[1];
-      acc[c][4 * q + 2] = v[2];
-      acc[c][4 * q + 3] = v[3];
-    }
-  h8 wf[2][2][2];
-#pragma unroll
-  for (int c = 0; c < 2; ++c)
-#pragma unroll
-    for (int p = 0; p < 2; ++p) wf[0][c][p] = *reinterpret_cast<LdsH8*>((c ? w1 : w0) + p * 1024);
-  TW_PRIO(2);
-  __builtin_amdgcn_sched_barrier(0);
-#pragma unroll
-  for (int ks = 0; ks < K16; ++ks) {
-#pragma unroll
-    for (int m = 0; m < 6; ++m) {
-      const int t = m >> 1, c = m & 1;
-      acc[c] = __builtin_amdgcn_mfma_f32_32x32x16_f16(wf[ks & 1][c][t == 0 ? 1 : 0], in[ks][t == 1 ? 1 : 0], acc[c], 0, 0, 0);
-      __builtin_amdgcn_sched_barrier(0);
-      if (m < 4 && ks + 1 < K16)
-        wf[(ks + 1) & 1][m & 1][m < 2 ? 1 : 0] = *reinterpret_cast<LdsH8*>(((m & 1) ? w1 : w0) + (ks + 1) * wstep + (m < 2 ? 1024 : 0));
-      __builtin_amdgcn_sched_barrier(0);
-    }
-  }
-  TW_PRIO(0);
-}
-
 __global__ __launch_bounds__(512) void tail_ws_kernel(TwArgs a) {
   __shared__ __attribute__((aligned(1024))) char lds[TW_LDS];
-  const int tid = threadIdx.x, lane = tid & 63, f = lane & 31, h = lane >> 5;
-  const int wv = __builtin_amdgcn_readfirstlane(tid >> 6);
-  const HdrRegs H = load_hdr(reinterpret_cast<const Header*>(a.blob));
-  const h8* const blob8 = reinterpret_cast<const h8*>(a.blob);
-  const f32x4* const blob4 = reinterpret_cast<const f32x4*>(a.blob);
-
-  int64_t fbg = (int64_t)blockIdx.x * 8 + wv;
-  const bool wave_live = fbg < a.nfb;
-  fbg = wave_live ? fbg : a.nfb - 1;
-  const int64_t row = fbg * 32 + f;
-  const bool row_live = wave_live && row < a.B;
-
-  LdsW* const ring = (LdsW*)(lds);
-  auto issue = [&](int idx, int slot_off) {
-    if (idx >= TW_UNITS) return;
-    uint32_t off, n16;
-    tw_unit(H, idx, off, n16);
-    const int npieces = (int)(n16 >> 6);
-#pragma unroll
-    for (int i = 0; i < TW_SLOT / 8192; ++i) {
-      const int pc = wv + 8 * i;
-      if (pc < npieces)
-        __builtin_amdgcn_global_load_lds((const __attribute__((address_space(1))) void*)(blob8 + off + pc * 64 + lane),
-                                         (__attribute__((address_space(3))) void*)(ring + slot_off + pc * 1024), 16, 0, 0);
-    }
-  };
-#ifdef TW_STAMPS
-  int tw_u = 0;
-#define TWS(i)                                                                                                                \
-  do {                                                                                                                        \
-    if (a.latent && lane == 0)                                                                                                \
-      reinterpret_cast<unsigned long long*>(a.latent)[((size_t)blockIdx.x * 8 + wv) * 96 + (i)] = __builtin_amdgcn_s_memtime(); \
-  } while (0)
-#define TW_STAMP_MID() TWS(2 + 2 * tw_u)
-#define TW_STAMP_END() do { TWS(3 + 2 * tw_u); ++tw_u; } while (0)
-#else
-#define TWS(i) do { } while (0)
-#define TW_STAMP_MID() do { } while (0)
-#define TW_STAMP_END() do { } while (0)
-#endif
-  TWS(0);
-  issue(0, 0);
-
-  {
-    f32x4* const bl = reinterpret_cast<f32x4*>(lds + TW_O_BIAS);
-#pragma unroll
-    for (int s = ST_E3; s < NUM_STAGES; ++s) {
-      const f32x4* src = blob4 + tw_b_off(s, H.k8_e0);
-      for (int i = tid; i < tw_bias_n16(s); i += 512) bl[tw_bias_off(s) / 16 + i] = src[i];
-    }
-  }
-  h8 x3[TrunkFrags::STEPS][2];
-  {
-    const u4* src = a.h3 + TrunkFrags::unit(fbg, 0, 0, 0) + lane;
-#pragma unroll
-    for (int ks = 0; ks < TrunkFrags::STEPS; ++ks)
-#pragma unroll
-      for (int p = 0; p < 2; ++p) x3[ks][p] = __builtin_bit_cast(h8, src[TrunkFrags::frag(0, ks, p)]);
-  }
-  asm volatile("s_waitcnt vmcnt(0)" ::: "memory");
-  __syncthreads();
-  TWS(1);
-
-  int cur = 0;
-  LdsC* const bias0 = (LdsC*)(lds + TW_O_BIAS) + 64 * h;
-  LdsC* const wl0 = (LdsC*)(lds) + lane * 16;
-  LdsW* const latw = (LdsW*)(lds + TW_O_LAT) + wv * TW_LAT_WAVE + f * 8;
-#ifdef TW_NO_SKEW
-  const bool late = false;
-#else
-  const bool late = wv >= 4;
-#endif
-#define TW_BEGIN(idx) issue((idx) + 1, cur ^ TW_SLOT); LdsC* const wl = wl0 + cur
-#define TW_MID()                                      \
-  TW_STAMP_MID();                                     \
-  asm volatile("s_waitcnt vmcnt(0)" ::: "memory");    \
-  if (late) __syncthreads()
-#define TW_END()                                      \
-  asm volatile("s_waitcnt vmcnt(0)" ::: "memory");    \
-  if (!late) __syncthreads();                         \
-  TW_STAMP_END();                                     \
-  cur ^= TW_SLOT
-
-  f32x16 acc[2];
-  auto emit = [&](auto act, const f32x16& ac, float inv, h8 (&d0)[2], h8 (&d1)[2]) {
-    h8 fr[2][2];
-    frags_from_acc<decltype(act)::value>(ac, inv, fr);
-    d0[0] = fr[0][0]; d0[1] = fr[0][1]; d1[0] = fr[1][0]; d1[1] = fr[1][1];
-  };
-  constexpr std::integral_constant<int, ACT_RELU> RELU{};
-  constexpr std::integral_constant<int, ACT_TANH> TANH{};
-  const float inv3 = H.inv_scale[ST_E3], inv4 = H.inv_scale[ST_E4], inv5 = H.inv_scale[ST_E5];
-  constexpr int JB3 = (int)(tw_job_w16(ST_E3) * 16), JB4 = (int)(tw_job_w16(ST_E4) * 16);
-
-  h8 x4[8][2];
-#pragma unroll
-  for (int u = 0; u < 2; ++u) {
-    TW_BEGIN(u);
-    LdsC* const b = bias0 + tw_bias_off(ST_E3) + (2 * u) * 128;
-    tw_job2p<16>(acc, wl, wl + JB3, 2048, b, b + 128, x3);
-    TW_MID();
-    emit(RELU, acc[0], inv3, x4[4 * u], x4[4 * u + 1]);
-    emit(RELU, acc[1], inv3, x4[4 * u + 2], x4[4 * u + 3]);
-    TW_END();
-  }
-  h8 x5[4][2];
-  {
-    TW_BEGIN(2);
-    LdsC* const b = bias0 + tw_bias_off(ST_E4);
-    tw_job2<8>(acc, wl, wl + JB4, 2048, b, b + 128, x4);
-    TW_MID();
-    emit(TANH, acc[0], inv4, x5[0], x5[1]);
-    emit(TANH, acc[1], inv4, x5[2], x5[3]);
-    TW_END();
-  }
-  {
-    TW_BEGIN(3);
-    LdsC* const b = bias0 + tw_bias_off(ST_E5);
-    tw_job2<4>(acc, wl, wl + 2048, 4096, b, b + 128, x5);
-    TW_MID();
-#ifndef TW_STAMPS
-    if (a.latent && row_live) {
-#pragma unroll
-      for (int nb = 0; nb < 2; ++nb)
-#pragma unroll
-        for (int q = 0; q < 16; ++q) {
-          const int rowi = 32 * nb + (q & 3) + 8 * (q >> 2) + 4 * h, g = rowi >> 4, cc = rowi & 15;
-          if (g < 3 && cc < 3) a.latent[row * NLML_LATENT + 3 * g + cc] = acc[nb][q] * inv5;
-        }
-    }
-#endif
-#pragma unroll
-    for (int nb = 0; nb < 2; ++nb) {
-      h8 fr[2][2];
-      frags_from_acc<ACT_NONE>(acc[nb], inv5, fr);
-#pragma unroll
-      for (int p = 0; p < 2; ++p)
-#pragma unroll
-        for (int pc = 0; pc < 2; ++pc)
-          if (2 * nb + p < 3 && h == 0) {
-            const u4 t = __builtin_bit_cast(u4, fr[p][pc]);
-            typedef unsigned u2 __attribute__((ext_vector_type(2)));
-            *reinterpret_cast<__attribute__((address_space(3))) u2*>(latw + ((2 * nb + p) * 2 + pc) * 256) = u2{t[0], t[1]};
-          }
-    }
-    TW_END();
-  }
-#pragma unroll 1
-  for (int g = 0; g < 3; ++g) {
-    const int u0 = 4 + TW_HEAD_UNITS * g;
-    const float i0 = H.inv_scale[ST_H0], i1 = H.inv_scale[ST_H1], i2 = H.inv_scale[ST_H2], i3 = H.inv_scale[ST_H3];
-    h8 xa[8][2];
-    {
-      TW_BEGIN(u0);
-      h8 xin[1][2];
-#pragma unroll
-      for (int pc = 0; pc < 2; ++pc) {
-        typedef unsigned u2 __attribute__((ext_vector_type(2)));
-        const u2 t = *reinterpret_cast<const __attribute__((address_space(3))) u2*>((LdsC*)latw + (g * 2 + pc) * 256);
-        xin[0][pc] = __builtin_bit_cast(h8, u4{h == 0 ? t[0] : 0u, h == 0 ? t[1] : 0u, 0u, 0u});
-      }
-      LdsC* const b = bias0 + tw_bias_off(ST_H0) + (4 * g) * 128;
-      constexpr int JB = (int)(tw_job_w16(ST_H0) * 16);
-#pragma unroll
-      for (int jj = 0; jj < 2; ++jj) {
-        tw_job2<1>(acc, wl + (2 * jj) * JB, wl + (2 * jj + 1) * JB, 2048, b + (2 * jj) * 128, b + (2 * jj + 1) * 128, xin);
-        if (jj == 1) { TW_MID(); }
-        emit(RELU, acc[0], i0, xa[4 * jj], xa[4 * jj + 1]);
-        emit(RELU, acc[1], i0, xa[4 * jj + 2], xa[4 * jj + 3]);
-      }
-      TW_END();
-    }
-    h8 xb[16][2];
-#pragma unroll
-    for (int j = 0; j < 4; ++j) {
-      TW_BEGIN(u0 + 1 + j);
-      LdsC* const b = bias0 + tw_bias_off(ST_H1) + (4 * g + j) * 256;
-      tw_job2p<8>(acc, wl, wl + 2048, 4096, b, b + 128, xa);
-      TW_MID();
-      emit(RELU, acc[0], i1, xb[4 * j], xb[4 * j + 1]);
-      emit(RELU, acc[1], i1, xb[4 * j + 2], xb[4 * j + 3]);
-      TW_END();
-    }
-    h8 xc[8][2];
-#pragma unroll
-    for (int u = 0; u < 2; ++u) {
-      TW_BEGIN(u0 + 5 + u);
-      constexpr int JB = (int)(tw_job_w16(ST_H2) * 16);
-      LdsC* const b = bias0 + tw_bias_off(ST_H2) + (4 * g + 2 * u) * 128;
-      tw_job2p<16>(acc, wl, wl + JB, 2048, b, b + 128, xb);
-      TW_MID();
-      emit(RELU, acc[0], i2, xc[4 * u], xc[4 * u + 1]);
-      emit(RELU, acc[1], i2, xc[4 * u + 2], xc[4 * u + 3]);
-      TW_END();
-    }
-    h8 xd[4][2];
-    {
-      TW_BEGIN(u0 + 7);
-      LdsC* const b = bias0 + tw_bias_off(ST_H3) + (2 * g) * 128;
-      tw_job2p<8>(acc, wl, wl + (int)(tw_job_w16(ST_H3) * 16), 2048, b, b + 128, xc);
-      TW_MID();
-      emit(RELU, acc[0], i3, xd[0], xd[1]);
-      emit(RELU, acc[1], i3, xd[2], xd[3]);
-      TW_END();
-    }
-    {
-      TW_BEGIN(u0 + 8);
-      LdsC* const b = bias0 + tw_bias_off(ST_H4) + g * 128;
-      tw_job2<4, 1>(acc, wl, wl, 2048, b, b, xd);
-      TW_MID();
-      if (h == 0 && row_live) a.out[row * 3 + g] = acc[0][0] * H.inv_scale[ST_H4];
-      TW_END();
-    }
-  }
-#undef TW_BEGIN
-#undef TW_MID
-#undef TW_END
+  tail_ws_body(a, (int64_t)blockIdx.x * 8, lds);
 }
 
 }
diff --git a/nlml_hpe_amd/csrc/encoder_heads_f16x2_tailws_dev.h b/nlml_hpe_amd/csrc/encoder_heads_f16x2_tailws_dev.h
--- /dev/null
+++ b/nlml_hpe_amd/csrc/encoder_heads_f16x2_tailws_dev.h
@@ -0,0 +1,363 @@
+#pragma once
+#include <hip/hip_runtime.h>
+
+#include "../../include/nlml_hpe.h"
+#include "abi_internal.h"
+#include "encoder_heads_f16x2_dev.h"
+#include "layout.h"
+
+#if defined(__HIP_DEVICE_COMPILE__) && !defined(__gfx950__)
+#error "global_load_lds_dwordx4: gfx950"
+#endif
+
+namespace nlml {
+namespace hx {
+
+typedef unsigned u4 __attribute__((ext_vector_type(4)));
+#define TW_PRIO(p) __builtin_amdgcn_s_setprio(p)
+typedef __attribute__((address_space(3))) const char LdsC;
+typedef __attribute__((address_space(3))) char LdsW;
+
+struct TwArgs {
+  const void* blob;
+  const u4* h3;
+  float* out;
+  float* latent;
+  int64_t B, nfb;
+};
+
+constexpr int TW_SLOT = 65536;
+constexpr int tw_bias_n16(int s) { return kStages[s].jobs * kStages[s].nb * 8; }
+constexpr int tw_bias_off(int s) {
+  int o = 0;
+  for (int t = ST_E3; t < s; ++t) o += tw_bias_n16(t) * 16;
+  return o;
+}
+constexpr uint32_t tw_b_off(int s, uint32_t k16_e0) {
+  int c = (int)(sizeof(Header) / 16), m = 0;
+  for (int t = 0; t < s; ++t) {
+    c += kStages[t].jobs * ((t == ST_E0 ? 0 : kStages[t].k8 * kStages[t].nb * 64 * PIECES) + kStages[t].nb * 8);
+    m += kStages[t].jobs * (t == ST_E0 ? kStages[t].nb * 64 * PIECES : 0);
+  }
+  return c + m * k16_e0 + kStages[s].jobs * ((s == ST_E0 ? 0 : kStages[s].k8 * kStages[s].nb * 64 * PIECES) + (s == ST_E0 ? kStages[s].nb * 64 * PIECES : 0) * k16_e0);
+}
+constexpr bool tw_b_off_is_layouts() {
+  for (int s = 0; s < NUM_STAGES; ++s)
+    if (tw_b_off(s, 0u) != layout_b_off(kLayoutHX, s, 0u) || tw_b_off(s, 88u) != layout_b_off(kLayoutHX, s, 88u)) return false;
+  return true;
+}
+static_assert(tw_b_off_is_layouts(), "the written-out bias offsets are layout.h's");
+constexpr int TW_O_BIAS = 2 * TW_SLOT;
+constexpr int TW_O_LAT = TW_O_BIAS + ((tw_bias_off(NUM_STAGES) + 511) / 512) * 512;
+constexpr int TW_LAT_WAVE = 3 * 2 * 256;
+constexpr int TW_LDS = TW_O_LAT + 8 * TW_LAT_WAVE;
+static_assert(TW_LDS <= 163840, "LDS map");
+
+constexpr int TW_HEAD_UNITS = 9, TW_UNITS = 4 + 3 * TW_HEAD_UNITS;
+constexpr uint32_t tw_job_w16(int s) { return layout_job_w16(kLayoutHX, s, 0u); }
+__device__ __forceinline__ void tw_unit(const HdrRegs& H, int idx, uint32_t& off, uint32_t& n16) {
+  constexpr uint32_t J3 = tw_job_w16(ST_E3), J4 = tw_job_w16(ST_E4), J5 = tw_job_w16(ST_E5);
+  constexpr uint32_t K0 = tw_job_w16(ST_H0), K1 = tw_job_w16(ST_H1), K2 = tw_job_w16(ST_H2), K3 = tw_job_w16(ST_H3), K4 = tw_job_w16(ST_H4);
+  static_assert(2 * J3 * 16 == TW_SLOT && 2 * J4 * 16 <= TW_SLOT && J5 * 16 <= TW_SLOT && 4 * K0 * 16 <= TW_SLOT && K1 * 16 <= TW_SLOT &&
+                    2 * K2 * 16 == TW_SLOT && 2 * K3 * 16 <= TW_SLOT && K4 * 16 <= TW_SLOT,
+                "a unit fits a buffer");
+  if (idx < 2) { n16 = 2 * J3; off = H.w_off(ST_E3) + idx * 2 * J3; }
+  else if (idx == 2) { n16 = 2 * J4; off = H.w_off(ST_E4); }
+  else if (idx == 3) { n16 = J5; off = H.w_off(ST_E5); }
+  else {
+    const int k = idx - 4, g = k / TW_HEAD_UNITS, r = k - TW_HEAD_UNITS * g;
+    if (r == 0) { n16 = 4 * K0; off = H.w_off(ST_H0) + 4 * g * K0; }
+    else if (r <= 4) { n16 = K1; off = H.w_off(ST_H1) + (4 * g + (r - 1)) * K1; }
+    else if (r <= 6) { n16 = 2 * K2; off = H.w_off(ST_H2) + (4 * g + 2 * (r - 5)) * K2; }
+    else if (r == 7) { n16 = 2 * K3; off = H.w_off(ST_H3) + 2 * g * K3; }
+    else { n16 = K4; off = H.w_off(ST_H4) + g * K4; }
+  }
+}
+
+template <int K16, int NCH = 2>
+__device__ __forceinline__ void tw_job2(f32x16 (&acc)[2], LdsC* w0, LdsC* w1, int wstep, LdsC* b0, LdsC* b1, const h8 (&in)[K16][2]) {
+  typedef const __attribute__((address_space(3))) h8 LdsH8;
+#pragma unroll
+  for (int c = 0; c < NCH; ++c)
+#pragma unroll
+    for (int q = 0; q < 4; ++q) {
+      const f32x4 v = *reinterpret_cast<const __attribute__((address_space(3))) f32x4*>((c ? b1 : b0) + q * 16);
+      acc[c][4 * q + 0] = v[0];
+      acc[c][4 * q + 1] = v[1];
+      acc[c][4 * q + 2] = v[2];
+      acc[c][4 * q + 3] = v[3];
+    }
+  TW_PRIO(2);
+#pragma unroll
+  for (int ks = 0; ks < K16; ++ks) {
+    h8 wf[NCH][2];
+#pragma unroll
+    for (int c = 0; c < NCH; ++c)
+#pragma unroll
+      for (int p = 0; p < 2; ++p) wf[c][p] = *reinterpret_cast<LdsH8*>((c ? w1 : w0) + ks * wstep + p * 1024);
+#pragma unroll
+    for (int t = 0; t < 3; ++t)
+#pragma unroll
+      for (int c = 0; c < NCH; ++c)
+        acc[c] = __builtin_amdgcn_mfma_f32_32x32x16_f16(wf[c][t == 0 ? 1 : 0], in[ks][t == 1 ? 1 : 0], acc[c], 0, 0, 0);
+  }
+  TW_PRIO(0);
+}
+
+template <int K16>
+__device__ __forceinline__ void tw_job2p(f32x16 (&acc)[2], LdsC* w0, LdsC* w1, int wstep, LdsC* b0, LdsC* b1, const h8 (&in)[K16][2]) {
+  typedef const __attribute__((address_space(3))) h8 LdsH8;
+#pragma unroll
+  for (int c = 0; c < 2; ++c)
+#pragma unroll
+    for (int q = 0; q < 4; ++q) {
+      const f32x4 v = *reinterpret_cast<const __attribute__((address_space(3))) f32x4*>((c ? b1 : b0) + q * 16);
+      acc[c][4 * q + 0] = v[0];
+      acc[c][4 * q + 1] = v[1];
+      acc[c][4 * q + 2] = v[2];
+      acc[c][4 * q + 3] = v[3];
+    }
+  h8 wf[2][2][2];
+#pragma unroll
+  for (int c = 0; c < 2; ++c)
+#pragma unroll
+    for (int p = 0; p < 2; ++p) wf[0][c][p] = *reinterpret_cast<LdsH8*>((c ? w1 : w0) + p * 1024);
+  TW_PRIO(2);
+  __builtin_amdgcn_sched_barrier(0);
+#pragma unroll
+  for (int ks = 0; ks < K16; ++ks) {
+#pragma unroll
+    for (int m = 0; m < 6; ++m) {
+      const int t = m >> 1, c = m & 1;
+      acc[c] = __builtin_amdgcn_mfma_f32_32x32x16_f16(wf[ks & 1][c][t == 0 ? 1 : 0], in[ks][t == 1 ? 1 : 0], acc[c], 0, 0, 0);
+      __builtin_amdgcn_sched_barrier(0);
+      if (m < 4 && ks + 1 < K16)
+        wf[(ks + 1) & 1][m & 1][m < 2 ? 1 : 0] = *reinterpret_cast<LdsH8*>(((m & 1) ? w1 : w0) + (ks + 1) * wstep + (m < 2 ? 1024 : 0));
+      __builtin_amdgcn_sched_barrier(0);
+    }
+  }
+  TW_PRIO(0);
+}
+
+__device__ __forceinline__ void tail_ws_body(const TwArgs& a, int64_t block0, char* const lds) {
+  const int tid = threadIdx.x, lane = tid & 63, f = lane & 31, h = lane >> 5;
+  const int wv = __builtin_amdgcn_readfirstlane(tid >> 6);
+  const HdrRegs H = load_hdr(reinterpret_cast<const Header*>(a.blob));
+  const h8* const blob8 = reinterpret_cast<const h8*>(a.blob);
+  const f32x4* const blob4 = reinterpret_cast<const f32x4*>(a.blob);
+
+  int64_t fbg = block0 + wv;
+  const bool wave_live = fbg < a.nfb;
+  fbg = wave_live ? fbg : a.nfb - 1;
+  const int64_t row = fbg * 32 + f;
+  const bool row_live = wave_live && row < a.B;
+
+  LdsW* const ring = (LdsW*)(lds);
+  auto issue = [&](int idx, int slot_off) {
+    if (idx >= TW_UNITS) return;
+    uint32_t off, n16;
+    tw_unit(H, idx, off, n16);
+    const int npieces = (int)(n16 >> 6);
+#pragma unroll
+    for (int i = 0; i < TW_SLOT / 8192; ++i) {
+      const int pc = wv + 8 * i;
+      if (pc < npieces)
+        __builtin_amdgcn_global_load_lds((const __attribute__((address_space(1))) void*)(blob8 + off + pc * 64 + lane),
+                                         (__attribute__((address_space(3))) void*)(ring + slot_off + pc * 1024), 16, 0, 0);
+    }
+  };
+#ifdef TW_STAMPS
+  int tw_u = 0;
+#define TWS(i)                                                                                                                \
+  do {                                                                                                                        \
+    if (a.latent && lane == 0)                                                                                                \
+      reinterpret_cast<unsigned long long*>(a.latent)[((size_t)blockIdx.x * 8 + wv) * 96 + (i)] = __builtin_amdgcn_s_memtime(); \
+  } while (0)
+#define TW_STAMP_MID() TWS(2 + 2 * tw_u)
+#define TW_STAMP_END() do { TWS(3 + 2 * tw_u); ++tw_u; } while (0)
+#else
+#define TWS(i) do { } while (0)
+#define TW_STAMP_MID() do { } while (0)
+#define TW_STAMP_END() do { } while (0)
+#endif
+  TWS(0);
+  issue(0, 0);
+
+  {
+    f32x4* const bl = reinterpret_cast<f32x4*>(lds + TW_O_BIAS);
+#pragma unroll
+    for (int s = ST_E3; s < NUM_STAGES; ++s) {
+      const f32x4* src = blob4 + tw_b_off(s, H.k8_e0);
+      for (int i = tid; i < tw_bias_n16(s); i += 512) bl[tw_bias_off(s) / 16 + i] = src[i];
+    }
+  }
+  h8 x3[TrunkFrags::STEPS][2];
+  {
+    const u4* src = a.h3 + TrunkFrags::unit(fbg, 0, 0, 0) + lane;
+#pragma unroll
+    for (int ks = 0; ks < TrunkFrags::STEPS; ++ks)
+#pragma unroll
+      for (int p = 0; p < 2; ++p) x3[ks][p] = __builtin_bit_cast(h8, src[TrunkFrags::frag(0, ks, p)]);
+  }
+  asm volatile("s_waitcnt vmcnt(0)" ::: "memory");
+  __syncthreads();
+  TWS(1);
+
+  int cur = 0;
+  LdsC* const bias0 = (LdsC*)(lds + TW_O_BIAS) + 64 * h;
+  LdsC* const wl0 = (LdsC*)(lds) + lane * 16;
+  LdsW* const latw = (LdsW*)(lds + TW_O_LAT) + wv * TW_LAT_WAVE + f * 8;
+#ifdef TW_NO_SKEW
+  const bool late = false;
+#else
+  const bool late = wv >= 4;
+#endif
+#define TW_BEGIN(idx) issue((idx) + 1, cur ^ TW_SLOT); LdsC* const wl = wl0 + cur
+#define TW_MID()                                      \
+  TW_STAMP_MID();                                     \
+  asm volatile("s_waitcnt vmcnt(0)" ::: "memory");    \
+  if (late) __syncthreads()
+#define TW_END()                                      \
+  asm volatile("s_waitcnt vmcnt(0)" ::: "memory");    \
+  if (!late) __syncthreads();                         \
+  TW_STAMP_END();                                     \
+  cur ^= TW_SLOT
+
+  f32x16 acc[2];
+  auto emit = [&](auto act, const f32x16& ac, float inv, h8 (&d0)[2], h8 (&d1)[2]) {
+    h8 fr[2][2];
+    frags_from_acc<decltype(act)::value>(ac, inv, fr);
+    d0[0] = fr[0][0]; d0[1] = fr[0][1]; d1[0] = fr[1][0]; d1[1] = fr[1][1];
+  };
+  constexpr std::integral_constant<int, ACT_RELU> RELU{};
+  constexpr std::integral_constant<int, ACT_TANH> TANH{};
+  const float inv3 = H.inv_scale[ST_E3], inv4 = H.inv_scale[ST_E4], inv5 = H.inv_scale[ST_E5];
+  constexpr int JB3 = (int)(tw_job_w16(ST_E3) * 16), JB4 = (int)(tw_job_w16(ST_E4) * 16);
+
+  h8 x4[8][2];
+#pragma unroll
+  for (int u = 0; u < 2; ++u) {
+    TW_BEGIN(u);
+    LdsC* const b = bias0 + tw_bias_off(ST_E3) + (2 * u) * 128;
+    tw_job2p<16>(acc, wl, wl + JB3, 2048, b, b + 128, x3);
+    TW_MID();
+    emit(RELU, acc[0], inv3, x4[4 * u], x4[4 * u + 1]);
+    emit(RELU, acc[1], inv3, x4[4 * u + 2], x4[4 * u + 3]);
+    TW_END();
+  }
+  h8 x5[4][2];
+  {
+    TW_BEGIN(2);
+    LdsC* const b = bias0 + tw_bias_off(ST_E4);
+    tw_job2<8>(acc, wl, wl + JB4, 2048, b, b + 128, x4);
+    TW_MID();
+    emit(TANH, acc[0], inv4, x5[0], x5[1]);
+    emit(TANH, acc[1], inv4, x5[2], x5[3]);
+    TW_END();
+  }
+  {
+    TW_BEGIN(3);
+    LdsC* const b = bias0 + tw_bias_off(ST_E5);
+    tw_job2<4>(acc, wl, wl + 2048, 4096, b, b + 128, x5);
+    TW_MID();
+#ifndef TW_STAMPS
+    if (a.latent && row_live) {
+#pragma unroll
+      for (int nb = 0; nb < 2; ++nb)
+#pragma unroll
+        for (int q = 0; q < 16; ++q) {
+          const int rowi = 32 * nb + (q & 3) + 8 * (q >> 2) + 4 * h, g = rowi >> 4, cc = rowi & 15;
+          if (g < 3 && cc < 3) a.latent[row * NLML_LATENT + 3 * g + cc] = acc[nb][q] * inv5;
+        }
+    }
+#endif
+#pragma unroll
+    for (int nb = 0; nb < 2; ++nb) {
+      h8 fr[2][2];
+      frags_from_acc<ACT_NONE>(acc[nb], inv5, fr);
+#pragma unroll
+      for (int p = 0; p < 2; ++p)
+#pragma unroll
+        for (int pc = 0; pc < 2; ++pc)
+          if (2 * nb + p < 3 && h == 0) {
+            const u4 t = __builtin_bit_cast(u4, fr[p][pc]);
+            typedef unsigned u2 __attribute__((ext_vector_type(2)));
+            *reinterpret_cast<__attribute__((address_space(3))) u2*>(latw + ((2 * nb + p) * 2 + pc) * 256) = u2{t[0], t[1]};
+          }
+    }
+    TW_END();
+  }
+#pragma unroll 1
+  for (int g = 0; g < 3; ++g) {
+    const int u0 = 4 + TW_HEAD_UNITS * g;
+    const float i0 = H.inv_scale[ST_H0], i1 = H.inv_scale[ST_H1], i2 = H.inv_scale[ST_H2], i3 = H.inv_scale[ST_H3];
+    h8 xa[8][2];
+    {
+      TW_BEGIN(u0);
+      h8 xin[1][2];
+#pragma unroll
+      for (int pc = 0; pc < 2; ++pc) {
+        typedef unsigned u2 __attribute__((ext_vector_type(2)));
+        const u2 t = *reinterpret_cast<const __attribute__((address_space(3))) u2*>((LdsC*)latw + (g * 2 + pc) * 256);
+        xin[0][pc] = __builtin_bit_cast(h8, u4{h == 0 ? t[0] : 0u, h == 0 ? t[1] : 0u, 0u, 0u});
+      }
+      LdsC* const b = bias0 + tw_bias_off(ST_H0) + (4 * g) * 128;
+      constexpr int JB = (int)(tw_job_w16(ST_H0) * 16);
+#pragma unroll
+      for (int jj = 0; jj < 2; ++jj) {
+        tw_job2<1>(acc, wl + (2 * jj) * JB, wl + (2 * jj + 1) * JB, 2048, b + (2 * jj) * 128, b + (2 * jj + 1) * 128, xin);
+        if (jj == 1) { TW_MID(); }
+        emit(RELU, acc[0], i0, xa[4 * jj], xa[4 * jj + 1]);
+        emit(RELU, acc[1], i0, xa[4 * jj + 2], xa[4 * jj + 3]);
+      }
+      TW_END();
+    }
+    h8 xb[16][2];
+#pragma unroll
+    for (int j = 0; j < 4; ++j) {
+      TW_BEGIN(u0 + 1 + j);
+      LdsC* const b = bias0 + tw_bias_off(ST_H1) + (4 * g + j) * 256;
+      tw_job2p<8>(acc, wl, wl + 2048, 4096, b, b + 128, xa);
+      TW_MID();
+      emit(RELU, acc[0], i1, xb[4 * j], xb[4 * j + 1]);
+      emit(RELU, acc[1], i1, xb[4 * j + 2], xb[4 * j + 3]);
+      TW_END();
+    }
+    h8 xc[8][2];
+#pragma unroll
+    for (int u = 0; u < 2; ++u) {
+      TW_BEGIN(u0 + 5 + u);
+      constexpr int JB = (int)(tw_job_w16(ST_H2) * 16);
+      LdsC* const b = bias0 + tw_bias_off(ST_H2) + (4 * g + 2 * u) * 128;
+      tw_job2p<16>(acc, wl, wl + JB, 2048, b, b + 128, xb);
+      TW_MID();
+      emit(RELU, acc[0], i2, xc[4 * u], xc[4 * u + 1]);
+      emit(RELU, acc[1], i2, xc[4 * u + 2], xc[4 * u + 3]);
+      TW_END();
+    }
+    h8 xd[4][2];
+    {
+      TW_BEGIN(u0 + 7);
+      LdsC* const b = bias0 + tw_bias_off(ST_H3) + (2 * g) * 128;
+      tw_job2p<8>(acc, wl, wl + (int)(tw_job_w16(ST_H3) * 16), 2048, b, b + 128, xc);
+      TW_MID();
+      emit(RELU, acc[0], i3, xd[0], xd[1]);
+      emit(RELU, acc[1], i3, xd[2], xd[3]);
+      TW_END();
+    }
+    {
+      TW_BEGIN(u0 + 8);
+      LdsC* const b = bias0 + tw_bias_off(ST_H4) + g * 128;
+      tw_job2<4, 1>(acc, wl, wl, 2048, b, b, xd);
+      TW_MID();
+      if (h == 0 && row_live) a.out[row * 3 + g] = acc[0][0] * H.inv_scale[ST_H4];
+      TW_END();
+    }
+  }
+#undef TW_BEGIN
+#undef TW_MID
+#undef TW_END
+}
+
+}
+}
diff --git a/nlml_hpe_amd/csrc/encoder_heads_f16x2_w8.hip b/nlml_hpe_amd/csrc/encoder_heads_f16x2_w8.hip
--- a/nlml_hpe_amd/csrc/encoder_heads_f16x2_w8.hip
+++ b/nlml_hpe_amd/csrc/encoder_heads_f16x2_w8.hip
@@ -4,6 +4,7 @@
 #include "abi_internal.h"
 #include "ipd_norm.h"
 #include "encoder_heads_f16x2_dev.h"
+#include "encoder_heads_f16x2_tailws_dev.h"
 #include "layout.h"
 
 #ifndef W8_D0_HI
@@ -201,10 +202,8 @@
 #define W8S_WALL(i) do { } while (0)
 #endif
 
-template <bool VEC4, bool NORM, bool TRUNK = false>
-__global__ __launch_bounds__(512) void encoder_heads_f16x2_w8_kernel(Args a) {
-  __shared__ __attribute__((aligned(16))) char lds[LDS_BYTES];
-
+template <bool VEC4, bool NORM, bool TRUNK, class ArgsT>
+__device__ __forceinline__ void w8_tile(ArgsT a, char* const lds, const int64_t tile) {
   const int tid = threadIdx.x;
   Ctx c;
   c.blob8 = reinterpret_cast<const h8*>(a.blob);
@@ -216,7 +215,7 @@
   c.h = c.lane >> 5;
   c.wv = __builtin_amdgcn_readfirstlane(tid >> 6);
   const int jw = c.wv >> 1, nbh = c.wv & 1;
-  const int64_t row0 = (int64_t)blockIdx.x * TILE_FACES;
+  const int64_t row0 = tile * TILE_FACES;
 
   {
     constexpr int WSTEP1 = 4 * 2 * 64;
@@ -290,7 +289,7 @@
     W8S(10);
     if constexpr (TRUNK) {
       typedef unsigned u4_ __attribute__((ext_vector_type(4)));
-      u4_* const dst = reinterpret_cast<u4_*>(a.h3ws) + (size_t)blockIdx.x * TrunkFrags::TILE_UNITS + c.lane;
+      u4_* const dst = reinterpret_cast<u4_*>(a.h3ws) + (size_t)tile * TrunkFrags::TILE_UNITS + c.lane;
 #pragma unroll
       for (int fb = 0; fb < 2; ++fb) {
         h8 fr[2][2];
@@ -319,6 +318,29 @@
 #else
   tail_stages<false, STRICT_INKERNEL_RESCUE_MAX, H1W8>(ct, a, row0, acc3, wr3);
 #endif
+}
+
+template <bool VEC4, bool NORM, bool TRUNK = false>
+__global__ __launch_bounds__(512) void encoder_heads_f16x2_w8_kernel(Args a) {
+  __shared__ __attribute__((aligned(16))) char lds[LDS_BYTES];
+  w8_tile<VEC4, NORM, TRUNK, const Args>(a, lds, (int64_t)blockIdx.x);
+}
+
+template <bool VEC4, bool NORM>
+__global__ __launch_bounds__(512) void encoder_heads_f16x2_w8q_kernel(Args a, TwArgs t) {
+  constexpr int QLDS = LDS_BYTES > TW_LDS ? LDS_BYTES : TW_LDS;
+  __shared__ __attribute__((aligned(1024))) char lds[QLDS];
+  const int64_t tile0 = (int64_t)blockIdx.x * 4, ntiles = t.nfb >> 1;
+#pragma unroll 1
+  for (int i = 0; i < 4; ++i) {
+    if (tile0 + i < ntiles) w8_tile<VEC4, NORM, true, const Args&>(a, lds, tile0 + i);
+    __syncthreads();
+  }
+  asm volatile("s_waitcnt vmcnt(0)" ::: "memory");
+  __builtin_amdgcn_fence(__ATOMIC_RELEASE, "workgroup");
+  __syncthreads();
+  __builtin_amdgcn_fence(__ATOMIC_ACQUIRE, "workgroup");
+  tail_ws_body(t, (int64_t)blockIdx.x * 8, lds);
 }
 
 }
@@ -348,18 +370,57 @@
   return launch_strict_reeval(x, ldx, raw, normalize, B, F, blob, out, latent, stream);
 }
 
-int launch_encoder_heads_f16x2_w8(const float* x, int64_t ldx, const float* raw, int normalize, int64_t B, int F,
-                                  const void* blob, float* out, float* latent, uint8_t* valid, void* stream) {
-  if (B == 0) return 0;
-  const K2Input in = k2_input(x, ldx, raw, normalize, F);
+
+static int launch_w8_fused_kernel(const K2Input& in, int64_t B, int F, const void* blob, float* out, float* latent, uint8_t* valid,
+                                  void* stream) {
   const hx::Args a = k2_args<hx::Args>(in, B, F, blob, out, latent, valid);
   const dim3 grid((unsigned)((B + TILE_FACES - 1) / TILE_FACES)), block(512);
   hipStream_t st = reinterpret_cast<hipStream_t>(stream);
   k2_with_variant(in, [&](auto V, auto N) {
     hipLaunchKernelGGL((hx::encoder_heads_f16x2_w8_kernel<decltype(V)::value, decltype(N)::value>), grid, block, 0, st, a);
   });
-  if (int rc = hip_launch_status()) return rc;
+  return hip_launch_status();
+}
+
+int launch_encoder_heads_f16x2_w8(const float* x, int64_t ldx, const float* raw, int normalize, int64_t B, int F,
+                                  const void* blob, float* out, float* latent, uint8_t* valid, void* stream) {
+  if (B == 0) return 0;
+  if (int rc = launch_w8_fused_kernel(k2_input(x, ldx, raw, normalize, F), B, F, blob, out, latent, valid, stream)) return rc;
   return launch_strict_reeval(x, ldx, raw, normalize, B, F, blob, out, latent, stream);
 }
 
-}
+size_t quad_workspace_bytes(int64_t quad_faces) { return quad_faces <= 0 ? 0 : hx::TrunkFrags::bytes(quad_faces); }
+
+int launch_encoder_heads_f16x2_w8_mixed(const float* x, int64_t ldx, const float* raw, int normalize, int64_t B, int F,
+                                        const void* blob, float* out, float* latent, uint8_t* valid, int64_t quad_faces,
+                                        void* workspace, size_t ws_bytes, void* stream) {
+  if (B == 0) return 0;
+  if (quad_faces < 0 || quad_faces > B || (quad_faces < B && quad_faces % (4 * TILE_FACES)))
+    return fail(NLML_E_BADARG, "quad path: the quad part is whole workgroups of 256 faces, or the whole batch");
+  K2Input in = k2_input(x, ldx, raw, normalize, F);
+  if (quad_faces > 0) {
+    if (!workspace || ws_bytes < quad_workspace_bytes(quad_faces)) return fail(NLML_E_BADARG, "quad path: workspace too small");
+    if (reinterpret_cast<uintptr_t>(workspace) & 15) return fail(NLML_E_BADARG, "quad path: workspace must be 16-byte aligned");
+    if (!in.vec4) return fail(NLML_E_BADARG, "quad path: x must be 16-byte aligned with F and ldx multiples of 4");
+    hx::Args a = k2_args<hx::Args>(in, quad_faces, F, blob, out, latent, valid);
+    a.h3ws = workspace;
+    const int64_t ntiles = (quad_faces + TILE_FACES - 1) / TILE_FACES;
+    hx::TwArgs t;
+    t.blob = blob; t.h3 = reinterpret_cast<const hx::u4*>(workspace); t.out = out; t.latent = latent; t.B = quad_faces; t.nfb = 2 * ntiles;
+    const dim3 grid((unsigned)((ntiles + 3) / 4)), block(512);
+    hipStream_t st = reinterpret_cast<hipStream_t>(stream);
+    if (a.norm) hipLaunchKernelGGL((hx::encoder_heads_f16x2_w8q_kernel<true, true>), grid, block, 0, st, a, t);
+    else hipLaunchKernelGGL((hx::encoder_heads_f16x2_w8q_kernel<true, false>), grid, block, 0, st, a, t);
+    if (int rc = hip_launch_status()) return rc;
+  }
+  if (quad_faces < B) {
+    K2Input rest = in;
+    rest.src = in.src + quad_faces * in.ld;
+    if (int rc = launch_w8_fused_kernel(rest, B - quad_faces, F, blob, out + quad_faces * 3,
+                                        latent ? latent + quad_faces * NLML_LATENT : nullptr, valid ? valid + quad_faces : nullptr, stream))
+      return rc;
+  }
+  return launch_strict_reeval(x, ldx, raw, normalize, B, F, blob, out, latent, stream);
+}
+
+}
diff --git a/nlml_hpe_amd/csrc/torch_ops.cpp b/nlml_hpe_amd/csrc/torch_ops.cpp
--- a/nlml_hpe_amd/csrc/torch_ops.cpp
+++ b/nlml_hpe_amd/csrc/torch_ops.cpp
@@ -138,7 +138,22 @@
   float* const out = r.pose.data_ptr<float>();
   const size_t blob_bytes = (size_t)blob.numel();
   OnDevice dev(in);
-  if (landmarks) {
+  at::Tensor quad_ws;
+  if (!ws && B > 0 && F > 0 && F % 4 == 0 && blob_bytes == nlml_encoder_heads_packed_bytes((int)F, NLML_MODE_F16X2S) &&
+      (landmarks || B == 1 || in.stride(0) % 4 == 0) && reinterpret_cast<uintptr_t>(in.data_ptr<float>()) % 16 == 0) {
+    int64_t quad_faces = 0;
+    size_t quad_bytes = 0;
+    check(nlml_k2_quad_faces(B, &quad_faces, &quad_bytes), "nlml_k2_quad_faces");
+    if (quad_faces > 0) quad_ws = at::empty({(int64_t)quad_bytes}, in.options().dtype(at::kByte));
+  }
+  if (quad_ws.defined()) {
+    if (landmarks)
+      check(nlml_landmarks_to_pose_ws(in.data_ptr<float>(), B, normalize ? 1 : 0, blob.data_ptr(), blob_bytes, out, nullptr, valid,
+                                      quad_ws.data_ptr(), (size_t)quad_ws.numel(), dev.stream), "nlml_landmarks_to_pose_ws");
+    else
+      check(nlml_encoder_heads_fwd_ws(in.data_ptr<float>(), B > 1 ? in.stride(0) : F, B, (int)F, blob.data_ptr(), blob_bytes, out, nullptr,
+                                      valid, quad_ws.data_ptr(), (size_t)quad_ws.numel(), dev.stream), "nlml_encoder_heads_fwd_ws");
+  } else if (landmarks) {
     const int norm = normalize ? 1 : 0;
     if (ws)
       check(nlml_landmarks_to_pose_small(in.data_ptr<float>(), B, norm, blob.data_ptr(), blob_bytes, out, nullptr, valid, ws->data_ptr(),
diff --git a/nlml_hpe_amd/ops.py b/nlml_hpe_amd/ops.py
--- a/nlml_hpe_amd/ops.py
+++ b/nlml_hpe_amd/ops.py
@@ -127,9 +127,9 @@
 _k2_ws: dict = {}
 
 
-def _k2_workspace(form: str, B: int, F: int, device, floor_faces: int = 0) -> torch.Tensor:
+def _k2_workspace(form: str, B: int, F: int, device, floor_faces: int = 0, need_bytes: int = 0) -> torch.Tensor:
     size_of = _lib.lib().nlml_encoder_heads_small_workspace_bytes if form == "small" else _lib.lib().nlml_encoder_heads_workspace_bytes
-    need = max(16, size_of(B, F))
+    need = max(16, need_bytes or size_of(B, F))
     pool = _k2_ws.setdefault((form, str(device), _stream_ptr(device)), [])
     for ws in pool:
         if ws.numel() >= need:
@@ -141,6 +141,20 @@
 
 def _small_workspace(B: int, F: int, device) -> torch.Tensor:
     return _k2_workspace("small", B, F, device, floor_faces=4096)
+
+
+def _k2_quad_part(B: int, F: int, src: torch.Tensor, blob: torch.Tensor) -> int:
+    import ctypes as C
+    L = _lib.lib()
+    if B <= 0 or blob.numel() != L.nlml_encoder_heads_packed_bytes(F, _lib.MODE_F16X2S):
+        return 0
+    ld = src.stride(0) if (src.dim() == 2 and B > 1) else F
+    if F % 4 or ld % 4 or src.data_ptr() % 16:
+        return 0
+    n, need = C.c_int64(0), C.c_size_t(0)
+    with torch.cuda.device(src.device):
+        rc = L.nlml_k2_quad_faces(B, C.byref(n), C.byref(need))
+    return int(need.value) if rc == 0 and n.value > 0 else 0
 
 
 def _k2_forward(form: str, x, raw, blob: torch.Tensor, F: int, normalize, return_latent: bool, return_valid: bool, workspace=None):
@@ -162,10 +176,13 @@
         head = (src.data_ptr(), B, int(bool(normalize)))
     dev = src.device
     tail = ()
+    quad_bytes = 0 if form else _k2_quad_part(B, F, src, blob)
+    if quad_bytes:
+        form = "ws"
     if form:
         symbol += "_" + form
         if workspace is None:
-            workspace = _small_workspace(B, F, dev) if form == "small" else _k2_workspace(form, B, F, dev)
+            workspace = _small_workspace(B, F, dev) if form == "small" else _k2_workspace(form, B, F, dev, need_bytes=quad_bytes)
         tail = (workspace.data_ptr(), workspace.numel())
     out = torch.empty((B, 3), dtype=torch.float32, device=dev)
     latent = torch.empty((B, LATENT), dtype=torch.float32, device=dev) if return_latent else None
@@ -360,6 +377,16 @@
 def landmarks_to_pose_streamed(raw: torch.Tensor, blob: torch.Tensor, normalize: bool = True, return_latent: bool = False,
                                return_valid: bool = False, workspace: torch.Tensor | None = None):
     return _k2_forward("streamed", None, raw, blob, F_REF, normalize, return_latent, return_valid, workspace)
+
+
+def landmarks_to_pose_quad(raw: torch.Tensor, blob: torch.Tensor, normalize: bool = True, return_latent: bool = False,
+                           return_valid: bool = False, workspace: torch.Tensor | None = None):
+    return _k2_forward("quad", None, raw, blob, F_REF, normalize, return_latent, return_valid, workspace)
+
+
+def encoder_heads_fwd_quad(x: torch.Tensor, blob: torch.Tensor, F: int, return_latent: bool = False,
+                           return_valid: bool = False, workspace: torch.Tensor | None = None):
+    return _k2_forward("quad", x, None, blob, F, None, return_latent, return_valid, workspace)
 
 
 _eval_ws: dict = {}
```

Measured after the change: 76.80 million (median of 6 runs). 2.0% higher.
